# serycjon/MFT

Measured on AMD Instinct MI355X. Metric: tracked frames/sec at 512x512, 12 RAFT iters; flow EPE vs reference, higher is better.
Workload: dtype f32 (update-block products as split fp16 x 3 on the fp16 matrix cores, fp32 accumulation; error per product <= ~2^-23, see DESIGN.md section 4 and parity below); 1 GPU; MFT.track on synthetic 512x512 video, deltas [inf,1,2,4,8,16,32], 7/7.00/7 (min/mean/max) flow pairs per timed frame, 12 RAFT iters, seeded synthetic weights (BASELINE.json configs[1]); parallelism=single GPU, frames_resident_in_hbm=True, preroll_frames=32

## Files before the change

### include/mftx.h

```cpp
#ifndef MFTX_H
#define MFTX_H

#include <stddef.h>
#include <stdint.h>

#ifdef __cplusplus
extern "C" {
#endif

#define MFTX_VERSION 400

#define MFTX_E_ARG (-1)
#define MFTX_E_ALIGN (-2)
#define MFTX_E_WORKSPACE (-3)
#define MFTX_E_STATE (-4)

#define MFTX_MAX_CANDIDATES 16

int mftx_version(void);
const char *mftx_last_error_string(void);

#define MFTX_PROFILE_CATEGORIES 14
int mftx_profile_begin(void);
int mftx_profile_end(double *ms, double *work, long long *count, int n);
// ... 20 lines not shown
                     float *out, int ld_out, float *hx, int ld_hx, void *stream);

int mftx_fmap_pyramid(const float *f2, int P, int C, int h, int w, float *lvl1, float *lvl2, float *lvl3, void *stream);
int mftx_corr_lookup_ondemand(const float *f1, const float *f2l0, const float *f2l1, const float *f2l2, const float *f2l3,
                              const float *coords, int P, int C, int h, int w, int r,
                              float *out, int ld_out, void *stream);

typedef struct mftx_conv_desc {
    const float *a0; int lda0; int c0;
    const float *a1; int lda1; int c1;
    const float *wpk; const float *bias;
    float *out; int ldo;
    int P, h, w;
    int N;
    int kh, kw;
    int act;
    float out_scale;
    const float *addend; int ld_addend;
    int stride, hin, win, pad_y, pad_x, residual_mode;
    int arith;
    int a_split, out_split;
} mftx_conv_desc;
#define MFTX_ARITH_F32 0
#define MFTX_ARITH_SPLIT 1
int mftx_conv2d(const mftx_conv_desc *d, void *stream);
int mftx_conv2d_tile(const mftx_conv_desc *d, int tile, void *stream);

int mftx_pack_tile_conv_weights(const float *wpk, int N, int taps, int cin, int cin_pad, void *wtile, void *stream);
int mftx_tile_conv2d(const mftx_conv_desc *d, const void *wtile, void *stream);
#define MFTX_OU_HEADS_WTILE_BYTES 6635520
int mftx_pack_ou_heads_weights(const float *w1pk, int cin_pad, const float *w2pk, void *wtile, void *wproj, void *stream);
int mftx_ou_heads(const float *a_split, int lda, int P, int h, int w, const void *wtile, const float *b1, const void *wproj, const float *b2,
                  float *T, float *out, int ld_out, void *stream);
int mftx_gru_half(const float *h_in, int ld_hin, const float *motion, int ld_mo, const void *wzr, const void *wq, const float *pre_zr,
                  const float *pre_q, float *z, const float *hf_in, float *hf_out, float *h_out, int ld_hout, int P, int h, int w, int pass,
                  void *stream);
int mftx_tile_conv_fills_chip(int P, int h, int w);
#define MFTX_FLOW_HEAD_WEIGHT_BYTES 32768
int mftx_pack_flow_head_weights(const float *w2pk, void *wproj, void *stream);
int mftx_flow_head(const float *hsplit, int ld_h, int P, int h, int w, const void *wtile, const float *b1, const void *wproj,
                   const float *b2, float *T, float *delta, float *coords, void *stream);
int mftx_split_weights(const float *wpk, void *out, long long n_floats, void *stream);
#define MFTX_SPLIT_LIMIT 65504.0f
int mftx_count_not_below(const float *x, long long n, float limit, unsigned *count, void *stream);

typedef struct mftx_raft mftx_raft;
#define MFTX_RAFT_NUM_WEIGHTS 34
int mftx_raft_create(const float *const *weights, int n_weights, mftx_raft **out);
void mftx_raft_destroy(mftx_raft *r);
size_t mftx_raft_workspace_bytes(int P, int h, int w);
int mftx_raft_set_ondemand(mftx_raft *r, int on);
int mftx_raft_set_split_weights(mftx_raft *r, const void *const *split, int n);
int mftx_raft_arith(const mftx_raft *r);
int mftx_raft_set_lookup_fused(mftx_raft *r, const void *wfused);
int mftx_raft_set_flow_fused(mftx_raft *r, const void *wflow);
int mftx_raft_set_tile_weights(mftx_raft *r, const void *const *tile, int n);
int mftx_raft_set_flow_head(mftx_raft *r, const void *wproj);
int mftx_raft_set_ou_heads(mftx_raft *r, const void *wtile, const void *wproj);
int mftx_raft_set_coords_trace(mftx_raft *r, float *trace);
#define MFTX_RAFT_OPT_FORK 0
#define MFTX_RAFT_OPT_PRESPLIT 1
#define MFTX_RAFT_OPT_GROUP 2
#define MFTX_RAFT_OPT_FUSE_LOOKUP 3
#define MFTX_RAFT_OPT_GRAPH 4
#define MFTX_RAFT_OPT_FUSE_FLOW 5
#define MFTX_RAFT_OPT_TILE_CONV 6
#define MFTX_RAFT_OPT_FUSE_HEAD 7
#define MFTX_RAFT_OPT_TILE_VOLUME 8
#define MFTX_RAFT_OPT_FUSE_GRU 9
#define MFTX_RAFT_OPT_TILE_CELLS 10
#define MFTX_RAFT_OPT_FUSE_OU 11
#define MFTX_RAFT_OPT_TILE_CONV2P 12
int mftx_raft_set_option(mftx_raft *r, int option, int value);
int mftx_raft_set_nonfinite_counter(mftx_raft *r, unsigned *counter);
int mftx_raft_clear_graphs(mftx_raft *r);
int mftx_raft_graph_stats(const mftx_raft *r, unsigned long long *captures, unsigned long long *replays);
size_t mftx_raft_workspace_bytes_for(const mftx_raft *r, int P, int h, int w);
int mftx_raft_workspace_layout(int P, int h, int w, size_t *offsets, int n);
int mftx_raft_workspace_layout_for(const mftx_raft *r, int P, int h, int w, size_t *offsets, int n);
int mftx_raft_refine(mftx_raft *r, int P, int h, int w, int iters,
                     const float *fmap1, const float *fmap2, const float *net, const float *inp,
                     const float *flow_init,
                     int pad_left, int pad_right, int pad_top, int pad_bottom,
                     float *flow, float *occl, float *sigma, float *packed, float *flow_lr,
                     void *workspace, size_t workspace_bytes, void *stream);
int mftx_raft_refine_gather(mftx_raft *r, int P, int h, int w, int iters, const float *const *fmap1,
                            const float *const *fmap2, const float *const *net, const float *const *inp,
                            const float *flow_init, int pad_left, int pad_right, int pad_top, int pad_bottom,
                            float *flow, float *occl, float *sigma, float *packed, float *flow_lr_out,
                            void *workspace, size_t workspace_bytes, void *stream);
size_t mftx_raft_frame_prepare_bytes(int h, int w);
int mftx_raft_frame_prepare(mftx_raft *r, int h, int w, const float *fmap, const float *inp, float *ctx_zr1, float *ctx_q1,
                            float *ctx_zr2, float *ctx_q2, void *fmap_split, void *scratch, size_t scratch_bytes, void *stream);
int mftx_raft_refine_gather_ex(mftx_raft *r, int P, int h, int w, int iters, const float *const *fmap1,
                               const float *const *fmap2, const float *const *net, const float *const *inp,
                               const float *const *ctx_parts, const void *const *fmap1_split, const void *fmap2_split,
                               const float *flow_init, int pad_left, int pad_right, int pad_top, int pad_bottom,
                               float *flow, float *occl, float *sigma, float *packed, float *flow_lr_out,
                               void *workspace, size_t workspace_bytes, void *stream);
int mftx_volume_query_split(const float *in, void *out, long long n_floats, void *stream);

typedef struct mftx_encoder mftx_encoder;
int mftx_encoder_create(const float *const *weights, int n_weights, int instance_norm, mftx_encoder **out);
int mftx_encoder_set_split_weights(mftx_encoder *e, const void *const *split, int n);
int mftx_encoder_set_graph(mftx_encoder *e, int on);
void mftx_encoder_destroy(mftx_encoder *e);
size_t mftx_encoder_workspace_bytes(int H0, int W0);
int mftx_encoder_forward(mftx_encoder *e, const uint8_t *img, int H0, int W0, float *out0, float *out1,
                         void *workspace, size_t workspace_bytes, void *stream);

int mftx_convex_upsample(const float *flow_lr, const float *ou, int ld_ou, const float *mask,
                         int P, int h, int w,
                         int pad_left, int pad_right, int pad_top, int pad_bottom,
                         float *flow, float *occl, float *sigma, float *packed, void *stream);

int mftx_chain(const float *flowL, const float *occlL, const float *sigmaL,
               const float *flowR, const float *occlR, const float *sigmaR,
               int H, int W, float *flowO, float *occlO, float *sigmaO, void *stream);

int mftx_warp_backward(const float *flow, const float *img, int C, int H, int W, float *out, void *stream);

int mftx_select(int K, const float *const *flow, const float *const *occl, const float *const *sigma,
                float thr, int H, int W,
                float *flowO, float *occlO, float *sigmaO, int8_t *chosen, void *stream);

int mftx_chain_select(int K,
                      const float *const *flowL, const float *const *occlL, const float *const *sigmaL,
                      const float *const *flowR, const float *const *occlR, const float *const *sigmaR,
                      float thr, int H, int W,
                      float *flowO, float *occlO, float *sigmaO, int8_t *chosen, void *stream);

int mftx_chain_select_packed(int K,
// ... 43 lines not shown
```

### mft_amd/_lib.py

```python
from __future__ import annotations

import ctypes as C
import os
from pathlib import Path

_HERE = Path(__file__).resolve().parent
LIB_PATH = _HERE / "libmftx.so"

MAX_CANDIDATES = 16
NUM_RAFT_WEIGHTS = 34
LOOKUP_CONVC1_WEIGHT_BYTES = 393216
FLOW_BRANCH_WEIGHT_BYTES = 352256
FLOW_HEAD_WEIGHT_BYTES = 32768
OU_HEADS_WTILE_BYTES = 6635520
SPLIT_LIMIT = 65504.0


class ConvDesc(C.Structure):
    _fields_ = [("a0", C.c_void_p), ("lda0", C.c_int), ("c0", C.c_int),
                ("a1", C.c_void_p), ("lda1", C.c_int), ("c1", C.c_int),
                ("wpk", C.c_void_p), ("bias", C.c_void_p),
                ("out", C.c_void_p), ("ldo", C.c_int),
                ("P", C.c_int), ("h", C.c_int), ("w", C.c_int),
                ("N", C.c_int), ("kh", C.c_int), ("kw", C.c_int),
                ("act", C.c_int), ("out_scale", C.c_float),
                ("addend", C.c_void_p), ("ld_addend", C.c_int),
                ("stride", C.c_int), ("hin", C.c_int), ("win", C.c_int), ("pad_y", C.c_int), ("pad_x", C.c_int),
                ("residual_mode", C.c_int), ("arith", C.c_int), ("a_split", C.c_int), ("out_split", C.c_int)]


_PP = C.POINTER(C.c_void_p)

SIGNATURES = {
    "mftx_version": (C.c_int, []),
    "mftx_last_error_string": (C.c_char_p, []),
    "mftx_profile_begin": (C.c_int, []),
    "mftx_profile_end": (C.c_int, [C.POINTER(C.c_double), C.POINTER(C.c_double), C.POINTER(C.c_longlong), C.c_int]),
    "mftx_corr_pyramid": (C.c_int, [C.c_void_p, C.c_void_p, C.c_int, C.c_int, C.c_int, C.c_int,
                                    C.c_void_p, C.c_void_p, C.c_void_p, C.c_void_p, C.c_void_p]),
    "mftx_corr_pyramid_split": (C.c_int, [C.c_void_p, C.c_void_p, C.c_int, C.c_int, C.c_int, C.c_int,
                                          C.c_void_p, C.c_void_p, C.c_void_p, C.c_void_p, C.c_void_p, C.c_void_p]),
    "mftx_corr_pyramid_layout": (C.c_int, [C.c_int, C.c_int, C.POINTER(C.c_longlong), C.POINTER(C.c_int)]),
    "mftx_corr_lookup": (C.c_int, [C.c_void_p] * 5 + [C.c_int] * 4 + [C.c_void_p, C.c_int, C.c_void_p]),
    "mftx_fmap_pyramid": (C.c_int, [C.c_void_p] + [C.c_int] * 4 + [C.c_void_p] * 4),
    "mftx_corr_lookup_ondemand": (C.c_int, [C.c_void_p] * 6 + [C.c_int] * 5 + [C.c_void_p, C.c_int, C.c_void_p]),
    "mftx_raft_set_ondemand": (C.c_int, [C.c_void_p, C.c_int]),
    "mftx_raft_workspace_bytes_for": (C.c_size_t, [C.c_void_p, C.c_int, C.c_int, C.c_int]),
    "mftx_conv2d": (C.c_int, [C.POINTER(ConvDesc), C.c_void_p]),
    "mftx_conv2d_tile": (C.c_int, [C.POINTER(ConvDesc), C.c_int, C.c_void_p]),
    "mftx_encoder_set_split_weights": (C.c_int, [C.c_void_p, _PP, C.c_int]),
    "mftx_raft_set_split_weights": (C.c_int, [C.c_void_p, _PP, C.c_int]),
    "mftx_raft_arith": (C.c_int, [C.c_void_p]),
    "mftx_raft_set_lookup_fused": (C.c_int, [C.c_void_p, C.c_void_p]),
    "mftx_raft_set_flow_fused": (C.c_int, [C.c_void_p, C.c_void_p]),
    "mftx_raft_set_tile_weights": (C.c_int, [C.c_void_p, _PP, C.c_int]),
    "mftx_raft_set_flow_head": (C.c_int, [C.c_void_p, C.c_void_p]),
    "mftx_raft_set_ou_heads": (C.c_int, [C.c_void_p, C.c_void_p, C.c_void_p]),
    "mftx_pack_ou_heads_weights": (C.c_int, [C.c_void_p, C.c_int, C.c_void_p, C.c_void_p, C.c_void_p, C.c_void_p]),
    "mftx_ou_heads": (C.c_int, [C.c_void_p, C.c_int, C.c_int, C.c_int, C.c_int, C.c_void_p, C.c_void_p, C.c_void_p, C.c_void_p, C.c_void_p,
                                C.c_void_p, C.c_int, C.c_void_p]),
    "mftx_pack_flow_head_weights": (C.c_int, [C.c_void_p, C.c_void_p, C.c_void_p]),
    "mftx_flow_head": (C.c_int, [C.c_void_p, C.c_int, C.c_int, C.c_int, C.c_int] + [C.c_void_p] * 8),
    "mftx_pack_tile_conv_weights": (C.c_int, [C.c_void_p, C.c_int, C.c_int, C.c_int, C.c_int, C.c_void_p, C.c_void_p]),
    "mftx_tile_conv2d": (C.c_int, [C.POINTER(ConvDesc), C.c_void_p, C.c_void_p]),
    "mftx_pack_flow_branch_weights": (C.c_int, [C.c_void_p, C.c_void_p, C.c_void_p, C.c_void_p]),
    "mftx_flow_branch": (C.c_int, [C.c_void_p, C.c_int, C.c_int, C.c_int, C.c_void_p, C.c_void_p, C.c_void_p, C.c_void_p,
                                   C.c_int, C.c_void_p, C.c_int, C.c_void_p]),
    "mftx_raft_set_option": (C.c_int, [C.c_void_p, C.c_int, C.c_int]),
    "mftx_raft_set_coords_trace": (C.c_int, [C.c_void_p, C.c_void_p]),
    "mftx_gru_half": (C.c_int, [C.c_void_p, C.c_int, C.c_void_p, C.c_int, C.c_void_p, C.c_void_p, C.c_void_p, C.c_void_p, C.c_void_p, C.c_void_p,
                                C.c_void_p, C.c_void_p, C.c_int, C.c_int, C.c_int, C.c_int, C.c_int, C.c_void_p]),
    "mftx_tile_conv_fills_chip": (C.c_int, [C.c_int, C.c_int, C.c_int]),
    "mftx_raft_clear_graphs": (C.c_int, [C.c_void_p]),
    "mftx_raft_set_nonfinite_counter": (C.c_int, [C.c_void_p, C.c_void_p]),
    "mftx_raft_graph_stats": (C.c_int, [C.c_void_p, C.POINTER(C.c_ulonglong), C.POINTER(C.c_ulonglong)]),
    "mftx_pack_lookup_convc1_weights": (C.c_int, [C.c_void_p, C.c_int, C.c_void_p, C.c_void_p]),
    "mftx_corr_lookup_convc1": (C.c_int, [C.c_void_p] * 5 + [C.c_int] * 3 + [C.c_void_p, C.c_void_p, C.c_void_p,
                                                                            C.c_int, C.c_int, C.c_void_p]),
    "mftx_split_weights": (C.c_int, [C.c_void_p, C.c_void_p, C.c_longlong, C.c_void_p]),
    "mftx_count_not_below": (C.c_int, [C.c_void_p, C.c_longlong, C.c_float, C.c_void_p, C.c_void_p]),
    "mftx_raft_create": (C.c_int, [_PP, C.c_int, C.POINTER(C.c_void_p)]),
    "mftx_raft_destroy": (None, [C.c_void_p]),
    "mftx_raft_workspace_bytes": (C.c_size_t, [C.c_int, C.c_int, C.c_int]),
    "mftx_raft_workspace_layout": (C.c_int, [C.c_int, C.c_int, C.c_int, C.POINTER(C.c_size_t), C.c_int]),
    "mftx_raft_workspace_layout_for": (C.c_int, [C.c_void_p, C.c_int, C.c_int, C.c_int, C.POINTER(C.c_size_t), C.c_int]),
    "mftx_raft_refine": (C.c_int, [C.c_void_p, C.c_int, C.c_int, C.c_int, C.c_int,
                                   C.c_void_p, C.c_void_p, C.c_void_p, C.c_void_p, C.c_void_p,
                                   C.c_int, C.c_int, C.c_int, C.c_int,
                                   C.c_void_p, C.c_void_p, C.c_void_p, C.c_void_p, C.c_void_p,
                                   C.c_void_p, C.c_size_t, C.c_void_p]),
    "mftx_raft_refine_gather": (C.c_int, [C.c_void_p, C.c_int, C.c_int, C.c_int, C.c_int,
                                          _PP, _PP, _PP, _PP, C.c_void_p,
                                          C.c_int, C.c_int, C.c_int, C.c_int,
                                          C.c_void_p, C.c_void_p, C.c_void_p, C.c_void_p, C.c_void_p,
                                          C.c_void_p, C.c_size_t, C.c_void_p]),
    "mftx_raft_refine_gather_ex": (C.c_int, [C.c_void_p, C.c_int, C.c_int, C.c_int, C.c_int,
                                             _PP, _PP, _PP, _PP, _PP, _PP, C.c_void_p, C.c_void_p,
                                             C.c_int, C.c_int, C.c_int, C.c_int,
                                             C.c_void_p, C.c_void_p, C.c_void_p, C.c_void_p, C.c_void_p,
                                             C.c_void_p, C.c_size_t, C.c_void_p]),
    "mftx_raft_frame_prepare_bytes": (C.c_size_t, [C.c_int, C.c_int]),
    "mftx_raft_frame_prepare": (C.c_int, [C.c_void_p, C.c_int, C.c_int] + [C.c_void_p] * 8 + [C.c_size_t, C.c_void_p]),
    "mftx_volume_query_split": (C.c_int, [C.c_void_p, C.c_void_p, C.c_longlong, C.c_void_p]),
    "mftx_encoder_create": (C.c_int, [_PP, C.c_int, C.c_int, C.POINTER(C.c_void_p)]),
    "mftx_encoder_destroy": (None, [C.c_void_p]),
    "mftx_encoder_set_graph": (C.c_int, [C.c_void_p, C.c_int]),
    "mftx_encoder_workspace_bytes": (C.c_size_t, [C.c_int, C.c_int]),
    "mftx_encoder_forward": (C.c_int, [C.c_void_p, C.c_void_p, C.c_int, C.c_int, C.c_void_p, C.c_void_p,
                                       C.c_void_p, C.c_size_t, C.c_void_p]),
    "mftx_convex_upsample": (C.c_int, [C.c_void_p, C.c_void_p, C.c_int, C.c_void_p] + [C.c_int] * 7
                             + [C.c_void_p] * 5),
    "mftx_chain": (C.c_int, [C.c_void_p] * 6 + [C.c_int, C.c_int] + [C.c_void_p] * 4),
    "mftx_warp_backward": (C.c_int, [C.c_void_p, C.c_void_p, C.c_int, C.c_int, C.c_int, C.c_void_p, C.c_void_p]),
    "mftx_select": (C.c_int, [C.c_int, _PP, _PP, _PP, C.c_float, C.c_int, C.c_int] + [C.c_void_p] * 5),
    "mftx_chain_select": (C.c_int, [C.c_int] + [_PP] * 6 + [C.c_float, C.c_int, C.c_int] + [C.c_void_p] * 5),
    "mftx_chain_select_packed": (C.c_int, [C.c_int] + [_PP] * 4 + [C.c_float, C.c_int, C.c_int] + [C.c_void_p] * 5),
    "mftx_chain_select_multi": (C.c_int, [C.c_int, C.POINTER(C.c_int)] + [_PP] * 4 + [C.c_float, C.c_int, C.c_int] + [_PP] * 4
                                + [C.c_void_p]),
    "mftx_sample_points": (C.c_int, [C.c_int, _PP, _PP, _PP, C.c_int, C.c_int, C.c_int, C.c_void_p, C.c_void_p,
                                     C.c_void_p, C.c_longlong, C.c_int, C.c_void_p]),
    "mftx_splat_forward": (C.c_int, [C.c_void_p, C.c_void_p, C.c_int, C.c_void_p, C.c_int, C.c_int, C.c_int, C.c_int, C.c_int,
                                     C.c_void_p, C.c_void_p]),
    "mftx_splat_resolve": (C.c_int, [C.c_void_p, C.c_int, C.c_int, C.c_int, C.c_int, C.c_float, C.c_int, C.c_void_p, C.c_void_p]),
    "mftx_overlay_edit": (C.c_int, [C.c_void_p, C.c_void_p, C.c_void_p, C.c_void_p, C.c_int, C.c_int, C.c_int, C.c_float,
                                    C.c_void_p, C.c_void_p, C.c_void_p]),
    "mftx_overlay_dots": (C.c_int, [C.c_void_p, C.c_void_p, C.c_int, C.c_int, C.c_void_p, C.c_longlong, C.c_int, C.c_double,
                                    C.c_int, C.c_int, C.c_int, C.c_void_p]),
    "mftx_quantize_workspace_bytes": (C.c_size_t, []),
    "mftx_quantize_u16": (C.c_int, [C.c_void_p, C.c_longlong, C.c_void_p, C.c_void_p, C.c_void_p, C.c_size_t, C.c_void_p]),
    "mftx_dequantize_u16": (C.c_int, [C.c_void_p, C.c_longlong, C.c_float, C.c_float, C.c_void_p, C.c_void_p]),
    "mftx_png_unfilter": (C.c_int, [C.c_void_p, C.c_int, C.c_int, C.c_int]),
    "mftx_copy_bytes": (C.c_int, [C.c_void_p, C.c_void_p, C.c_longlong, C.c_void_p]),
}
# ... 35 lines not shown
```

### mft_amd/csrc/common.h

```cpp
#pragma once
#include <hip/hip_runtime.h>
#include <cstdarg>
#include <cstdio>
#include <cstdint>
#include <cstdlib>
#include "../../include/mftx.h"

namespace mftx {

void set_error(const char *fmt, ...);

inline int fail(int code, const char *fmt, ...) {
    char buf[512];
    va_list ap;
    va_start(ap, fmt);
    vsnprintf(buf, sizeof buf, fmt, ap);
    va_end(ap);
    set_error("%s", buf);
    return code;
}

inline int check_launch(const char *what) {
    hipError_t e = hipGetLastError();
    if (e != hipSuccess) {
// ... 102 lines not shown
                       int ld_out, float *hx, int ld_hx, hipStream_t s, const float *T = nullptr, const float *b2h = nullptr,
                       float *coords_out = nullptr, float *delta_out = nullptr);
struct TileConvLaunch {
    const float *a0; int lda0;
    const float *a1; int lda1;
    int cin;
    const void *wf;
    const float *bias;
    const float *addend; int ld_addend;
    float *out; int ldo; int out_split;
    float *z, *rh, *hf, *hx; int ld_hf, ld_hx;
    const void *wproj; float *tout;
    int P, h, w, N, kh, kw, epi;
    int cells;
};
struct GruHalfLaunch {
    const float *h_in; int ld_hin; const float *mo; int ld_mo;
    const void *wzr, *wq;
    const float *pre_zr, *pre_q;
    const float *const *ctx;
    float *z; const float *hf_in; float *hf_out;
    float *h_out; int ld_hout;
    int P, h, w, pass;
    int cells;
};
int launch_gru_half(const GruHalfLaunch &d, hipStream_t s);
int launch_pack_flow_head(const float *w2pk, void *out, hipStream_t s);
int launch_pack_tile_conv2p(const float *wpk, int N, int cin_pad, void *out, hipStream_t s);
int launch_tile_conv2p(const float *a, int lda, const void *wf, const float *bias, float *out, int ldo, int n_valid, int P, int h, int w, int cells,
                       hipStream_t s);
constexpr size_t OU_HEAD_WTILE_BYTES = 8ull * 5 * 9 * 9 * 128 * 16, OU_HEAD_WPROJ_BYTES = 32768;
int launch_pack_ou_head(const float *w1pk, int cin_pad, const float *w2pk, void *wtile, void *wproj, hipStream_t s);
struct OuGather { const float *hx, *corr; int ld_corr; const float *coords1, *delta; float *flow_lr; };
int launch_ou_heads(const float *a, int lda, int P, int h, int w, const void *wtile, const float *b1, const void *wproj, const float *b2, float *T,
                    float *out, int ld_out, int cells, hipStream_t s, const OuGather *ga = nullptr);
int launch_flow_head_sum(const float *T, const float *b2, float *delta, const float *coords_in, float *coords_out, int P, int h, int w, hipStream_t s);
bool tile_conv_applicable(int kh, int kw, int cin, int N);
bool tile_conv_small_tiles_fill(int P, int h, int w);
bool tile_conv_fills_chip(int P, int h, int w, int kh, int kw);
int launch_pack_tile_conv(const float *wpk, int N, int taps, int cin, int cin_pad, void *out, hipStream_t s);
int launch_tile_conv(const TileConvLaunch &d, hipStream_t s);
int launch_fmap_pyramid(const float *f2, int P, int C, int h, int w, float *const lvl[3], hipStream_t s);
int launch_corr_ondemand(const float *f1, const float *const f2lvl[4], const float *coords, int P, int h, int w,
                         float *out, int ld_out, hipStream_t s);
int launch_convex_upsample(const float *flow_lr, const float *ou, int ld_ou, const float *mask,
                           int P, int h, int w, int pl, int pr, int pt, int pb,
                           float *flow, float *occl, float *sigma, float *packed, hipStream_t s, unsigned *nonfinite = nullptr);

}
```

### mft_amd/csrc/raft_engine.hip

```cpp
#include "common.h"
#include "profile.h"
#include "motion_front.h"
#include "graph_cache.h"
#include <cstdlib>
#include <new>

namespace mftx {


struct InitGather { int on; PairPtrs netp, inpp; };
struct CtxTable { const float **table; const float *own[4]; int supplied; PairPtrs parts[4]; };
__global__ void init_state_kernel(const float *__restrict__ net, const float *__restrict__ inp,
                                  const float *__restrict__ flow_init, float *hx, float *hf, float *coords1, int M, int h,
                                  int w, InitGather ga, CtxTable ct) {
    const long long i = (long long)blockIdx.x * blockDim.x + threadIdx.x;
    if (i >= (long long)M * 64) return;
    if (ct.table != nullptr && i < (long long)(M / (h * w)) * 4) {
        const int b = (int)(i >> 2), k = (int)(i & 3);
        ct.table[i] = ct.supplied ? ct.parts[k].p[b] : ct.own[k] + (long long)b * h * w * ((k & 1) ? 128 : 256);
    }
    const int m = (int)(i >> 6), q = (int)(i & 63);
    if (ga.on) {
        const int b = m / (h * w);
        net = ga.netp.p[b] - (long long)b * h * w * 128;
        inp = ga.inpp.p[b] - (long long)b * h * w * 128;
    }
    const float4 v = (q < 32) ? reinterpret_cast<const float4 *>(net)[(long long)m * 32 + q]
                              : reinterpret_cast<const float4 *>(inp)[(long long)m * 32 + (q - 32)];
    if (hf != nullptr) {
        store_split4v(hx + (long long)m * 384, 4 * q, v);
        if (q < 32) reinterpret_cast<float4 *>(hf + (long long)m * 128)[q] = v;
    } else {
        reinterpret_cast<float4 *>(hx + (long long)m * 384)[q] = v;
    }
    if (q == 0) {
        const int rem = m % (h * w);
        float cx = (float)(rem % w), cy = (float)(rem / w);
        if (flow_init != nullptr) {
            cx += flow_init[2 * (long long)m];
            cy += flow_init[2 * (long long)m + 1];
        }
        coords1[2 * (long long)m] = cx;
        coords1[2 * (long long)m + 1] = cy;
    }
}

__global__ __launch_bounds__(256) void convf1_kernel(ConvF1Args q) {
    __shared__ __attribute__((aligned(16))) float patch[2][7][48];
    const int half = threadIdx.x >> 7;
    convf1_strip(q, blockIdx.x * 2 + half, patch[half], threadIdx.x & 127);
}

__global__ __launch_bounds__(256) void lookup_convf1_kernel(LookupArgs lp, ConvF1Args q, int lookup_blocks, int f1_blocks) {
    __shared__ __attribute__((aligned(16))) float patch[2][7][48];
// ... 28 lines not shown
        } else v = load_split4(hx + (long long)m * 384 + 256, 4 * (q - 146));
        store_split4v(ouin + (long long)m * 712, 4 * q, v);
        return;
    }
    if (q < 64) v = reinterpret_cast<const float4 *>(hx + (long long)m * 384)[q];
    else if (q < 145) v = reinterpret_cast<const float4 *>(corr + (long long)m * ld_corr)[q - 64];
    else if (q == 145) {
        const int rem = m % (h * w);
        const float fx = coords1[2 * (long long)m] - (float)(rem % w);
        const float fy = coords1[2 * (long long)m + 1] - (float)(rem / w);
        v = make_float4(fx, fy, delta[2 * (long long)m], delta[2 * (long long)m + 1]);
        flow_lr[2 * (long long)m] = fx;
        flow_lr[2 * (long long)m + 1] = fy;
    } else v = reinterpret_cast<const float4 *>(hx + (long long)m * 384 + 256)[q - 146];
    reinterpret_cast<float4 *>(ouin + (long long)m * 712)[q] = v;
}

enum WeightSlot {
    W_CONVC1, B_CONVC1, W_CONVC2, B_CONVC2, W_CONVF1, B_CONVF1, W_CONVF2, B_CONVF2, W_CONV, B_CONV,
    W_ZR1_DYN, W_ZR1_INP, B_ZR1, W_Q1_DYN, W_Q1_INP, B_Q1, W_ZR2_DYN, W_ZR2_INP, B_ZR2, W_Q2_DYN, W_Q2_INP, B_Q2,
    W_FH1, B_FH1, W_FH2, B_FH2, W_MASK0, B_MASK0, W_MASK2, B_MASK2,
    W_OU1, B_OU1, W_OU2, B_OU2, W_COUNT
};

struct Workspace {
    float *lvl[4];
    float *f2l[3];
    float *coords1, *corr, *cor1, *corflo, *flo1, *hx, *z, *rh, *fh, *delta, *mask, *ouin, *ouh, *ou, *flow_lr;
    float *pre_zr[2], *pre_q[2];
    float *f2s;
    float *hf;
    float *hb, *hfb;
    const float **ctx;
    int ld_corr;
    size_t bytes;
};

static Workspace carve(void *base, int P, int h, int w, bool ondemand = false, bool split = false) {
    Workspace ws{};
    const size_t N = (size_t)h * w, M = (size_t)P * N;
    size_t off = 0;
    auto take = [&](size_t floats) {
        float *p = base ? reinterpret_cast<float *>(static_cast<char *>(base) + off) : nullptr;
        off += (floats * sizeof(float) + 255) & ~size_t(255);
        return p;
    };
    const PyramidLayout L = pyramid_layout(h, w);
    for (int l = 0; l < 4; ++l) ws.lvl[l] = take(ondemand ? 0 : M * (size_t)L.stride[l]);
    for (int l = 1; l < 4; ++l) ws.f2l[l - 1] = take(ondemand ? (size_t)P * (h >> l) * (w >> l) * 256 : 0);
    ws.coords1 = take(M * 2);
    ws.ld_corr = 324;
    ws.corr = take(M * ws.ld_corr);
    ws.cor1 = take(M * 256);
    ws.corflo = take(M * 256);
    ws.flo1 = take(M * 128);
    ws.hx = take(M * 384);
    ws.z = take(M * 128);
    ws.rh = take(M * 128);
    ws.fh = take(M * 256);
    ws.delta = take(M * 2);
    ws.mask = take(M * 576);
    ws.ouin = take(M * 712);
    ws.ouh = take(M * 256);
    ws.ou = take(M * 4);
    ws.flow_lr = take(M * 2);
    for (int pass = 0; pass < 2; ++pass) { ws.pre_zr[pass] = take(M * 256); ws.pre_q[pass] = take(M * 128); }
    ws.f2s = take(ondemand || !split ? 0 : M * 256);
    ws.hf = take(split ? M * 128 : 0);
    ws.hb = take(split ? M * 128 : 0);
    ws.hfb = take(split ? M * 128 : 0);
    ws.ctx = reinterpret_cast<const float **>(take(split ? (size_t)P * 8 : 0));
    ws.bytes = off;
    return ws;
}

}

using namespace mftx;

struct mftx_raft {
    uint32_t magic;
    int ondemand;
    int arith;
    const float *w[W_COUNT];
    const float *wg[W_COUNT];
    hipStream_t side;
    hipEvent_t ev_fork, ev_join;
    float *coords_trace;
    GraphCache *graphs;
    const void *wfused;
    const void *wflow;
    const void *wproj;
    const void *wt[W_COUNT];
    const void *wou, *wouproj;
    int opt[13];
    unsigned *nonfinite;
};
static constexpr int GEMM_SLOTS[] = {W_CONVC1, W_CONVC2, W_CONVF2, W_CONV, W_ZR1_DYN, W_ZR1_INP, W_Q1_DYN, W_Q1_INP,
                                     W_ZR2_DYN, W_ZR2_INP, W_Q2_DYN, W_Q2_INP, W_FH1, W_MASK0, W_MASK2, W_OU1};
static constexpr uint32_t RAFT_MAGIC = 0x4d465458;

extern "C" int mftx_raft_create(const float *const *weights, int n_weights, mftx_raft **out) {
    if (!weights || !out) return fail(MFTX_E_ARG, "raft_create: null pointer");
    if (n_weights != W_COUNT) return fail(MFTX_E_ARG, "raft_create: expected %d weight tensors, got %d", (int)W_COUNT, n_weights);
    for (int i = 0; i < W_COUNT; ++i) {
        if (!weights[i]) return fail(MFTX_E_ARG, "raft_create: weight %d is null", i);
        if (!aligned16(weights[i])) return fail(MFTX_E_ALIGN, "raft_create: weight %d not 16-byte aligned", i);
    }
    mftx_raft *r = new (std::nothrow) mftx_raft;
    if (!r) return fail(MFTX_E_ARG, "raft_create: out of host memory");
    r->magic = RAFT_MAGIC;
    r->ondemand = 0;
    r->arith = MFTX_ARITH_F32;
    r->side = nullptr; r->ev_fork = nullptr; r->ev_join = nullptr;
    r->wfused = nullptr;
    r->wflow = nullptr;
    r->wproj = nullptr;
    r->wou = nullptr; r->wouproj = nullptr;
    for (int i = 0; i < W_COUNT; ++i) r->wt[i] = nullptr;
    r->coords_trace = nullptr;
    r->nonfinite = nullptr;
    r->graphs = new (std::nothrow) GraphCache;
    r->opt[MFTX_RAFT_OPT_FORK] = -1; r->opt[MFTX_RAFT_OPT_PRESPLIT] = 1; r->opt[MFTX_RAFT_OPT_GROUP] = 1; r->opt[MFTX_RAFT_OPT_FUSE_LOOKUP] = 1; r->opt[MFTX_RAFT_OPT_GRAPH] = 1; r->opt[MFTX_RAFT_OPT_FUSE_FLOW] = 1; r->opt[MFTX_RAFT_OPT_TILE_CONV] = 1; r->opt[MFTX_RAFT_OPT_FUSE_HEAD] = 1; r->opt[MFTX_RAFT_OPT_TILE_VOLUME] = 1; r->opt[MFTX_RAFT_OPT_FUSE_GRU] = 1; r->opt[MFTX_RAFT_OPT_TILE_CELLS] = 0; r->opt[MFTX_RAFT_OPT_FUSE_OU] = 1; r->opt[MFTX_RAFT_OPT_TILE_CONV2P] = 1;
    for (int i = 0; i < W_COUNT; ++i) r->w[i] = r->wg[i] = weights[i];
    *out = r;
    return 0;
}

extern "C" void mftx_raft_destroy(mftx_raft *r) {
    if (r && r->magic == RAFT_MAGIC) {
        r->magic = 0;
        if (r->ev_fork) (void)hipEventDestroy(r->ev_fork);
        if (r->ev_join) (void)hipEventDestroy(r->ev_join);
        if (r->side) (void)hipStreamDestroy(r->side);
        delete r->graphs;
        delete r;
    }
}

static int ensure_side_stream(mftx_raft *r) {
    if (r->side) return 0;
    hipError_t e = hipStreamCreateWithFlags(&r->side, hipStreamNonBlocking);
    if (e == hipSuccess) e = hipEventCreateWithFlags(&r->ev_fork, hipEventDisableTiming);
    if (e == hipSuccess) e = hipEventCreateWithFlags(&r->ev_join, hipEventDisableTiming);
    if (e != hipSuccess) return fail((int)e, "raft_refine: side stream: %s", hipGetErrorString(e));
    return 0;
}

extern "C" size_t mftx_raft_workspace_bytes(int P, int h, int w) {
    if (P <= 0 || h <= 0 || w <= 0) return 0;
    return carve(nullptr, P, h, w).bytes;
// ... 34 lines not shown

extern "C" int mftx_raft_set_flow_fused(mftx_raft *r, const void *wflow) {
    if (!r || r->magic != RAFT_MAGIC) return fail(MFTX_E_STATE, "raft_set_flow_fused: bad handle");
    if (wflow && !aligned16(wflow)) return fail(MFTX_E_ALIGN, "raft_set_flow_fused: weights not 16-byte aligned");
    r->wflow = wflow;
    if (r->graphs) r->graphs->clear();
    return 0;
}

extern "C" int mftx_raft_set_tile_weights(mftx_raft *r, const void *const *tile, int n) {
    if (!r || r->magic != RAFT_MAGIC) return fail(MFTX_E_STATE, "raft_set_tile_weights: bad handle");
    if (r->graphs) r->graphs->clear();
    if (!tile) { for (int i = 0; i < W_COUNT; ++i) r->wt[i] = nullptr; return 0; }
    if (n != W_COUNT) return fail(MFTX_E_ARG, "raft_set_tile_weights: expected %d slots, got %d", (int)W_COUNT, n);
    for (int i = 0; i < W_COUNT; ++i)
        if (tile[i] && !aligned16(tile[i])) return fail(MFTX_E_ALIGN, "raft_set_tile_weights: slot %d not 16-byte aligned", i);
    for (int i = 0; i < W_COUNT; ++i) r->wt[i] = tile[i];
    return 0;
}

extern "C" int mftx_raft_set_flow_head(mftx_raft *r, const void *wproj) {
    if (!r || r->magic != RAFT_MAGIC) return fail(MFTX_E_STATE, "raft_set_flow_head: bad handle");
    if (wproj && !aligned16(wproj)) return fail(MFTX_E_ALIGN, "raft_set_flow_head: weights not 16-byte aligned");
    r->wproj = wproj;
    if (r->graphs) r->graphs->clear();
    return 0;
}

extern "C" int mftx_raft_set_ou_heads(mftx_raft *r, const void *wtile, const void *wproj) {
    if (!r || r->magic != RAFT_MAGIC) return fail(MFTX_E_STATE, "raft_set_ou_heads: bad handle");
    if ((wtile == nullptr) != (wproj == nullptr)) return fail(MFTX_E_ARG, "raft_set_ou_heads: both weight streams, or neither");
    if (wtile && (!aligned16(wtile) || !aligned16(wproj))) return fail(MFTX_E_ALIGN, "raft_set_ou_heads: weights not 16-byte aligned");
    r->wou = wtile; r->wouproj = wproj;
    if (r->graphs) r->graphs->clear();
    return 0;
}

extern "C" int mftx_raft_set_coords_trace(mftx_raft *r, float *trace) {
    if (!r || r->magic != RAFT_MAGIC) return fail(MFTX_E_STATE, "raft_set_coords_trace: bad handle");
    r->coords_trace = trace;
    return 0;
}

extern "C" int mftx_raft_clear_graphs(mftx_raft *r) {
    if (!r || r->magic != RAFT_MAGIC) return fail(MFTX_E_STATE, "raft_clear_graphs: bad handle");
    if (r->graphs) r->graphs->clear();
    return 0;
}

extern "C" int mftx_raft_set_nonfinite_counter(mftx_raft *r, unsigned *counter) {
    if (!r || r->magic != RAFT_MAGIC) return fail(MFTX_E_STATE, "raft_set_nonfinite_counter: bad handle");
    if (counter && (reinterpret_cast<uintptr_t>(counter) & 3)) return fail(MFTX_E_ALIGN, "raft_set_nonfinite_counter: counter not 4-byte aligned");
    r->nonfinite = counter;
    return 0;
}

extern "C" int mftx_raft_set_option(mftx_raft *r, int option, int value) {
    if (!r || r->magic != RAFT_MAGIC) return fail(MFTX_E_STATE, "raft_set_option: bad handle");
    if (option < 0 || option > MFTX_RAFT_OPT_TILE_CONV2P) return fail(MFTX_E_ARG, "raft_set_option: unknown option %d", option);
    r->opt[option] = value;
    if (r->graphs) r->graphs->clear();
    return 0;
}

extern "C" int mftx_raft_arith(const mftx_raft *r) {
    return (r && r->magic == RAFT_MAGIC) ? r->arith : -1;
// ... 5 lines not shown
}

static int workspace_layout(const mftx_raft *r, int P, int h, int w, size_t *offsets, int n) {
    if (P <= 0 || h <= 0 || w <= 0 || !offsets || n != 19) return fail(MFTX_E_ARG, "workspace_layout: need 19 slots");
    char *base = reinterpret_cast<char *>(uintptr_t(1) << 40);
    Workspace ws = carve(base, P, h, w, r && r->ondemand != 0, r && r->arith == MFTX_ARITH_SPLIT);
    float *ptrs[19] = {ws.lvl[0], ws.lvl[1], ws.lvl[2], ws.lvl[3], ws.coords1, ws.corr, ws.cor1, ws.corflo, ws.flo1,
                       ws.hx, ws.z, ws.rh, ws.fh, ws.delta, ws.mask, ws.ouin, ws.ouh, ws.ou, ws.flow_lr};
    for (int i = 0; i < 19; ++i) offsets[i] = (size_t)(reinterpret_cast<char *>(ptrs[i]) - base);
    return 0;
}
extern "C" int mftx_raft_workspace_layout(int P, int h, int w, size_t *offsets, int n) {
    return workspace_layout(nullptr, P, h, w, offsets, n);
}
extern "C" int mftx_raft_workspace_layout_for(const mftx_raft *r, int P, int h, int w, size_t *offsets, int n) {
    if (!r || r->magic != RAFT_MAGIC) return fail(MFTX_E_STATE, "workspace_layout_for: bad handle");
    return workspace_layout(r, P, h, w, offsets, n);
}

#define TRY(expr) do { int _e = (expr); if (_e) return _e; } while (0)

static mftx_conv_desc conv_desc(const float *a0, int lda0, int c0, const float *a1, int lda1, int c1,
                                const float *w, const float *b, float *out, int ldo, int P, int h, int wd, int N,
                                int kh, int kw, int act, float scale = 1.f, const float *addend = nullptr,
                                int ld_addend = 0) {
    mftx_conv_desc d{};
    d.addend = addend; d.ld_addend = ld_addend;
    d.a0 = a0; d.lda0 = lda0; d.c0 = c0; d.a1 = a1; d.lda1 = lda1; d.c1 = c1;
    d.wpk = w; d.bias = b; d.out = out; d.ldo = ldo; d.P = P; d.h = h; d.w = wd; d.N = N;
    d.kh = kh; d.kw = kw; d.act = act; d.out_scale = scale;
    return d;
}

struct RefineGather { PairPtrs f1, f2, net, inp; bool f2_shared; bool has_ctx, has_f1s; PairPtrs ctx[4], f1s; const float *f2s; };

static int launch_context_parts(const mftx_raft *r, bool tiles_on, bool sp, const float *inp, int ld, int P, int h, int w,
                                float *const zr[2], float *const q[2], hipStream_t s) {
    const float *const *W = r->w;
    const float *const *G = r->wg;
    for (int pass = 0; pass < 2; ++pass) {
        const int kh = pass ? 5 : 1, kw = pass ? 1 : 5;
        const int slot[2] = {pass ? W_ZR2_INP : W_ZR1_INP, pass ? W_Q2_INP : W_Q1_INP};
        const float *bias[2] = {W[pass ? B_ZR2 : B_ZR1], W[pass ? B_Q2 : B_Q1]};
        float *out[2] = {zr[pass], q[pass]};
        for (int k = 0; k < 2; ++k) {
            const int N = k ? 128 : 256;
            if (tiles_on && r->wt[slot[k]]) {
                TileConvLaunch t{};
                t.a0 = inp; t.lda0 = ld; t.cin = 128; t.wf = r->wt[slot[k]]; t.bias = bias[k];
                t.P = P; t.h = h; t.w = w; t.N = N; t.kh = kh; t.kw = kw; t.epi = 0;
                t.cells = r->opt[MFTX_RAFT_OPT_TILE_CELLS];
                t.out = out[k]; t.ldo = N;
                TRY(launch_tile_conv(t, s));
            } else {
                mftx_conv_desc d = conv_desc(inp, ld, 128, nullptr, 0, 0, G[slot[k]], bias[k], out[k], N, P, h, w, N, kh, kw, 0);
                d.arith = r->arith; d.a_split = sp; d.out_split = false;
                TRY(launch_conv(d, s));
            }
        }
    }
    return 0;
}
static int refine_impl(mftx_raft *r, int P, int h, int w, int iters, const float *fmap1,
                                const float *fmap2, const float *net, const float *inp, const float *flow_init,
                                int pad_left,
                                int pad_right, int pad_top, int pad_bottom, float *flow, float *occl,
                                float *sigma, float *packed, float *flow_lr_out, void *workspace,
// ... 23 lines not shown
    const bool use_graph = r->graphs && r->opt[MFTX_RAFT_OPT_GRAPH] != 0 && !prof_enabled() && !r->coords_trace && !ondemand;
    hipStream_t caller = s;
    bool proxied = false;
    if (use_graph && s == nullptr) {
        hipStream_t own = r->graphs->proxy.enter(s);
        if (own) { s = own; proxied = true; }
    }
    struct Leave { GraphCache *g; hipStream_t caller; bool on; ~Leave() { if (on) g->proxy.leave(caller); } } leave{r->graphs, caller, proxied};
    const int N = h * w, M = P * N;
    const float *const *W = r->w;
    const float *const *G = r->wg;
    const int AR = r->arith;
    auto gemm = [AR, SP](mftx_conv_desc d, bool a = true, bool o = false) { d.arith = AR; d.a_split = SP && a; d.out_split = SP && o; return d; };

    const float *f2lv[4] = {fmap2, ws.f2l[0], ws.f2l[1], ws.f2l[2]};
    if (ondemand) TRY(launch_fmap_pyramid(fmap2, P, 256, h, w, ws.f2l, s));
    else if (gather) {
        const long long pair_floats = (long long)N * 256;
        const float *f2s = ws.f2s;
        if (gather->f2_shared && gather->f2s) f2s = gather->f2s;
        else if (gather->f2_shared) TRY(launch_split_weights(gather->f2.p[0], ws.f2s, pair_floats, s));
        else for (int b = 0; b < P; ++b) TRY(launch_split_weights(gather->f2.p[b], ws.f2s + b * pair_floats, pair_floats, s));
        TRY(launch_volume_tile(nullptr, f2s, P, h, w, ws.lvl, s, gather->has_f1s ? &gather->f1s : &gather->f1, gather->f2_shared ? 0 : pair_floats,
                               gather->has_f1s));
    }
    else TRY(launch_corr_pyramid(fmap1, fmap2, P, 256, h, w, ws.lvl, s, r->arith == MFTX_ARITH_SPLIT ? ws.f2s : nullptr, r->opt[MFTX_RAFT_OPT_TILE_VOLUME]));
    const bool tiles_on = SP && r->opt[MFTX_RAFT_OPT_TILE_CONV] != 0 &&
                          (r->opt[MFTX_RAFT_OPT_TILE_CONV] == 2 ||
                           (tile_conv_fills_chip(P, h, w, 3, 3) && tile_conv_fills_chip(P, h, w, 1, 5) && tile_conv_fills_chip(P, h, w, 5, 1)));
    auto tile_w = [&](int slot) -> const void * { return tiles_on ? r->wt[slot] : nullptr; };
    const bool gru_fused = tile_w(W_ZR1_DYN) && tile_w(W_Q1_DYN) && tile_w(W_ZR2_DYN) && tile_w(W_Q2_DYN) &&
                           r->opt[MFTX_RAFT_OPT_FUSE_GRU] != 0;
    const bool ctx_supplied = gather && gather->has_ctx && gru_fused;
    {
        const long long slots = (long long)M * 64;
        ProfScope prof(PC_GLUE, s, 0);
        InitGather ga{};
        if (gather) { ga.on = 1; ga.netp = gather->net; ga.inpp = gather->inp; }
        CtxTable ct{};
        if (gru_fused) {
            ct.table = ws.ctx;
            ct.own[0] = ws.pre_zr[0]; ct.own[1] = ws.pre_q[0]; ct.own[2] = ws.pre_zr[1]; ct.own[3] = ws.pre_q[1];
            ct.supplied = ctx_supplied ? 1 : 0;
            if (ctx_supplied) for (int k = 0; k < 4; ++k) ct.parts[k] = gather->ctx[k];
        }
        hipLaunchKernelGGL(init_state_kernel, dim3((unsigned)((slots + 255) / 256)), dim3(256), 0, s, net, inp,
                           flow_init, ws.hx, SP ? ws.hf : nullptr, ws.coords1, M, h, w, ga, ct);
        TRY(check_launch("init_state"));
    }
    float *flow_lr = flow_lr_out ? flow_lr_out : ws.flow_lr;
    auto core = [&]() -> int {
    auto tile_layer = [&](const float *a0, int lda0, const float *a1, int lda1, const void *wf, const float *bias, int N, int kh, int kw, int epi) {
        TileConvLaunch t{};
        t.a0 = a0; t.lda0 = lda0; t.a1 = a1; t.lda1 = lda1; t.cin = a1 ? 256 : 128; t.wf = wf; t.bias = bias;
        t.P = P; t.h = h; t.w = w; t.N = N; t.kh = kh; t.kw = kw; t.epi = epi;
        t.cells = r->opt[MFTX_RAFT_OPT_TILE_CELLS];
        return t;
    };
    if (!ctx_supplied) TRY(launch_context_parts(r, tiles_on, SP, ws.hx + 128, 384, P, h, w, ws.pre_zr, ws.pre_q, s));
    const float *lv[4] = {ws.lvl[0], ws.lvl[1], ws.lvl[2], ws.lvl[3]};
    const int strips = cdiv(w, F1_CELLS);
    float *ccur = ws.coords1, *calt = ws.flo1;
    bool pending = false;
    for (int it = 0; it < iters; ++it) {
        const bool last = (it == iters - 1);
        if (r->coords_trace &&
            hipMemcpyAsync(r->coords_trace + (size_t)it * M * 2, ccur, (size_t)M * 8, hipMemcpyDeviceToDevice, s) != hipSuccess)
            return fail(MFTX_E_STATE, "raft_refine: coords trace copy failed");
        const ConvF1Args f1{ccur, W[W_CONVF1], W[B_CONVF1], ws.flo1, ws.hx, h, w, strips, P * h * strips, SP ? 1 : 0};
        const int f1_blocks = cdiv(f1.n_strips, 2);
        const bool nofuse = r->opt[MFTX_RAFT_OPT_GROUP] == 0, nopair = nofuse;
        const mftx_conv_desc c2 = gemm(conv_desc(ws.cor1, 256, 256, nullptr, 0, 0, G[W_CONVC2], W[B_CONVC2], ws.corflo, 256, P, h, w, 192, 3, 3, 1), true, true);
        const mftx_conv_desc f2 = gemm(conv_desc(ws.flo1, 128, 128, nullptr, 0, 0, G[W_CONVF2], W[B_CONVF2], ws.corflo + 192, 256, P, h, w, 64, 3, 3, 1), true, true);
        const int fork_env = r->opt[MFTX_RAFT_OPT_FORK];
        const bool fuse_flow = SP && r->wflow != nullptr && r->opt[MFTX_RAFT_OPT_FUSE_FLOW] != 0 && !nofuse;
        if (fuse_flow) {
            if (pending) {
                TRY(launch_flow_branch(ccur, P, h, w, r->wflow, W[B_CONVF1], W[B_CONVF2], ws.corflo + 192, 256, ws.hx, 384, s, ws.fh, W[B_FH2], calt, ws.delta));
                float *t = ccur; ccur = calt; calt = t;
                pending = false;
            } else TRY(launch_flow_branch(ccur, P, h, w, r->wflow, W[B_CONVF1], W[B_CONVF2], ws.corflo + 192, 256, ws.hx, 384, s));
        }
        const bool serial = fuse_flow || prof_enabled() || nofuse || (AR == MFTX_ARITH_SPLIT && (fork_env == 0 || fork_env == 2));
        const bool forked = !serial && AR == MFTX_ARITH_SPLIT;
        const bool flow_first = !fuse_flow && serial && fuse_lookup && fork_env == 2 && !prof_enabled() && !nofuse;
        if (flow_first) {
            hipLaunchKernelGGL(convf1_kernel, dim3(f1_blocks), dim3(256), 0, s, f1);
            TRY(check_launch("convf1"));
            TRY(launch_conv(f2, s));
        }
        if (forked) {
            TRY(ensure_side_stream(r));
// ... 73 lines not shown
        }
        const bool head_fused = tile_w(W_FH1) && r->wproj != nullptr && r->opt[MFTX_RAFT_OPT_FUSE_HEAD] != 0;
        if (head_fused) {
            TileConvLaunch t = tile_layer(ws.hx, 384, nullptr, 0, tile_w(W_FH1), W[B_FH1], 256, 3, 3, 4);
            t.wproj = r->wproj; t.tout = ws.fh;
            TRY(launch_tile_conv(t, s));
            const bool defer = !last && fuse_flow && r->opt[MFTX_RAFT_OPT_FUSE_HEAD] != 2 && !r->coords_trace;
            if (defer) pending = true;
            else {
                float *dst = last ? ws.coords1 : ccur;
                TRY(launch_flow_head_sum(ws.fh, W[B_FH2], ws.delta, ccur, dst, P, h, w, s));
                ccur = dst;
            }
        } else if (tile_w(W_FH1)) {
            TileConvLaunch t = tile_layer(ws.hx, 384, nullptr, 0, tile_w(W_FH1), W[B_FH1], 256, 3, 3, 1);
            t.out = ws.fh; t.ldo = 256;
            TRY(launch_tile_conv(t, s));
        } else TRY(launch_conv(gemm(conv_desc(ws.hx, 384, 128, nullptr, 0, 0, G[W_FH1], W[B_FH1], ws.fh, 256, P, h, w, 256, 3, 3, 1), true, false), s));
        if (!head_fused) {
            const mftx_conv_desc fh2 = conv_desc(ws.fh, 256, 256, nullptr, 0, 0, W[W_FH2], W[B_FH2], ws.delta, 2, P, h, w, 2, 3, 3, 0);
            if (!conv_small_applicable(fh2)) return fail(MFTX_E_STATE, "raft_refine: flow-head layer does not fit the small-N kernel");
            TRY(launch_conv_small(fh2, s, ccur, 2));
        }
        if (!last) continue;
        if (r->coords_trace &&
            hipMemcpyAsync(r->coords_trace + (size_t)iters * M * 2, ccur, (size_t)M * 8, hipMemcpyDeviceToDevice, s) != hipSuccess)
            return fail(MFTX_E_STATE, "raft_refine: coords trace copy failed");
        if (tile_w(W_MASK0)) {
            TileConvLaunch t = tile_layer(ws.hx, 384, nullptr, 0, tile_w(W_MASK0), W[B_MASK0], 256, 3, 3, 1);
            t.out = ws.fh; t.ldo = 256; t.out_split = SP ? 1 : 0;
            TRY(launch_tile_conv(t, s));
        } else TRY(launch_conv(gemm(conv_desc(ws.hx, 384, 128, nullptr, 0, 0, G[W_MASK0], W[B_MASK0], ws.fh, 256, P, h, w, 256, 3, 3, 1), true, true), s));
        TRY(launch_conv(gemm(conv_desc(ws.fh, 256, 256, nullptr, 0, 0, G[W_MASK2], W[B_MASK2], ws.mask, 576, P, h, w, 576, 1, 1, 0, 0.25f), true, false), s));
        const bool ou_fused = tiles_on && r->wou != nullptr && r->opt[MFTX_RAFT_OPT_FUSE_OU] != 0;
        if (!ou_fused || r->opt[MFTX_RAFT_OPT_FUSE_OU] == 2) {
            const long long slots = (long long)M * 178;
            ProfScope prof(PC_GLUE, s, 0);
            hipLaunchKernelGGL(ou_gather_kernel, dim3((unsigned)((slots + 255) / 256)), dim3(256), 0, s, ws.hx,
                               ws.corr, ws.ld_corr, ccur, ws.delta, ws.ouin, flow_lr, M, h, w, SP ? 1 : 0);
            TRY(check_launch("ou_gather"));
        }
        if (ou_fused) {
            const OuGather ga{ws.hx, ws.corr, ws.ld_corr, ccur, ws.delta, flow_lr};
            const bool mat = r->opt[MFTX_RAFT_OPT_FUSE_OU] == 2;
            TRY(launch_ou_heads(mat ? ws.ouin : nullptr, 712, P, h, w, r->wou, W[B_OU1], r->wouproj, W[B_OU2], ws.ouh, ws.ou, 4, r->opt[MFTX_RAFT_OPT_TILE_CELLS], s,
                                mat ? nullptr : &ga));
        } else {
            TRY(launch_conv(gemm(conv_desc(ws.ouin, 712, 712, nullptr, 0, 0, G[W_OU1], W[B_OU1], ws.ouh, 256, P, h, w, 256, 3, 3, 1), true, false), s));
            TRY(launch_conv(conv_desc(ws.ouh, 256, 256, nullptr, 0, 0, W[W_OU2], W[B_OU2], ws.ou, 4, P, h, w, 3, 3, 3, 0), s));
        }
    }
    return 0;
    };
    if (use_graph) {
        if (AR == MFTX_ARITH_SPLIT && r->opt[MFTX_RAFT_OPT_FORK] != 0) TRY(ensure_side_stream(r));
        GraphKey key{};
        key.v[0] = (uintptr_t)P; key.v[1] = (uintptr_t)h; key.v[2] = (uintptr_t)w; key.v[3] = (uintptr_t)iters;
        key.v[4] = reinterpret_cast<uintptr_t>(workspace); key.v[5] = reinterpret_cast<uintptr_t>(flow_lr_out);
        key.v[6] = (uintptr_t)AR; key.v[7] = reinterpret_cast<uintptr_t>(r->wfused); key.v[8] = reinterpret_cast<uintptr_t>(s);
        key.v[9] = reinterpret_cast<uintptr_t>(r->wflow); key.v[10] = reinterpret_cast<uintptr_t>(r->wt[W_ZR1_DYN]); key.v[11] = reinterpret_cast<uintptr_t>(r->wproj);
        key.v[12] = reinterpret_cast<uintptr_t>(r->wou); key.v[13] = ctx_supplied ? 1 : 0;
        TRY(r->graphs->run(key, s, core));
    } else {
        TRY(core());
    }
    return launch_convex_upsample(flow_lr, ws.ou, 4, ws.mask, P, h, w, pad_left, pad_right, pad_top, pad_bottom,
                                  flow, occl, sigma, packed, s, r->nonfinite);
}

extern "C" int mftx_raft_refine(mftx_raft *r, int P, int h, int w, int iters, const float *fmap1,
                                const float *fmap2, const float *net, const float *inp, const float *flow_init,
                                int pad_left, int pad_right, int pad_top, int pad_bottom, float *flow, float *occl,
                                float *sigma, float *packed, float *flow_lr_out, void *workspace,
                                size_t workspace_bytes, void *stream) {
    return refine_impl(r, P, h, w, iters, fmap1, fmap2, net, inp, flow_init, pad_left, pad_right, pad_top, pad_bottom, flow, occl, sigma,
                       packed, flow_lr_out, workspace, workspace_bytes, stream, nullptr);
}

extern "C" int mftx_raft_refine_gather(mftx_raft *r, int P, int h, int w, int iters, const float *const *fmap1,
                                       const float *const *fmap2, const float *const *net, const float *const *inp,
                                       const float *flow_init, int pad_left, int pad_right, int pad_top, int pad_bottom,
                                       float *flow, float *occl, float *sigma, float *packed, float *flow_lr_out,
                                       void *workspace, size_t workspace_bytes, void *stream) {
    return mftx_raft_refine_gather_ex(r, P, h, w, iters, fmap1, fmap2, net, inp, nullptr, nullptr, nullptr, flow_init, pad_left, pad_right, pad_top,
                                      pad_bottom, flow, occl, sigma, packed, flow_lr_out, workspace, workspace_bytes, stream);
}

extern "C" int mftx_raft_refine_gather_ex(mftx_raft *r, int P, int h, int w, int iters, const float *const *fmap1,
                                          const float *const *fmap2, const float *const *net, const float *const *inp,
                                          const float *const *ctx_parts, const void *const *fmap1_split, const void *fmap2_split,
                                          const float *flow_init, int pad_left, int pad_right, int pad_top, int pad_bottom,
                                          float *flow, float *occl, float *sigma, float *packed, float *flow_lr_out,
                                          void *workspace, size_t workspace_bytes, void *stream) {
    if (!r || r->magic != RAFT_MAGIC) return fail(MFTX_E_STATE, "raft_refine_gather: bad handle");
    if (!fmap1 || !fmap2 || !net || !inp) return fail(MFTX_E_ARG, "raft_refine_gather: null pointer");
    if (P < 1 || P > MFTX_MAX_GATHER) return fail(MFTX_E_ARG, "raft_refine_gather: 1 .. %d pairs", MFTX_MAX_GATHER);
    if (r->arith != MFTX_ARITH_SPLIT || r->ondemand || r->opt[MFTX_RAFT_OPT_TILE_VOLUME] == 0)
        return fail(MFTX_E_STATE, "raft_refine_gather: needs the split arithmetic with the stored, tile-resident correlation volume (use mftx_raft_refine)");
    RefineGather g{};
    g.f2_shared = true;
    for (int b = 0; b < P; ++b) {
        if (!fmap1[b] || !fmap2[b] || !net[b] || !inp[b]) return fail(MFTX_E_ARG, "raft_refine_gather: pair %d has a null map", b);
        if (!aligned16(fmap1[b]) || !aligned16(fmap2[b]) || !aligned16(net[b]) || !aligned16(inp[b])) return fail(MFTX_E_ALIGN, "raft_refine_gather: maps must be 16-byte aligned");
        g.f1.p[b] = fmap1[b]; g.f2.p[b] = fmap2[b]; g.net.p[b] = net[b]; g.inp.p[b] = inp[b];
        if (fmap2[b] != fmap2[0]) g.f2_shared = false;
    }
    if (ctx_parts) {
        for (int i = 0; i < 4 * P; ++i)
            if (!ctx_parts[i] || !aligned16(ctx_parts[i])) return fail(MFTX_E_ALIGN, "raft_refine_gather: context part %d of pair %d null or not 16-byte aligned", i & 3, i >> 2);
        g.has_ctx = true;
        for (int b = 0; b < P; ++b) for (int k = 0; k < 4; ++k) g.ctx[k].p[b] = ctx_parts[4 * b + k];
    }
    if (fmap1_split) {
        for (int b = 0; b < P; ++b) {
            if (!fmap1_split[b] || !aligned16(fmap1_split[b])) return fail(MFTX_E_ALIGN, "raft_refine_gather: split map of pair %d null or not 16-byte aligned", b);
            g.f1s.p[b] = static_cast<const float *>(fmap1_split[b]);
        }
        g.has_f1s = true;
    }
    if (fmap2_split) {
        if (!aligned16(fmap2_split)) return fail(MFTX_E_ALIGN, "raft_refine_gather: the second map's split form must be 16-byte aligned");
        if (!g.f2_shared) return fail(MFTX_E_ARG, "raft_refine_gather: a split second map goes with ONE second map for all pairs");
        g.f2s = static_cast<const float *>(fmap2_split);
    }
    return refine_impl(r, P, h, w, iters, nullptr, nullptr, nullptr, nullptr, flow_init, pad_left, pad_right, pad_top, pad_bottom, flow, occl,
                       sigma, packed, flow_lr_out, workspace, workspace_bytes, stream, &g);
}

__global__ void split_rows_kernel(const float *__restrict__ in, float *__restrict__ out, long long slots, int c4) {
    const long long i = (long long)blockIdx.x * blockDim.x + threadIdx.x;
    if (i >= slots) return;
    const long long m = i / c4;
    const int q = (int)(i - m * c4);
    store_split4v(out + m * 4 * c4, 4 * q, reinterpret_cast<const float4 *>(in)[i]);
}

extern "C" size_t mftx_raft_frame_prepare_bytes(int h, int w) {
    if (h <= 0 || w <= 0) return 0;
    return ((size_t)h * w * 128 * sizeof(float) + 255) & ~size_t(255);
}

extern "C" int mftx_raft_frame_prepare(mftx_raft *r, int h, int w, const float *fmap, const float *inp, float *ctx_zr1, float *ctx_q1,
                                       float *ctx_zr2, float *ctx_q2, void *fmap_split, void *scratch, size_t scratch_bytes, void *stream) {
    if (!r || r->magic != RAFT_MAGIC) return fail(MFTX_E_STATE, "raft_frame_prepare: bad handle");
    if (h < 16 || w < 16 || (long long)h * w > (1ll << 24)) return fail(MFTX_E_ARG, "raft_frame_prepare: bad size");
    const bool want_ctx = ctx_zr1 || ctx_q1 || ctx_zr2 || ctx_q2;
    if (!want_ctx && !fmap_split) return fail(MFTX_E_ARG, "raft_frame_prepare: nothing to write");
    if (r->arith != MFTX_ARITH_SPLIT || r->opt[MFTX_RAFT_OPT_PRESPLIT] == 0)
        return fail(MFTX_E_STATE, "raft_frame_prepare: needs the split arithmetic with split-form activations");
    hipStream_t s = (hipStream_t)stream;
    const long long N = (long long)h * w;
    if (fmap_split) {
        if (!fmap) return fail(MFTX_E_ARG, "raft_frame_prepare: a split map needs fmap");
        TRY(launch_split_weights(fmap, fmap_split, N * 256, s));
    }
    if (!want_ctx) return 0;
    if (!inp || !ctx_zr1 || !ctx_q1 || !ctx_zr2 || !ctx_q2 || !scratch) return fail(MFTX_E_ARG, "raft_frame_prepare: the context parts need inp, all four outputs and the scratch");
    if (r->opt[MFTX_RAFT_OPT_TILE_CONV] == 1)
        return fail(MFTX_E_STATE, "raft_frame_prepare: MFTX_RAFT_OPT_TILE_CONV must be pinned (0 or 2), the batch decides otherwise");
    if (!aligned16(inp) || !aligned16(ctx_zr1) || !aligned16(ctx_q1) || !aligned16(ctx_zr2) || !aligned16(ctx_q2) ||
        (reinterpret_cast<uintptr_t>(scratch) & 255))
        return fail(MFTX_E_ALIGN, "raft_frame_prepare: maps must be 16-byte and the scratch 256-byte aligned");
    if (scratch_bytes < mftx_raft_frame_prepare_bytes(h, w))
        return fail(MFTX_E_WORKSPACE, "raft_frame_prepare: scratch %zu < %zu bytes", scratch_bytes, mftx_raft_frame_prepare_bytes(h, w));
    float *inps = static_cast<float *>(scratch);
    {
        const long long slots = N * 32;
        hipLaunchKernelGGL(split_rows_kernel, dim3((unsigned)((slots + 255) / 256)), dim3(256), 0, s, inp, inps, slots, 32);
        TRY(check_launch("split_rows"));
    }
    float *const zr[2] = {ctx_zr1, ctx_zr2}, *const q[2] = {ctx_q1, ctx_q2};
    return launch_context_parts(r, r->opt[MFTX_RAFT_OPT_TILE_CONV] == 2, true, inps, 128, 1, h, w, zr, q, s);
}

extern "C" int mftx_volume_query_split(const float *in, void *out, long long n_floats, void *stream) {
    if (!in || !out) return fail(MFTX_E_ARG, "volume_query_split: null pointer");
    return launch_volume_query_split(in, out, n_floats, (hipStream_t)stream);
}

extern "C" int mftx_raft_graph_stats(const mftx_raft *r, unsigned long long *captures, unsigned long long *replays) {
    if (!r || r->magic != RAFT_MAGIC || !captures || !replays) return fail(MFTX_E_STATE, "raft_graph_stats: bad arguments");
    *captures = r->graphs ? r->graphs->captures : 0;
    *replays = r->graphs ? r->graphs->replays : 0;
    return 0;
}

extern "C" int mftx_corr_pyramid(const float *f1, const float *f2, int P, int C, int h, int w, float *lvl0,
                                 float *lvl1, float *lvl2, float *lvl3, void *stream) {
    if (!f1 || !f2 || !lvl0 || !lvl1 || !lvl2 || !lvl3) return fail(MFTX_E_ARG, "corr_pyramid: null pointer");
    if (P <= 0 || C <= 0 || C % 32 || h < 8 || w < 8) return fail(MFTX_E_ARG, "corr_pyramid: need C %% 32 == 0, h, w >= 8");
    if (!aligned16(f1) || !aligned16(f2)) return fail(MFTX_E_ALIGN, "corr_pyramid: features must be 16-byte aligned");
    if (!aligned16(lvl0) || !aligned16(lvl1) || !aligned16(lvl2) || !aligned16(lvl3))
        return fail(MFTX_E_ALIGN, "corr_pyramid: levels must be 16-byte aligned");
    float *const lv[4] = {lvl0, lvl1, lvl2, lvl3};
    return launch_corr_pyramid(f1, f2, P, C, h, w, lv, (hipStream_t)stream);
}

extern "C" int mftx_corr_pyramid_split(const float *f1, const float *f2, int P, int C, int h, int w, float *lvl0,
                                       float *lvl1, float *lvl2, float *lvl3, float *f2_scratch, void *stream) {
    if (!f1 || !f2 || !lvl0 || !lvl1 || !lvl2 || !lvl3 || !f2_scratch) return fail(MFTX_E_ARG, "corr_pyramid_split: null pointer");
    if (P <= 0 || C <= 0 || C % 32 || h < 8 || w < 8) return fail(MFTX_E_ARG, "corr_pyramid_split: need C %% 32 == 0, h, w >= 8");
    if (!aligned16(f1) || !aligned16(f2) || (reinterpret_cast<uintptr_t>(f2_scratch) & 31))
        return fail(MFTX_E_ALIGN, "corr_pyramid_split: features must be 16-byte aligned, the scratch 32-byte aligned");
// ... 58 lines not shown
        return launch_tile_conv2p(d->a0, d->lda0, wtile, d->bias, d->out, d->ldo, d->N, d->P, d->h, d->w, 0, (hipStream_t)stream);
    }
    if (d->c0 != 128 || (d->c1 != 0 && d->c1 != 128)) return fail(MFTX_E_ARG, "tile_conv2d: channel segments of 128");
    TileConvLaunch t{};
    t.a0 = d->a0; t.lda0 = d->lda0; t.a1 = d->c1 ? d->a1 : nullptr; t.lda1 = d->lda1; t.cin = d->c0 + d->c1; t.wf = wtile; t.bias = d->bias;
    t.addend = d->addend; t.ld_addend = d->ld_addend; t.out = d->out; t.ldo = d->ldo; t.out_split = d->out_split;
    t.P = d->P; t.h = d->h; t.w = d->w; t.N = d->N; t.kh = d->kh; t.kw = d->kw; t.epi = d->act;
    return launch_tile_conv(t, (hipStream_t)stream);
}

extern "C" int mftx_gru_half(const float *h_in, int ld_hin, const float *motion, int ld_mo, const void *wzr, const void *wq, const float *pre_zr,
                             const float *pre_q, float *z, const float *hf_in, float *hf_out, float *h_out, int ld_hout, int P, int h, int w, int pass,
                             void *stream) {
    GruHalfLaunch g{};
    g.h_in = h_in; g.ld_hin = ld_hin; g.mo = motion; g.ld_mo = ld_mo; g.wzr = wzr; g.wq = wq; g.pre_zr = pre_zr; g.pre_q = pre_q;
    g.z = z; g.hf_in = hf_in; g.hf_out = hf_out; g.h_out = h_out; g.ld_hout = ld_hout; g.P = P; g.h = h; g.w = w; g.pass = pass;
    return launch_gru_half(g, (hipStream_t)stream);
}

extern "C" int mftx_tile_conv_fills_chip(int P, int h, int w) {
    if (P <= 0 || h <= 0 || w <= 0) return 0;
    return tile_conv_fills_chip(P, h, w, 3, 3) || tile_conv_small_tiles_fill(P, h, w) ? 1 : 0;
}

extern "C" int mftx_pack_ou_heads_weights(const float *w1pk, int cin_pad, const float *w2pk, void *wtile, void *wproj, void *stream) {
    return launch_pack_ou_head(w1pk, cin_pad, w2pk, wtile, wproj, (hipStream_t)stream);
}

extern "C" int mftx_ou_heads(const float *a_split, int lda, int P, int h, int w, const void *wtile, const float *b1, const void *wproj, const float *b2,
                             float *T, float *out, int ld_out, void *stream) {
    return launch_ou_heads(a_split, lda, P, h, w, wtile, b1, wproj, b2, T, out, ld_out, 0, (hipStream_t)stream);
}

extern "C" int mftx_pack_flow_head_weights(const float *w2pk, void *wproj, void *stream) {
    return launch_pack_flow_head(w2pk, wproj, (hipStream_t)stream);
}

extern "C" int mftx_flow_head(const float *hsplit, int ld_h, int P, int h, int w, const void *wtile, const float *b1, const void *wproj,
                              const float *b2, float *T, float *delta, float *coords, void *stream) {
    if (!hsplit || !wtile || !b1 || !wproj || !b2 || !T || !delta) return fail(MFTX_E_ARG, "flow_head: null pointer");
    TileConvLaunch t{};
    t.a0 = hsplit; t.lda0 = ld_h; t.cin = 128; t.wf = wtile; t.bias = b1; t.wproj = wproj; t.tout = T;
    t.P = P; t.h = h; t.w = w; t.N = 256; t.kh = 3; t.kw = 3; t.epi = 4;
    if (int e = launch_tile_conv(t, (hipStream_t)stream)) return e;
    return launch_flow_head_sum(T, b2, delta, coords, coords, P, h, w, (hipStream_t)stream);
}

extern "C" int mftx_pack_flow_branch_weights(const float *w98, const float *w2pk, void *wflow, void *stream) {
    if (!w98 || !w2pk || !wflow) return fail(MFTX_E_ARG, "pack_flow_branch_weights: null pointer");
    if (!aligned16(wflow)) return fail(MFTX_E_ALIGN, "pack_flow_branch_weights: output not 16-byte aligned");
    return launch_pack_flow_branch(w98, w2pk, wflow, (hipStream_t)stream);
}

extern "C" int mftx_flow_branch(const float *coords, int P, int h, int w, const void *wflow, const float *b1, const float *b2,
                                float *out, int ld_out, float *hx, int ld_hx, void *stream) {
    return launch_flow_branch(coords, P, h, w, wflow, b1, b2, out, ld_out, hx, ld_hx, (hipStream_t)stream);
}

extern "C" int mftx_fmap_pyramid(const float *f2, int P, int C, int h, int w, float *lvl1, float *lvl2, float *lvl3,
                                 void *stream) {
    if (!f2 || !lvl1 || !lvl2 || !lvl3) return fail(MFTX_E_ARG, "fmap_pyramid: null pointer");
    if (P <= 0 || C <= 0 || C % 4 || h < 8 || w < 8) return fail(MFTX_E_ARG, "fmap_pyramid: need C %% 4 == 0, h, w >= 8");
    if (!aligned16(f2) || !aligned16(lvl1) || !aligned16(lvl2) || !aligned16(lvl3))
        return fail(MFTX_E_ALIGN, "fmap_pyramid: maps must be 16-byte aligned");
    float *const lv[3] = {lvl1, lvl2, lvl3};
    return launch_fmap_pyramid(f2, P, C, h, w, lv, (hipStream_t)stream);
// ... 41 lines not shown
```

### mft_amd/csrc/tile_conv.hip

```cpp
#include "common.h"
#include "profile.h"
#include "device_prims.h"

namespace mftx {

enum TcEpi { TC_LINEAR = 0, TC_RELU = 1, TC_GRU_ZR = 2, TC_GRU_Q = 3,
             TC_RELU_PROJ = 4 };

#ifdef MFTX_LF_TRACE
__device__ unsigned long long tc_trace_buf[8][16];
#define TC_T(code) do { if (blockIdx.x == 0 && tcount < 16) { unsigned long long t_; asm volatile("s_memtime %0\n\ts_waitcnt lgkmcnt(0)" : "=s"(t_) :: "memory"); \
                        if ((threadIdx.x & 63) == 0) tc_trace_buf[threadIdx.x >> 6][tcount] = ((unsigned long long)(code) << 56) | (t_ & 0x00ffffffffffffffull); ++tcount; } } while (0)
__device__ unsigned long long tc_clock_buf[4096][4];
#define TC_CLK(slot) do { if (wv == ((slot) ? 7 : 0) && blockIdx.x < 4096) { unsigned long long t_, r_; \
                          asm volatile("s_waitcnt vmcnt(0) lgkmcnt(0)\n\ts_memtime %0\n\ts_memrealtime %1\n\ts_waitcnt lgkmcnt(0)" : "=s"(t_), "=s"(r_) :: "memory"); \
                          if (lane == 0) { tc_clock_buf[blockIdx.x][slot] = t_; tc_clock_buf[blockIdx.x][2 + slot] = r_; } } } while (0)
#else
#define TC_T(code) do { } while (0)
#define TC_CLK(slot) do { } while (0)
#endif

struct TileConvArgs {
    const float *a0; int lda0;
    const float *a1; int lda1;
    const void *wf;
    const float *bias;
    const float *addend; int ld_addend;
    float *out; int ldo; int out_split;
    float *z, *rh, *hf, *hx; int ld_hf, ld_hx;
    const void *wproj; float *tout;
    int P, h, w, tiles_x, tiles_y;
};

template <int TH, int TW, int KH, int KW, int CIN, int N>
struct TcGeom {
    static constexpr int CELLS = TH * TW, RT = CELLS / 32;
    static constexpr int HH = TH + KH - 1, HWD = TW + KW - 1, HCELLS = HH * HWD;
    static constexpr int CELLB = CIN * 4 + 16;
    static constexpr int NT = N / 32, KS = 8 / NT;
    static constexpr int CG = CIN / 16, GPW = CG / KS;
    static constexpr int STEPS = KH * KW * GPW;
    static constexpr int RED_ROW = N + 4;
    static constexpr int A_BYTES = HCELLS * CELLB, RED_BYTES = KS * CELLS * RED_ROW * 4;
    static constexpr int LDS = A_BYTES > RED_BYTES ? A_BYTES : RED_BYTES;
    static constexpr int PROJ_ROW = 20, PROJ_BYTES = 2 * CELLS * PROJ_ROW * 4;
    static_assert((CELLS == 128 || CELLS == 64 || CELLS == 32) && (N == 128 || N == 256) && (CIN == 128 || CIN == 256 || CIN == 144), "tile_conv: shapes");
    static_assert(LDS <= 160 * 1024, "tile_conv: the input tile must fit the CU's LDS");
};

template <int TH, int TW, int KH, int KW, int CIN, int N, int EPI>
__global__ __launch_bounds__(512, 2) void tile_conv_kernel(TileConvArgs p) {
    using G = TcGeom<TH, TW, KH, KW, CIN, N>;
    extern __shared__ __attribute__((aligned(16))) unsigned char tc_lds[];
    unsigned char *lds = tc_lds;
    const int tid = (int)threadIdx.x, lane = tid & 63, wv = __builtin_amdgcn_readfirstlane(tid >> 6);
    const int tile = (int)blockIdx.x;
    const int tx_ = tile % p.tiles_x, ty_ = (tile / p.tiles_x) % p.tiles_y, img = tile / (p.tiles_x * p.tiles_y);
    const int x0 = tx_ * TW, y0 = ty_ * TH;
    const long long img_base = (long long)img * p.h * p.w;
    const int nt = wv % G::NT, ks = wv / G::NT;
    const uint4 *__restrict__ w2 = reinterpret_cast<const uint4 *>(p.wf) + (long long)((nt * G::KS + ks) * G::STEPS) * 128 + lane;

#ifdef MFTX_LF_TRACE
    int tcount = 0;
#endif
    TC_T(1);
    TC_CLK(0);
    constexpr int PF = 3;
    uint4 bq[PF][2];
#pragma unroll
    for (int s = 0; s < PF; ++s) { bq[s][0] = w2[s * 128]; bq[s][1] = w2[s * 128 + 64]; }

    {
        constexpr int PPC = CIN / 4;
        constexpr int TOTAL = G::HCELLS * PPC, ROUNDS = (TOTAL + 511) / 512, B = 6;
#pragma unroll 1
        for (int r0 = 0; r0 < ROUNDS; r0 += B) {
            uint4 v[B];
#pragma unroll
// ... 510 lines not shown
        !aligned16(d.pre_zr) || !aligned16(d.pre_q) || !aligned16(d.z) || !aligned16(d.hf_in) || !aligned16(d.hf_out))
        return fail(MFTX_E_ALIGN, "gru_half: split-form rows are 32-byte aligned with strides in multiples of 8; the rest 16-byte aligned");
    GruHalfArgs a{};
    a.h_in = d.h_in; a.ld_hin = d.ld_hin; a.mo = d.mo; a.ld_mo = d.ld_mo; a.wzr = d.wzr; a.wq = d.wq; a.pre_zr = d.pre_zr; a.pre_q = d.pre_q; a.ctx = d.ctx; a.pass = d.pass;
    a.z = d.z; a.hf_in = d.hf_in; a.hf_out = d.hf_out; a.h_out = d.h_out; a.ld_hout = d.ld_hout; a.P = d.P; a.h = d.h; a.w = d.w;
    const bool hz = d.pass == 0;
    auto best = [&](int cells, int &th, int &tw) {
        const int ta = hz ? cells / 64 : 64, tb = hz ? 64 : cells / 64;
        const int sa = hz ? cells / 32 : 32, sb = hz ? 32 : cells / 32;
        const long long nl = cells >= 64 ? gru_half_tiles(d.P, d.h, d.w, ta, tb, hz) : (1ll << 62), ns = gru_half_tiles(d.P, d.h, d.w, sa, sb, hz);
        if (nl <= ns) { th = ta; tw = tb; return nl; }
        th = sa; tw = sb; return ns;
    };
    int th = 0, tw = 0, cells = d.cells;
    if (!cells) {
        cells = 128;
        if (!tc_fills(best(128, th, tw))) cells = 64;
    }
    if (cells != 128 && cells != 64 && cells != 32) return fail(MFTX_E_ARG, "gru_half: 128, 64 or 32 cells per tile");
    if (cells == 32) cells = 64;
    best(cells, th, tw);
#define GH(TH, TW, KH, KW) if (th == TH && tw == TW) return gru_half_launch<TH, TW, KH, KW>(a, s)
    if (hz) { GH(2, 64, 1, 5); GH(4, 32, 1, 5); GH(1, 64, 1, 5); GH(2, 32, 1, 5); }
    else { GH(64, 2, 5, 1); GH(32, 4, 5, 1); GH(64, 1, 5, 1); GH(32, 2, 5, 1); }
#undef GH
    return fail(MFTX_E_STATE, "gru_half: no kernel for tiles of %d x %d cells", th, tw);
}

struct OuHeadArgs {
    const float *a; int lda;
    const float *hx; const float *corr; int ld_corr; const float *coords1; const float *delta; float *flow_lr;
    const void *wf;
    const float *bias;
    const void *wproj; float *tout;
    int P, h, w, tiles_x, tiles_y;
};
constexpr int OU_C = 712, OU_PASSES = 5, OU_CP = 144, OU_PROJ_ROW = 28;

template <int TH, int TW, bool GATHER>
__global__ __launch_bounds__(512, 2) void ou_head_kernel(OuHeadArgs p) {
    using G = TcGeom<TH, TW, 3, 3, OU_CP, 256>;
    constexpr int RT = G::RT, CELLS = G::CELLS, PF = 3;
    extern __shared__ __attribute__((aligned(16))) unsigned char tc_lds[];
    unsigned char *lds = tc_lds;
    const int tid = (int)threadIdx.x, lane = tid & 63, wv = __builtin_amdgcn_readfirstlane(tid >> 6);
    const int tile = (int)blockIdx.x;
    const int tx_ = tile % p.tiles_x, ty_ = (tile / p.tiles_x) % p.tiles_y, img = tile / (p.tiles_x * p.tiles_y);
    const int x0 = tx_ * TW, y0 = ty_ * TH;
    const long long img_base = (long long)img * p.h * p.w;
    const uint4 *__restrict__ w2 = reinterpret_cast<const uint4 *>(p.wf) + (long long)(wv * OU_PASSES * G::STEPS) * 128 + lane;
    f32x16 acc[RT], accx[RT];
#pragma unroll
    for (int i = 0; i < RT; ++i)
#pragma unroll
        for (int r = 0; r < 16; ++r) { acc[i][r] = 0.f; accx[i][r] = 0.f; }
    const unsigned char *abase[RT];
    {
        const int r = lane & 31;
#pragma unroll
        for (int i = 0; i < RT; ++i) {
            const int m = 32 * i + r;
            abase[i] = lds + ((m / TW) * G::HWD + (m % TW)) * G::CELLB + (lane >> 5) * 32;
        }
    }
#pragma unroll 1
    for (int pass = 0; pass < OU_PASSES; ++pass) {
        uint4 bq[PF][2];
        const uint4 *__restrict__ wp = w2 + (long long)pass * G::STEPS * 128;
#pragma unroll
        for (int s = 0; s < PF; ++s) { bq[s][0] = wp[s * 128]; bq[s][1] = wp[s * 128 + 64]; }
        if (pass) lds_barrier();
        if constexpr (!GATHER) {
            constexpr int PPC = OU_CP / 4, TOTAL = G::HCELLS * PPC, ROUNDS = (TOTAL + 511) / 512, B = 7;
            const int pc_valid = pass == OU_PASSES - 1 ? (OU_C - (OU_PASSES - 1) * OU_CP) / 4 : PPC;
#pragma unroll 1
            for (int rr = 0; rr < ROUNDS; rr += B) {
                uint4 v[B];
#pragma unroll
                for (int k = 0; k < B; ++k) {
                    const int q = (rr + k) * 512 + tid;
                    v[k] = make_uint4(0u, 0u, 0u, 0u);
                    if (rr + k < ROUNDS && q < TOTAL) {
                        const int c = q / PPC, pc = q - c * PPC;
                        const int cy = c / G::HWD, cx = c - cy * G::HWD;
                        const int yy = y0 - 1 + cy, xx = x0 - 1 + cx;
                        if (yy >= 0 && yy < p.h && xx >= 0 && xx < p.w && pc < pc_valid)
                            v[k] = *reinterpret_cast<const uint4 *>(p.a + (img_base + (long long)yy * p.w + xx) * p.lda + pass * OU_CP + pc * 4);
                    }
                }
#pragma unroll
                for (int k = 0; k < B; ++k) {
                    const int q = (rr + k) * 512 + tid;
                    if (rr + k < ROUNDS && q < TOTAL) {
                        const int c = q / PPC, pc = q - c * PPC;
                        *reinterpret_cast<uint4 *>(lds + c * G::CELLB + pc * 16) = v[k];
                    }
                }
            }
        } else {
            constexpr int GPC = OU_CP / 8, TOTAL = G::HCELLS * GPC, ROUNDS = (TOTAL + 511) / 512, B = 4;
            const float k2048l = __builtin_bit_cast(float, __builtin_amdgcn_readfirstlane(0x45000000));
#pragma unroll 1
            for (int rr = 0; rr < ROUNDS; rr += B) {
                f32x4 v0[B], v1[B];
                int kind[B];
#pragma unroll
                for (int k = 0; k < B; ++k) {
                    const int q = (rr + k) * 512 + tid;
                    v0[k] = f32x4{0.f, 0.f, 0.f, 0.f}; v1[k] = v0[k]; kind[k] = 0;
                    if (rr + k < ROUNDS && q < TOTAL) {
                        const int c = q / GPC, gl = q - c * GPC, Gi = GPC * pass + gl;
                        const int cy = c / G::HWD, cx = c - cy * G::HWD;
                        const int yy = y0 - 1 + cy, xx = x0 - 1 + cx;
                        if (yy >= 0 && yy < p.h && xx >= 0 && xx < p.w && Gi < 89) {
                            const long long cell = img_base + (long long)yy * p.w + xx;
                            if (Gi < 32 || Gi >= 73) {
                                const float *src = p.hx + cell * 384 + (Gi < 32 ? 8 * Gi : 256 + 8 * (Gi - 73));
                                v0[k] = *reinterpret_cast<const f32x4 *>(src); v1[k] = *reinterpret_cast<const f32x4 *>(src + 4); kind[k] = 1;
                            } else if (Gi < 72) {
                                const float *src = p.corr + cell * p.ld_corr + 8 * (Gi - 32);
                                v0[k] = *reinterpret_cast<const f32x4 *>(src); v1[k] = *reinterpret_cast<const f32x4 *>(src + 4); kind[k] = 2;
                            } else {
                                v0[k] = *reinterpret_cast<const f32x4 *>(p.corr + cell * p.ld_corr + 320);
                                const float2 cc = reinterpret_cast<const float2 *>(p.coords1)[cell], dd = reinterpret_cast<const float2 *>(p.delta)[cell];
                                const float fx = cc.x - (float)xx, fy = cc.y - (float)yy;
                                v1[k] = f32x4{fx, fy, dd.x, dd.y}; kind[k] = 2;
                                if (cy >= 1 && cy <= TH && cx >= 1 && cx <= TW) reinterpret_cast<float2 *>(p.flow_lr)[cell] = make_float2(fx, fy);
                            }
                        }
                    }
                }
#pragma unroll
                for (int k = 0; k < B; ++k) {
                    const int q = (rr + k) * 512 + tid;
                    if (rr + k < ROUNDS && q < TOTAL) {
                        const int c = q / GPC, gl = q - c * GPC;
                        u32x4 hi = __builtin_bit_cast(u32x4, v0[k]), lo = __builtin_bit_cast(u32x4, v1[k]);
                        if (kind[k] == 2) split8_raw(v0[k], v1[k], k2048l, hi, lo);
                        *reinterpret_cast<u32x4 *>(lds + c * G::CELLB + gl * 32) = hi;
                        *reinterpret_cast<u32x4 *>(lds + c * G::CELLB + gl * 32 + 16) = lo;
                    }
                }
            }
        }
        lds_barrier();
        tc_kloop<G, 3>(abase, wp, bq, acc, accx);
    }
    lds_barrier();

    const float inv2048 = 1.f / 2048.f;
    float *red = reinterpret_cast<float *>(lds);
#pragma unroll
    for (int i = 0; i < RT; ++i)
#pragma unroll
        for (int b = 0; b < 4; ++b) {
            f32x4 v;
#pragma unroll
            for (int e = 0; e < 4; ++e) v[e] = acc[i][4 * b + e] + accx[i][4 * b + e] * inv2048;
            *reinterpret_cast<f32x4 *>(red + (32 * i + (lane & 31)) * G::RED_ROW + 32 * wv + 8 * b + 4 * (lane >> 5)) = v;
        }
    lds_barrier();
    const float k2048 = __builtin_bit_cast(float, __builtin_amdgcn_readfirstlane(0x45000000));
    const int mt = wv & 3, kh = wv >> 2;
    const uint4 *__restrict__ wpj = reinterpret_cast<const uint4 *>(p.wproj) + lane;
    float *tp = reinterpret_cast<float *>(lds + G::RED_BYTES);
    if (mt < RT) {
        f32x16 d, dx;
#pragma unroll
        for (int r = 0; r < 16; ++r) { d[r] = 0.f; dx[r] = 0.f; }
        const float *xrow = red + (32 * mt + (lane & 31)) * G::RED_ROW + 8 * (lane >> 5);
#pragma unroll
        for (int gg = 0; gg < 8; ++gg) {
            const int g = 8 * kh + gg;
            f32x4 u = *reinterpret_cast<const f32x4 *>(xrow + 16 * g), v = *reinterpret_cast<const f32x4 *>(xrow + 16 * g + 4);
            u += *reinterpret_cast<const f32x4 *>(p.bias + 16 * g + 8 * (lane >> 5));
            v += *reinterpret_cast<const f32x4 *>(p.bias + 16 * g + 8 * (lane >> 5) + 4);
#pragma unroll
            for (int e = 0; e < 4; ++e) { u[e] = relu_keep_nan(u[e]); v[e] = relu_keep_nan(v[e]); }
            u32x4 hi, lo;
            split8_raw(u, v, k2048, hi, lo);
            const f16x8 wh = __builtin_bit_cast(f16x8, wpj[(g * 2) * 64]), wl = __builtin_bit_cast(f16x8, wpj[(g * 2 + 1) * 64]);
            asm volatile("s_nop 1" : "+v"(hi), "+v"(lo));
            const f16x8 xh = __builtin_bit_cast(f16x8, hi), xl = __builtin_bit_cast(f16x8, lo);
            d = mfma_f16(wh, xh, d);
            dx = mfma_f16(wl, xh, dx);
            dx = mfma_f16(wh, xl, dx);
        }
#pragma unroll
        for (int b = 0; b < 4; ++b) {
            const int j0 = 8 * b + 4 * (lane >> 5);
            if (j0 < OU_PROJ_ROW) {
                f32x4 v;
#pragma unroll
                for (int e = 0; e < 4; ++e) v[e] = d[4 * b + e] + dx[4 * b + e] * inv2048;
                *reinterpret_cast<f32x4 *>(tp + (kh * CELLS + 32 * mt + (lane & 31)) * OU_PROJ_ROW + j0) = v;
            }
        }
    }
    lds_barrier();
    for (int idx = tid; idx < CELLS * 27; idx += 512) {
        const int m = idx / 27, j = idx - m * 27;
        const int yy = y0 + m / TW, xx = x0 + m % TW;
        if (yy < p.h && xx < p.w)
            p.tout[(img_base + (long long)yy * p.w + xx) * 27 + j] = tp[m * OU_PROJ_ROW + j] + tp[(CELLS + m) * OU_PROJ_ROW + j];
    }
}

__global__ void pack_ou_head_kernel(const float *__restrict__ wpk, int cin_pad, uint4 *__restrict__ out, long long pieces) {
    const long long idx = (long long)blockIdx.x * blockDim.x + threadIdx.x;
    if (idx >= pieces) return;
    constexpr int GP = OU_CP / 16, STEPS = 9 * GP;
    const int lane = (int)(idx & 63), part = (int)((idx >> 6) & 1);
    const long long t = idx >> 7;
    const int step = (int)(t % STEPS), pass = (int)((t / STEPS) % OU_PASSES), nt = (int)(t / STEPS / OU_PASSES);
    const int tap = step / GP, g = step % GP;
    const int n = 32 * nt + (lane & 31);
    unsigned w[4];
#pragma unroll
    for (int e = 0; e < 4; ++e) {
        const int c = OU_CP * pass + 16 * g + 8 * (lane >> 5) + 2 * e;
        const long long base = ((long long)n * 9 + tap) * cin_pad + c;
        const unsigned a = split_halves(c < OU_C ? wpk[base] : 0.f), b = split_halves(c + 1 < OU_C ? wpk[base + 1] : 0.f);
        w[e] = part ? ((a >> 16) | (b & 0xffff0000u)) : ((a & 0xffffu) | (b << 16));
    }
    out[idx] = make_uint4(w[0], w[1], w[2], w[3]);
}

__global__ void pack_proj27_kernel(const float *__restrict__ w2pk, uint4 *__restrict__ out) {
    const int idx = (int)(blockIdx.x * blockDim.x + threadIdx.x);
    if (idx >= 16 * 2 * 64) return;
    const int lane = idx & 63, part = (idx >> 6) & 1, g = idx >> 7;
    const int j = lane & 31;
    unsigned w[4];
#pragma unroll
    for (int e = 0; e < 4; ++e) {
        const int k = 16 * g + 8 * (lane >> 5) + 2 * e;
        const float v0 = j < 27 ? w2pk[((long long)(j % 3) * 9 + (j / 3)) * 256 + k] : 0.f;
        const float v1 = j < 27 ? w2pk[((long long)(j % 3) * 9 + (j / 3)) * 256 + k + 1] : 0.f;
        const unsigned a = split_halves(v0), b = split_halves(v1);
        w[e] = part ? ((a >> 16) | (b & 0xffff0000u)) : ((a & 0xffffu) | (b << 16));
    }
    out[idx] = make_uint4(w[0], w[1], w[2], w[3]);
}

__global__ __launch_bounds__(256) void ou_heads_sum_kernel(const float *__restrict__ T, const float *__restrict__ b2, float *__restrict__ out, int ld_out,
                                                           int P, int h, int w) {
    const long long i = (long long)blockIdx.x * blockDim.x + threadIdx.x;
    if (i >= (long long)P * h * w * 4) return;
    const int o = (int)(i & 3);
    if (o == 3) return;
    const long long cell = i >> 2;
    const int rem = (int)(cell % ((long long)h * w)), y = rem / w, x = rem - y * w;
    float sum = 0.f;
#pragma unroll
    for (int dy = 0; dy < 3; ++dy)
#pragma unroll
        for (int dx = 0; dx < 3; ++dx) {
            const int yy = y + dy - 1, xx = x + dx - 1;
            if (yy >= 0 && yy < h && xx >= 0 && xx < w) sum += T[(cell + (long long)(dy - 1) * w + (dx - 1)) * 27 + 3 * (3 * dy + dx) + o];
        }
    out[cell * ld_out + o] = sum + b2[o];
}

int launch_pack_ou_head(const float *w1pk, int cin_pad, const float *w2pk, void *wtile, void *wproj, hipStream_t s) {
    if (!w1pk || !w2pk || !wtile || !wproj) return fail(MFTX_E_ARG, "pack_ou_head_weights: null pointer");
    if (cin_pad < OU_C) return fail(MFTX_E_ARG, "pack_ou_head_weights: the first layers have 712 input channels");
    if (!aligned16(wtile) || !aligned16(wproj)) return fail(MFTX_E_ALIGN, "pack_ou_head_weights: outputs not 16-byte aligned");
    const long long pieces = 8ll * OU_PASSES * 9 * (OU_CP / 16) * 128;
    hipLaunchKernelGGL(pack_ou_head_kernel, dim3((unsigned)((pieces + 255) / 256)), dim3(256), 0, s, w1pk, cin_pad, reinterpret_cast<uint4 *>(wtile), pieces);
    hipLaunchKernelGGL(pack_proj27_kernel, dim3(8), dim3(256), 0, s, w2pk, reinterpret_cast<uint4 *>(wproj));
    return check_launch("pack_ou_head");
}

template <int TH, int TW, bool GATHER>
static int ou_head_launch(OuHeadArgs a, hipStream_t s) {
    using G = TcGeom<TH, TW, 3, 3, OU_CP, 256>;
    constexpr int lds_bytes = (G::A_BYTES > G::RED_BYTES ? G::A_BYTES : G::RED_BYTES) + 2 * G::CELLS * OU_PROJ_ROW * 4;
    static_assert(G::RED_BYTES + 2 * G::CELLS * OU_PROJ_ROW * 4 <= 160 * 1024 && lds_bytes <= 160 * 1024, "ou_head: LDS");
    a.tiles_x = cdiv(a.w, TW); a.tiles_y = cdiv(a.h, TH);
    const long long tiles = (long long)a.P * a.tiles_x * a.tiles_y;
    if (tiles > 0x7fffffffLL) return fail(MFTX_E_ARG, "ou_heads: too many tiles");
    auto kern = ou_head_kernel<TH, TW, GATHER>;
    static bool attr_set = false;
    if (!attr_set) {
        if (hipFuncSetAttribute(reinterpret_cast<const void *>(kern), hipFuncAttributeMaxDynamicSharedMemorySize, lds_bytes) != hipSuccess)
            return fail(MFTX_E_STATE, "ou_heads: cannot reserve %d bytes of LDS", lds_bytes);
        attr_set = true;
    }
    ProfScope prof(PC_CONV_GEMM, s, 2.0 * a.P * a.h * a.w * (256.0 * 9 * OU_C + 256.0 * 27));
    hipLaunchKernelGGL(kern, dim3((unsigned)tiles), dim3(512), lds_bytes, s, a);
    return check_launch("ou_heads");
}

int launch_ou_heads(const float *a, int lda, int P, int h, int w, const void *wtile, const float *b1, const void *wproj, const float *b2, float *T,
                    float *out, int ld_out, int cells, hipStream_t s, const OuGather *ga) {
    if ((!a && !ga) || !wtile || !b1 || !wproj || !b2 || !T || !out) return fail(MFTX_E_ARG, "ou_heads: null pointer");
    if (P <= 0 || h <= 0 || w <= 0 || ld_out < 3) return fail(MFTX_E_ARG, "ou_heads: bad sizes");
    if (!aligned16(wtile) || !aligned16(wproj) || !aligned16(b1) || !aligned16(T))
        return fail(MFTX_E_ALIGN, "ou_heads: weights, bias and scratch 16-byte aligned");
    OuHeadArgs k{};
    k.wf = wtile; k.bias = b1; k.wproj = wproj; k.tout = T; k.P = P; k.h = h; k.w = w;
    if (ga) {
        if (!ga->hx || !ga->corr || !ga->coords1 || !ga->delta || !ga->flow_lr) return fail(MFTX_E_ARG, "ou_heads: null pointer among the input's parts");
        if ((reinterpret_cast<uintptr_t>(ga->hx) & 31) || !aligned16(ga->corr) || ga->ld_corr % 4 || ga->ld_corr < 324 || (reinterpret_cast<uintptr_t>(ga->coords1) & 7) ||
            (reinterpret_cast<uintptr_t>(ga->delta) & 7) || (reinterpret_cast<uintptr_t>(ga->flow_lr) & 7))
            return fail(MFTX_E_ALIGN, "ou_heads: hx 32-byte, corr 16-byte (row stride a multiple of 4), coordinates 8-byte aligned");
        k.hx = ga->hx; k.corr = ga->corr; k.ld_corr = ga->ld_corr; k.coords1 = ga->coords1; k.delta = ga->delta; k.flow_lr = ga->flow_lr;
    } else {
        if ((reinterpret_cast<uintptr_t>(a) & 31) || lda % 8 || lda < OU_C) return fail(MFTX_E_ALIGN, "ou_heads: split-form rows are 32-byte aligned with strides in multiples of 8");
        k.a = a; k.lda = lda;
    }
    if (!cells) cells = tile_conv_cells(P, h, w, 3);
    int e;
    if (cells == 128) e = ga ? ou_head_launch<8, 16, true>(k, s) : ou_head_launch<8, 16, false>(k, s);
    else if (cells == 64) e = ga ? ou_head_launch<4, 16, true>(k, s) : ou_head_launch<4, 16, false>(k, s);
    else if (cells == 32) e = ga ? ou_head_launch<2, 16, true>(k, s) : ou_head_launch<2, 16, false>(k, s);
    else return fail(MFTX_E_ARG, "ou_heads: 128, 64 or 32 cells per tile");
    if (e) return e;
    const long long n = (long long)P * h * w * 4;
    ProfScope prof(PC_CONV_SMALL, s, 2.0 * P * h * w * 3 * 9);
    hipLaunchKernelGGL(ou_heads_sum_kernel, dim3((unsigned)((n + 255) / 256)), dim3(256), 0, s, T, b2, out, ld_out, P, h, w);
    return check_launch("ou_heads_sum");
}

__global__ void pack_tile_conv_kernel(const float *__restrict__ wpk, int taps, int cin, int cin_pad, int N, uint4 *__restrict__ out, long long pieces) {
    const long long idx = (long long)blockIdx.x * blockDim.x + threadIdx.x;
    if (idx >= pieces) return;
    const int NT = N / 32, KS = 8 / NT, GPW = cin / 16 / KS, STEPS = taps * GPW;
    const int lane = (int)(idx & 63), part = (int)((idx >> 6) & 1);
    const long long t = idx >> 7;
    const int step = (int)(t % STEPS), ks = (int)((t / STEPS) % KS), nt = (int)(t / STEPS / KS);
    const int tap = step / GPW, g = (step % GPW) * KS + ks;
    const int n = 32 * nt + (lane & 31);
    unsigned w[4];
#pragma unroll
    for (int e = 0; e < 4; ++e) {
        const long long base = ((long long)n * taps + tap) * cin_pad + 16 * g + 8 * (lane >> 5) + 2 * e;
        const unsigned a = split_halves(wpk[base]), b = split_halves(wpk[base + 1]);
        w[e] = part ? ((a >> 16) | (b & 0xffff0000u)) : ((a & 0xffffu) | (b << 16));
    }
    out[idx] = make_uint4(w[0], w[1], w[2], w[3]);
}

int launch_pack_tile_conv(const float *wpk, int N, int taps, int cin, int cin_pad, void *out, hipStream_t s) {
    if (!wpk || !out) return fail(MFTX_E_ARG, "pack_tile_conv_weights: null pointer");
    if ((N != 128 && N != 256) || (cin != 128 && cin != 256) || (taps != 9 && taps != 5) || cin_pad < cin)
        return fail(MFTX_E_ARG, "pack_tile_conv_weights: N in {128, 256}, cin in {128, 256}, 5 or 9 taps");
    if (!aligned16(out)) return fail(MFTX_E_ALIGN, "pack_tile_conv_weights: output not 16-byte aligned");
    const long long pieces = (long long)N * taps * cin * 4 / 16;
    hipLaunchKernelGGL(pack_tile_conv_kernel, dim3((unsigned)((pieces + 255) / 256)), dim3(256), 0, s, wpk, taps, cin, cin_pad, N,
// ... 383 lines not shown
```

### mft_amd/ops.py

```python
from __future__ import annotations

import ctypes as C
import math
from typing import NamedTuple

import torch

from . import _lib
from ._lib import ConvDesc, MftxError, check

ACT = {None: 0, "none": 0, "relu": 1, "sigmoid": 2, "tanh": 3}


def _stream():
    return C.c_void_p(torch.cuda.current_stream().cuda_stream)


def _device_visible(t):
    return isinstance(t, torch.Tensor) and (t.is_cuda or t.is_pinned())


def copy_bytes(src: torch.Tensor, dst: torch.Tensor):
    if not (_device_visible(src) and _device_visible(dst)):
        raise MftxError("copy_bytes: tensors must be on the device or in pinned host memory")
# ... 319 lines not shown
    check(_lib.load().mftx_gru_half(_chk(h_split, "h"), h_split.shape[1], _chk(motion_split, "motion"), motion_split.shape[1],
                                    _chk(wzr_tile, "wzr", torch.uint8), _chk(wq_tile, "wq", torch.uint8), _chk(pre_zr, "pre_zr"),
                                    _chk(pre_q, "pre_q"), _chk(z, "z"), _chk(hf, "hf"), _chk(hf_out, "hf_out"), _chk(h_out, "h_out"), 128, P, h, w,
                                    1 if vertical else 0, _stream()), "mftx_gru_half")
    return hf_out, h_out, z


def pack_flow_head_weights(w2pk: torch.Tensor, check_range: bool = True) -> torch.Tensor:
    lib = _lib.load()
    if w2pk.dim() != 3 or w2pk.shape[0] < 2 or tuple(w2pk.shape[1:]) != (9, 256):
        raise MftxError("pack_flow_head_weights: expected the packed weight [>= 2, 9, 256]")
    if check_range and count_not_below(w2pk, _lib.SPLIT_LIMIT):
        raise SplitRangeError(f"pack_flow_head_weights: weights not below {_lib.SPLIT_LIMIT} in magnitude")
    out = torch.empty(_lib.FLOW_HEAD_WEIGHT_BYTES, dtype=torch.uint8, device=w2pk.device)
    check(lib.mftx_pack_flow_head_weights(_chk(w2pk, "w2pk"), out.data_ptr(), _stream()), "mftx_pack_flow_head_weights")
    return out


def pack_ou_heads_weights(w1pk: torch.Tensor, w2pk: torch.Tensor, check_range: bool = True):
    lib = _lib.load()
    if w1pk.dim() != 3 or w1pk.shape[0] < 256 or w1pk.shape[1] != 9 or w1pk.shape[2] < 712:
        raise MftxError("pack_ou_heads_weights: expected the packed first layers [>= 256, 9, >= 712]")
    if w2pk.dim() != 3 or w2pk.shape[0] < 3 or tuple(w2pk.shape[1:]) != (9, 256):
        raise MftxError("pack_ou_heads_weights: expected the packed second layers [>= 3, 9, 256]")
    if check_range and (count_not_below(w1pk, _lib.SPLIT_LIMIT) or count_not_below(w2pk, _lib.SPLIT_LIMIT)):
        raise SplitRangeError(f"pack_ou_heads_weights: weights not below {_lib.SPLIT_LIMIT} in magnitude")
    wtile = torch.empty(_lib.OU_HEADS_WTILE_BYTES, dtype=torch.uint8, device=w1pk.device)
    wproj = torch.empty(_lib.FLOW_HEAD_WEIGHT_BYTES, dtype=torch.uint8, device=w1pk.device)
    check(lib.mftx_pack_ou_heads_weights(_chk(w1pk, "w1pk"), w1pk.shape[2], _chk(w2pk, "w2pk"), wtile.data_ptr(), wproj.data_ptr(), _stream()),
          "mftx_pack_ou_heads_weights")
    return wtile, wproj


def ou_heads(a_split: torch.Tensor, h: int, w: int, wtile: torch.Tensor, b1, wproj: torch.Tensor, b2):
    lib = _lib.load()
    M = a_split.shape[0]
    P = M // (h * w)
    T = torch.empty(M, 27, dtype=torch.float32, device=a_split.device)
    out = torch.zeros(M, 4, dtype=torch.float32, device=a_split.device)
    check(lib.mftx_ou_heads(_chk(a_split, "a"), a_split.shape[1], P, h, w, _chk(wtile, "wtile", torch.uint8), _chk(b1, "b1"),
                            _chk(wproj, "wproj", torch.uint8), _chk(b2, "b2"), T.data_ptr(), out.data_ptr(), 4, _stream()), "mftx_ou_heads")
    return out


def flow_head(hsplit: torch.Tensor, h: int, w: int, wtile: torch.Tensor, b1, wproj: torch.Tensor, b2, coords=None):
    lib = _lib.load()
    M = hsplit.shape[0]
    P = M // (h * w)
    T = torch.empty(M, 18, dtype=torch.float32, device=hsplit.device)
    delta = torch.empty(M, 2, dtype=torch.float32, device=hsplit.device)
    check(lib.mftx_flow_head(_chk(hsplit, "hsplit"), hsplit.stride(0), P, h, w, _chk(wtile, "wtile", torch.uint8), _chk(b1, "b1"),
                             _chk(wproj, "wproj", torch.uint8), _chk(b2, "b2"), T.data_ptr(), delta.data_ptr(),
                             _chk(coords, "coords") if coords is not None else None, _stream()), "mftx_flow_head")
    return delta


def pack_flow_branch_weights(w98: torch.Tensor, w2pk: torch.Tensor, check_range: bool = True) -> torch.Tensor:
    lib = _lib.load()
    if tuple(w98.shape) != (98, 128) or w2pk.dim() != 3 or w2pk.shape[0] < 64 or tuple(w2pk.shape[1:]) != (9, 128):
        raise MftxError("pack_flow_branch_weights: expected convf1 as [98, 128] and convf2 as [>= 64, 9, 128]")
    if check_range:
        bad = count_not_below(w98, _lib.SPLIT_LIMIT) + count_not_below(w2pk, _lib.SPLIT_LIMIT)
        if bad:
            raise SplitRangeError(f"pack_flow_branch_weights: {bad} weights are not below {_lib.SPLIT_LIMIT} in magnitude")
    out = torch.empty(_lib.FLOW_BRANCH_WEIGHT_BYTES, dtype=torch.uint8, device=w98.device)
    check(lib.mftx_pack_flow_branch_weights(_chk(w98, "w98"), _chk(w2pk, "w2pk"), out.data_ptr(), _stream()),
# ... 366 lines not shown

    GEMM_SLOTS = (0, 2, 6, 8, 10, 11, 13, 14, 16, 17, 19, 20, 22, 26, 28, 30)

    OPTIONS = {"fork": 0, "presplit": 1, "group": 2, "fuse_lookup": 3, "graph": 4, "fuse_flow": 5, "tile_conv": 6, "fuse_head": 7, "tile_volume": 8, "fuse_gru": 9, "tile_cells": 10, "fuse_ou": 11, "tile_conv2p": 12}
    TILE_SLOTS = {2: (192, 256), 8: (128, 256), 10: (256, 256), 11: (256, 128), 13: (128, 256), 14: (128, 128), 16: (256, 256),
                  17: (256, 128), 19: (128, 256), 20: (128, 128), 22: (256, 128), 26: (256, 128)}

    def __init__(self, state_dict: dict, device, ondemand_corr=False, arith=ARITH_SPLIT, options=None):
        lib = _lib.load()
        self.device = torch.device(device)
        self.weights = pack_raft_weights(state_dict, self.device)
        arr, self._keep = _lib.ptr_array([_chk(t, "weight") for t in self.weights])
        handle = C.c_void_p()
        check(lib.mftx_raft_create(arr, len(self.weights), C.byref(handle)), "mftx_raft_create")
        self._h = handle
        self._ws = None
        self.arith = int(arith)
        if self.arith == ARITH_SPLIT:
            self.split = [split_weights(t) if i in self.GEMM_SLOTS else None for i, t in enumerate(self.weights)]
            sarr, self._keep_split = _lib.ptr_array([t.data_ptr() if t is not None else None for t in self.split])
            check(lib.mftx_raft_set_split_weights(self._h, sarr, len(self.split)), "mftx_raft_set_split_weights")
            self.wfused = pack_lookup_convc1_weights(self.weights[0])
            check(lib.mftx_raft_set_lookup_fused(self._h, self.wfused.data_ptr()), "mftx_raft_set_lookup_fused")
            self.wflow = pack_flow_branch_weights(self.weights[4], self.weights[6])
            check(lib.mftx_raft_set_flow_fused(self._h, self.wflow.data_ptr()), "mftx_raft_set_flow_fused")
            self.wtile = [pack_tile_conv_weights(t, *self.TILE_SLOTS[i]) if i in self.TILE_SLOTS else None
                          for i, t in enumerate(self.weights)]
            tarr, self._keep_tile = _lib.ptr_array([t.data_ptr() if t is not None else None for t in self.wtile])
            check(lib.mftx_raft_set_tile_weights(self._h, tarr, len(self.wtile)), "mftx_raft_set_tile_weights")
            self.wproj = pack_flow_head_weights(self.weights[24])
            check(lib.mftx_raft_set_flow_head(self._h, self.wproj.data_ptr()), "mftx_raft_set_flow_head")
            self.wou, self.wouproj = pack_ou_heads_weights(self.weights[30], self.weights[32])
            check(lib.mftx_raft_set_ou_heads(self._h, self.wou.data_ptr(), self.wouproj.data_ptr()), "mftx_raft_set_ou_heads")
        elif self.arith != ARITH_F32:
            raise MftxError(f"unknown arithmetic {arith!r}")
        self._nonfinite = torch.zeros(4, dtype=torch.int32, device=self.device)
        check(lib.mftx_raft_set_nonfinite_counter(self._h, self._nonfinite.data_ptr()), "mftx_raft_set_nonfinite_counter")
        options = dict(options or {})
        self._gather = bool(options.pop("gather", 1))
        for k, v in options.items():
            self.set_option(k, v)
        self.ondemand_corr = bool(ondemand_corr)
        if self.ondemand_corr:
            check(lib.mftx_raft_set_ondemand(self._h, 1), "mftx_raft_set_ondemand")

    def __del__(self):
        try:
            if getattr(self, "_h", None):
                _lib.load().mftx_raft_destroy(self._h)
                self._h = None
        except Exception:
            pass

    def debug_refine(self, fmap1, fmap2, net, inp, h, w, iters, pads=(0, 0, 0, 0), flow_init=None):
        lib = _lib.load()
        P = fmap1.shape[0]
        M = P * h * w
        trace = torch.empty(iters + 1, M, 2, dtype=torch.float32, device=self.device)
        check(lib.mftx_raft_set_coords_trace(self._h, trace.data_ptr()), "mftx_raft_set_coords_trace")
        try:
            out = self.refine(fmap1, fmap2, net, inp, h, w, iters, pads=pads, flow_init=flow_init)
        finally:
            check(lib.mftx_raft_set_coords_trace(self._h, None), "mftx_raft_set_coords_trace")
        if self.ondemand_corr:
            pyramid = None
        else:
# ... 32 lines not shown
        if name == "tile_volume":
            self._tile_volume = int(value)

    def workspace(self, P, h, w):
        need = _lib.load().mftx_raft_workspace_bytes_for(self._h, P, h, w)
        if self._ws is None or self._ws.numel() < need:
            if self._ws is not None:
                check(_lib.load().mftx_raft_clear_graphs(self._h), "mftx_raft_clear_graphs")
            self._ws = torch.empty(need, dtype=torch.uint8, device=self.device)
        return self._ws

    REGIONS = ("lvl0", "lvl1", "lvl2", "lvl3", "coords1", "corr", "cor1", "corflo", "flo1", "hx", "z", "rh", "fh",
               "delta", "mask", "ouin", "ouh", "ou", "flow_lr")

    SPLIT_REGIONS = {"cor1": 256, "corflo": 256, "flo1": 128, "hx": 384, "rh": 128, "ouin": 712}

    def region(self, name, P, h, w, cols):
        offs = (C.c_size_t * 19)()
        check(_lib.load().mftx_raft_workspace_layout_for(self._h, P, h, w, offs, 19), "mftx_raft_workspace_layout_for")
        off = offs[self.REGIONS.index(name)]
        M = P * h * w
        if self.arith == ARITH_SPLIT and name in self.SPLIT_REGIONS:
            ld = self.SPLIT_REGIONS[name]
            raw = self._ws[off: off + 4 * M * ld].view(torch.float32).reshape(M, ld)
            return unsplit_activations(raw)[:, :cols]
        return self._ws[off: off + 4 * M * cols].view(torch.float32).reshape(M, cols)

    MAX_GATHER = 16

    def can_gather(self, P):
        return (self.arith == ARITH_SPLIT and not self.ondemand_corr and P <= self.MAX_GATHER and
                getattr(self, "_tile_volume", 1) != 0 and getattr(self, "_gather", True))

    def prepare_frame(self, fmap, inp, h, w, context=True, split=True):
        lib = _lib.load()
        N = h * w
        dev = self.device
        ctx = fsplit = scratch = None
        if context:
            ctx = tuple(torch.empty(N, c, dtype=torch.float32, device=dev) for c in (256, 128, 256, 128))
            scratch = torch.empty(lib.mftx_raft_frame_prepare_bytes(h, w), dtype=torch.uint8, device=dev)
        if split:
            fsplit = torch.empty(N, 256, dtype=torch.float32, device=dev)
        cp = [t.data_ptr() for t in ctx] if context else [None] * 4
        check(lib.mftx_raft_frame_prepare(self._h, h, w, _chk(fmap, "fmap") if split else None, _chk(inp, "inp") if context else None,
                                          *cp, fsplit.data_ptr() if split else None,
                                          scratch.data_ptr() if context else None, scratch.numel() if context else 0, _stream()),
              "mftx_raft_frame_prepare")
        return ctx, fsplit

    def refine(self, fmap1, fmap2, net, inp, h, w, iters, pads=(0, 0, 0, 0), want_flow_lr=False, flow_init=None,
               packed=None, planar=True, prepared=None):
        lib = _lib.load()
        gathered = isinstance(fmap1, (list, tuple))
        P = len(fmap1) if gathered else fmap1.shape[0]
        pl, pr, pt, pb = pads
        H0, W0 = 8 * h - pt - pb, 8 * w - pl - pr
        dev = self.device
        if not planar and packed is None:
            raise MftxError("refine: planar=False needs a packed output")
        flow = torch.empty(P, 2, H0, W0, dtype=torch.float32, device=dev) if planar else None
        occl = torch.empty(P, 1, H0, W0, dtype=torch.float32, device=dev) if planar else None
        sigma = torch.empty(P, 1, H0, W0, dtype=torch.float32, device=dev) if planar else None
        flow_lr = torch.empty(P, h * w, 2, dtype=torch.float32, device=dev) if want_flow_lr else None
        if flow_init is not None and tuple(flow_init.shape) != (P, h * w, 2):
            raise MftxError("flow_init must be [P, h*w, 2]")
        if packed is not None and tuple(packed.shape) != (P, H0, W0, 4):
            raise MftxError("packed must be [P, H0, W0, 4]")
        ws = self.workspace(P, h, w)
        if gathered:
            if not self.can_gather(P) or not (len(fmap2) == len(net) == len(inp) == P):
                raise MftxError("refine: per-pair map lists need the split arithmetic with the tile-resident volume and P <= 16")
            arrs = [_lib.ptr_array([_chk(t, "map") for t in lst]) for lst in (fmap1, fmap2, net, inp)]
            if prepared:
                ctx, f1s, f2s = prepared.get("ctx"), prepared.get("f1s"), prepared.get("f2s")
                if (ctx is not None and len(ctx) != P) or (f1s is not None and len(f1s) != P):
                    raise MftxError("refine: prepared parts for every pair, or none")
                carr = _lib.ptr_array([_chk(t, "context part") for parts in ctx for t in parts]) if ctx is not None else (None, None)
                sarr = _lib.ptr_array([_chk(t, "split map") for t in f1s]) if f1s is not None else (None, None)
                check(lib.mftx_raft_refine_gather_ex(self._h, P, h, w, iters, arrs[0][0], arrs[1][0], arrs[2][0], arrs[3][0],
                                                     carr[0], sarr[0], _chk(f2s, "split map") if f2s is not None else None,
                                                     _chk(flow_init, "flow_init") if flow_init is not None else None,
                                                     pl, pr, pt, pb,
                                                     flow.data_ptr() if planar else None, occl.data_ptr() if planar else None,
                                                     sigma.data_ptr() if planar else None,
                                                     _chk(packed, "packed") if packed is not None else None,
                                                     flow_lr.data_ptr() if want_flow_lr else None,
                                                     ws.data_ptr(), ws.numel(), _stream()), "mftx_raft_refine_gather_ex")
                return (flow, occl, sigma, flow_lr) if want_flow_lr else (flow, occl, sigma)
            check(lib.mftx_raft_refine_gather(self._h, P, h, w, iters, arrs[0][0], arrs[1][0], arrs[2][0], arrs[3][0],
                                              _chk(flow_init, "flow_init") if flow_init is not None else None,
                                              pl, pr, pt, pb,
                                              flow.data_ptr() if planar else None, occl.data_ptr() if planar else None,
                                              sigma.data_ptr() if planar else None,
                                              _chk(packed, "packed") if packed is not None else None,
                                              flow_lr.data_ptr() if want_flow_lr else None,
                                              ws.data_ptr(), ws.numel(), _stream()), "mftx_raft_refine_gather")
            return (flow, occl, sigma, flow_lr) if want_flow_lr else (flow, occl, sigma)
        if prepared:
            raise MftxError("refine: prepared parts go with per-pair map lists")
        check(lib.mftx_raft_refine(self._h, P, h, w, iters, _chk(fmap1, "fmap1"), _chk(fmap2, "fmap2"),
                                   _chk(net, "net"), _chk(inp, "inp"),
                                   _chk(flow_init, "flow_init") if flow_init is not None else None,
                                   pl, pr, pt, pb,
                                   flow.data_ptr() if planar else None, occl.data_ptr() if planar else None,
                                   sigma.data_ptr() if planar else None,
                                   _chk(packed, "packed") if packed is not None else None,
                                   flow_lr.data_ptr() if want_flow_lr else None,
                                   ws.data_ptr(), ws.numel(), _stream()), "mftx_raft_refine")
        return (flow, occl, sigma, flow_lr) if want_flow_lr else (flow, occl, sigma)
```

### mft_amd/raft.py

```python
from __future__ import annotations

import logging
import os
from pathlib import Path

import numpy as np
import torch
import torch.nn.functional as F

from . import ops
from .weights import make_weights, strip_module_prefix

logger = logging.getLogger(__name__)


def pad_amounts(H0, W0):
    ph = (((H0 // 8) + 1) * 8 - H0) % 8
    pw = (((W0 // 8) + 1) * 8 - W0) % 8
    return pw // 2, pw - pw // 2, ph // 2, ph - ph // 2


_STREAMS = {}


def _shared_stream(device, kind, index=0):
    device = torch.device(device)
    dev_index = device.index if device.index is not None else torch.cuda.current_device()
    key = (dev_index, kind, index)
    st = _STREAMS.get(key)
    if st is None:
        st = _STREAMS[key] = torch.cuda.Stream(device=torch.device("cuda", dev_index))
    return st


class FrameFeatures:
    __slots__ = ("fmap", "net", "inp", "h", "w", "pads", "shape", "ready", "ctx", "fsplit")

    def __init__(self, fmap, net, inp, h, w, pads, shape, ready=None):
        self.fmap, self.net, self.inp, self.h, self.w, self.pads, self.shape = fmap, net, inp, h, w, pads, shape
        self.ready = ready
        self.ctx = None
        self.fsplit = None

    def tensors(self):
        return [t for t in (self.fmap, self.net, self.inp, self.fsplit) + tuple(self.ctx or ()) if t is not None]


class RAFTWrapper:
    has_packed_output = True
    STAGING_SLOTS = 4

    def __init__(self, config, device="cuda", state_dict=None):
        self.C = config
        self.device = torch.device(device)
        if self.device.type != "cuda":
            raise RuntimeError("mft_amd.RAFTWrapper runs on an MI355X (HIP) device only; there is no CPU path")
        if state_dict is None:
            state_dict = self._load_weights(config)
        sd = {k: (v if isinstance(v, torch.Tensor) else torch.from_numpy(np.asarray(v)))
              for k, v in strip_module_prefix(state_dict).items()}
        self.sd = {k: v.to(self.device) for k, v in sd.items()}
        self._ondemand = bool(getattr(getattr(config, "raft_params", None), "alternate_corr", False))
        arith = getattr(getattr(config, "raft_params", None), "arith", None) or "split"
        if arith not in ("split", "fp32"):
            raise ValueError(f"raft_params.arith must be 'split' or 'fp32', got {arith!r}")
        self._arith = ops.ARITH_SPLIT if arith == "split" else ops.ARITH_F32
        self._engine_options = dict(getattr(getattr(config, "raft_params", None), "engine_options", None) or {})
        try:
            self._build_engines()
        except ops.SplitRangeError as e:
            logger.warning("raft_params.arith = 'split' refused (%s): falling back to arith = 'fp32'", e)
            self._arith = ops.ARITH_F32
            self._build_engines()
        self._check_finite = bool(getattr(getattr(config, "raft_params", None), "check_finite", False))
        self._split_streams = int(os.environ.get("MFTX_SPLIT_STREAMS", "") or getattr(config, "split_streams", 0) or
                                  (1 if self._arith == ops.ARITH_SPLIT else 2))
        self._engines, self._side = [], []
        self._fif = self._frames_in_flight_setting(config)
# ... 11 lines not shown
        ae = getattr(config, "__dict__", {}).get("async_encode", None)
        self._enc_waits_for_device_frames = ae is None
        if ae is None:
            ae = self._frames_in_flight_setting(config) > 1
        self._enc_stream = _shared_stream(self.device, "enc") if ae else None

    def _frames_in_flight_setting(self, config):
        return max(1, int(os.environ.get("MFTX_FRAMES_IN_FLIGHT", "") or getattr(config, "frames_in_flight", 0) or
                          (2 if self._arith == ops.ARITH_SPLIT else 1)))

    def _build_engines(self):
        graph = bool(self._engine_options.get("graph", 1))
        self.fnet_engine = ops.EncoderEngine(self.sd, "fnet", True, self.device, arith=self._arith, graph=graph)
        self.cnet_engine = ops.EncoderEngine(self.sd, "cnet", False, self.device, arith=self._arith, graph=graph)
        self.engine = ops.RaftEngine(self.sd, self.device, ondemand_corr=self._ondemand, arith=self._arith,
                                     options=self._engine_options)

    def set_nominal_pairs(self, n):
        n = max(1, int(n))
        if n != self.nominal_pairs:
            self.nominal_pairs = n
            self._tile_choice = {}

    def _pin_kernels(self, h, w):
        if self._arith != ops.ARITH_SPLIT or "tile_conv" in self._engine_options:
            return
        v = self._tile_choice.get((h, w))
        if v is None:
            v = self._tile_choice[(h, w)] = 2 if ops._lib.load().mftx_tile_conv_fills_chip(self.nominal_pairs, h, w) else 0
        for e in self._all_engines():
            if getattr(e, "_tile_conv", None) != v:
                e.set_option("tile_conv", v)

    PREPARED_FRAMES = 34

    def _prepare(self, f):
        if not self._frame_prepare or f.net is None or not self.engine.can_gather(1) or f.h < 16 or f.w < 16:
            return
        opt = self._engine_options
        if int(opt.get("presplit", 1)) == 0:
            return
        self._pin_kernels(f.h, f.w)
        fits = self._prepare_ok.get((f.h, f.w))
        if fits is None:
            per_frame = f.h * f.w * 4096
            need = self.PREPARED_FRAMES * per_frame
            ws_bytes = int(ops._lib.load().mftx_raft_workspace_bytes_for(self.engine._h, self.nominal_pairs, f.h, f.w))
            for k in range(self._fif):
                e = self._lanes[k][0] if k < len(self._lanes) else (self.engine if k == 0 else None)
                have = e._ws.numel() if e is not None and e._ws is not None else 0
                need += max(0, ws_bytes - have)
            free, total = torch.cuda.mem_get_info(self.device)
            cached = torch.cuda.memory_reserved(self.device) - torch.cuda.memory_allocated(self.device)
            fits = self._prepare_ok[(f.h, f.w)] = need <= free + cached - total // 10
            if not fits:
                logger.warning("frame_prepare: %.1f MB of prepared parts per cached frame of %d x %d cells do not fit beside the "
                               "workspaces (%.1f GB free): computing them per pair", per_frame / 1e6, f.h, f.w, (free + cached) / 1e9)
        if not fits:
            return
        context = getattr(self.engine, "_tile_conv", 1) == 2 and int(opt.get("fuse_gru", 1)) != 0
        f.ctx, f.fsplit = self.engine.prepare_frame(f.fmap, f.inp, f.h, f.w, context=context, split=True)

    def _prepared(self, fls, frs, flow_init):
        if not self._frame_prepare or flow_init is not None:
            return None
        ctx = [f.ctx for f in fls] if all(f.ctx is not None for f in fls) and getattr(self.engine, "_tile_conv", 1) == 2 else None
        f1s = [f.fsplit for f in fls] if all(f.fsplit is not None for f in fls) else None
        f2s = frs[0].fsplit if all(f is frs[0] for f in frs) else None
        if ctx is None and f1s is None and f2s is None:
            return None
        return {"ctx": ctx, "f1s": f1s, "f2s": f2s}

    def _all_engines(self):
        return list(dict.fromkeys([self.engine] + list(self._engines) + [e for e, _ in self._lanes]))

    def _lane(self):
        while len(self._lanes) < self._fif:
            eng = self.engine if not self._lanes else ops.RaftEngine(self.sd, self.device, ondemand_corr=self._ondemand,
                                                                      arith=self._arith, options=self._engine_options)
            self._lanes.append((eng, _shared_stream(self.device, "lane", len(self._lanes))))
            self._lanes_stale = True
        lane = self._lanes[self._lane_next % self._fif]
        self._lane_next += 1
        return lane

    def _lanes_fit(self, P, h, w):
        while self._fif > max(1, len(self._lanes)):
            k = max(1, len(self._lanes))
            need = int(ops._lib.load().mftx_raft_workspace_bytes_for(self.engine._h, P, h, w))
            free, total = torch.cuda.mem_get_info(self.device)
            cached = torch.cuda.memory_reserved(self.device) - torch.cuda.memory_allocated(self.device)
            if need <= free + cached - total // 10:
                return
            logger.warning("frames_in_flight = %d needs %.1f GB more workspace (lane %d, %d pairs of %d x %d cells) but only %.1f GB of "
                           "the device's %.1f GB are free: running with %d frame(s) in flight", self._fif, need / 1e9, k, P, h, w,
                           (free + cached) / 1e9, total / 1e9, k)
            self._fif = k

    def nonfinite_count(self, reset=False):
        return sum(e.nonfinite_count(reset=reset) for e in self._all_engines())

    def nonfinite_snapshot(self, host_words):
        for i, e in enumerate(self._all_engines()):
            e.nonfinite_snapshot(host_words[i])
# ... 399 lines not shown
```

Measured before the change: 193.1 frames/s.

## Hoist OU-head context-input conv contribution into per-frame prepared parts

Splits the occlusion/uncertainty head's first 3x3 conv weights so that the part acting on the loop-invariant context features (inp) is computed once per frame, or once per refine when not supplied, and stored as a 256-channel partial. The fused OU head then uses a smaller weight tile and adds the cached partial. When all context parts are supplied, init_state also skips copying the inp half of the state. This removes repeated per-pair conv work on the same frame's context features, at the cost of extra per-frame HBM storage (prepared bytes per cell rise from 4096 to 5120) and more API surface.

```diff
diff --git a/include/mftx.h b/include/mftx.h
--- a/include/mftx.h
+++ b/include/mftx.h
@@ -76,6 +76,11 @@
 int mftx_pack_ou_heads_weights(const float *w1pk, int cin_pad, const float *w2pk, void *wtile, void *wproj, void *stream);
 int mftx_ou_heads(const float *a_split, int lda, int P, int h, int w, const void *wtile, const float *b1, const void *wproj, const float *b2,
                   float *T, float *out, int ld_out, void *stream);
+#define MFTX_OU_HEADS_WTILE4_BYTES 5455872
+#define MFTX_OU_HEADS_WCTX_BYTES 1179648
+int mftx_pack_ou_heads_context_weights(const float *w1pk, int cin_pad, void *wtile4, void *wctx, void *stream);
+int mftx_ou_heads_context(const float *a_split, int lda, const float *ou_ctx, int P, int h, int w, const void *wtile4, const void *wproj,
+                          const float *b2, float *T, float *out, int ld_out, int cells, void *stream);
 int mftx_gru_half(const float *h_in, int ld_hin, const float *motion, int ld_mo, const void *wzr, const void *wq, const float *pre_zr,
                   const float *pre_q, float *z, const float *hf_in, float *hf_out, float *h_out, int ld_hout, int P, int h, int w, int pass,
                   void *stream);
@@ -101,6 +106,7 @@
 int mftx_raft_set_tile_weights(mftx_raft *r, const void *const *tile, int n);
 int mftx_raft_set_flow_head(mftx_raft *r, const void *wproj);
 int mftx_raft_set_ou_heads(mftx_raft *r, const void *wtile, const void *wproj);
+int mftx_raft_set_ou_context(mftx_raft *r, const void *wtile4, const void *wctx);
 int mftx_raft_set_coords_trace(mftx_raft *r, float *trace);
 #define MFTX_RAFT_OPT_FORK 0
 #define MFTX_RAFT_OPT_PRESPLIT 1
@@ -142,6 +148,15 @@
                                const float *flow_init, int pad_left, int pad_right, int pad_top, int pad_bottom,
                                float *flow, float *occl, float *sigma, float *packed, float *flow_lr_out,
                                void *workspace, size_t workspace_bytes, void *stream);
+int mftx_raft_frame_prepare_ex(mftx_raft *r, int h, int w, const float *fmap, const float *inp, float *ctx_zr1, float *ctx_q1,
+                               float *ctx_zr2, float *ctx_q2, float *ou_ctx, void *fmap_split, void *scratch, size_t scratch_bytes,
+                               void *stream);
+int mftx_raft_refine_gather_ex2(mftx_raft *r, int P, int h, int w, int iters, const float *const *fmap1,
+                                const float *const *fmap2, const float *const *net, const float *const *inp,
+                                const float *const *ctx_parts, const float *const *ou_parts, const void *const *fmap1_split,
+                                const void *fmap2_split, const float *flow_init, int pad_left, int pad_right, int pad_top,
+                                int pad_bottom, float *flow, float *occl, float *sigma, float *packed, float *flow_lr_out,
+                                void *workspace, size_t workspace_bytes, void *stream);
 int mftx_volume_query_split(const float *in, void *out, long long n_floats, void *stream);
 
 typedef struct mftx_encoder mftx_encoder;
diff --git a/mft_amd/_lib.py b/mft_amd/_lib.py
--- a/mft_amd/_lib.py
+++ b/mft_amd/_lib.py
@@ -13,6 +13,8 @@
 FLOW_BRANCH_WEIGHT_BYTES = 352256
 FLOW_HEAD_WEIGHT_BYTES = 32768
 OU_HEADS_WTILE_BYTES = 6635520
+OU_HEADS_WTILE4_BYTES = 5455872
+OU_HEADS_WCTX_BYTES = 1179648
 SPLIT_LIMIT = 65504.0
 
 
@@ -59,6 +61,10 @@
     "mftx_pack_ou_heads_weights": (C.c_int, [C.c_void_p, C.c_int, C.c_void_p, C.c_void_p, C.c_void_p, C.c_void_p]),
     "mftx_ou_heads": (C.c_int, [C.c_void_p, C.c_int, C.c_int, C.c_int, C.c_int, C.c_void_p, C.c_void_p, C.c_void_p, C.c_void_p, C.c_void_p,
                                 C.c_void_p, C.c_int, C.c_void_p]),
+    "mftx_raft_set_ou_context": (C.c_int, [C.c_void_p, C.c_void_p, C.c_void_p]),
+    "mftx_pack_ou_heads_context_weights": (C.c_int, [C.c_void_p, C.c_int, C.c_void_p, C.c_void_p, C.c_void_p]),
+    "mftx_ou_heads_context": (C.c_int, [C.c_void_p, C.c_int, C.c_void_p, C.c_int, C.c_int, C.c_int, C.c_void_p, C.c_void_p, C.c_void_p, C.c_void_p,
+                                        C.c_void_p, C.c_int, C.c_int, C.c_void_p]),
     "mftx_pack_flow_head_weights": (C.c_int, [C.c_void_p, C.c_void_p, C.c_void_p]),
     "mftx_flow_head": (C.c_int, [C.c_void_p, C.c_int, C.c_int, C.c_int, C.c_int] + [C.c_void_p] * 8),
     "mftx_pack_tile_conv_weights": (C.c_int, [C.c_void_p, C.c_int, C.c_int, C.c_int, C.c_int, C.c_void_p, C.c_void_p]),
@@ -99,6 +105,12 @@
                                              C.c_int, C.c_int, C.c_int, C.c_int,
                                              C.c_void_p, C.c_void_p, C.c_void_p, C.c_void_p, C.c_void_p,
                                              C.c_void_p, C.c_size_t, C.c_void_p]),
+    "mftx_raft_refine_gather_ex2": (C.c_int, [C.c_void_p, C.c_int, C.c_int, C.c_int, C.c_int,
+                                              _PP, _PP, _PP, _PP, _PP, _PP, _PP, C.c_void_p, C.c_void_p,
+                                              C.c_int, C.c_int, C.c_int, C.c_int,
+                                              C.c_void_p, C.c_void_p, C.c_void_p, C.c_void_p, C.c_void_p,
+                                              C.c_void_p, C.c_size_t, C.c_void_p]),
+    "mftx_raft_frame_prepare_ex": (C.c_int, [C.c_void_p, C.c_int, C.c_int] + [C.c_void_p] * 9 + [C.c_size_t, C.c_void_p]),
     "mftx_raft_frame_prepare_bytes": (C.c_size_t, [C.c_int, C.c_int]),
     "mftx_raft_frame_prepare": (C.c_int, [C.c_void_p, C.c_int, C.c_int] + [C.c_void_p] * 8 + [C.c_size_t, C.c_void_p]),
     "mftx_volume_query_split": (C.c_int, [C.c_void_p, C.c_void_p, C.c_longlong, C.c_void_p]),
diff --git a/mft_amd/csrc/common.h b/mft_amd/csrc/common.h
--- a/mft_amd/csrc/common.h
+++ b/mft_amd/csrc/common.h
@@ -158,8 +158,11 @@
 constexpr size_t OU_HEAD_WTILE_BYTES = 8ull * 5 * 9 * 9 * 128 * 16, OU_HEAD_WPROJ_BYTES = 32768;
 int launch_pack_ou_head(const float *w1pk, int cin_pad, const float *w2pk, void *wtile, void *wproj, hipStream_t s);
 struct OuGather { const float *hx, *corr; int ld_corr; const float *coords1, *delta; float *flow_lr; };
+constexpr size_t OU_HEAD_WTILE4_BYTES = 8ull * (90 + 3 * 81) * 128 * 16, OU_HEAD_WCTX_BYTES = 256ull * 9 * 128 * 4;
+struct OuContext { const float *part; const float *const *table; };
+int launch_pack_ou_head4(const float *w1pk, int cin_pad, void *wtile4, void *wctx, hipStream_t s);
 int launch_ou_heads(const float *a, int lda, int P, int h, int w, const void *wtile, const float *b1, const void *wproj, const float *b2, float *T,
-                    float *out, int ld_out, int cells, hipStream_t s, const OuGather *ga = nullptr);
+                    float *out, int ld_out, int cells, hipStream_t s, const OuGather *ga = nullptr, const OuContext *oc = nullptr);
 int launch_flow_head_sum(const float *T, const float *b2, float *delta, const float *coords_in, float *coords_out, int P, int h, int w, hipStream_t s);
 bool tile_conv_applicable(int kh, int kw, int cin, int N);
 bool tile_conv_small_tiles_fill(int P, int h, int w);
diff --git a/mft_amd/csrc/raft_engine.hip b/mft_amd/csrc/raft_engine.hip
--- a/mft_amd/csrc/raft_engine.hip
+++ b/mft_amd/csrc/raft_engine.hip
@@ -9,7 +9,8 @@
 
 
 struct InitGather { int on; PairPtrs netp, inpp; };
-struct CtxTable { const float **table; const float *own[4]; int supplied; PairPtrs parts[4]; };
+struct CtxTable { const float **table; const float *own[4]; int supplied; PairPtrs parts[4];
+                  const float **otable; const float *oown; int osupplied; PairPtrs oparts; int skip_inp; };
 __global__ void init_state_kernel(const float *__restrict__ net, const float *__restrict__ inp,
                                   const float *__restrict__ flow_init, float *hx, float *hf, float *coords1, int M, int h,
                                   int w, InitGather ga, CtxTable ct) {
@@ -19,7 +20,9 @@
         const int b = (int)(i >> 2), k = (int)(i & 3);
         ct.table[i] = ct.supplied ? ct.parts[k].p[b] : ct.own[k] + (long long)b * h * w * ((k & 1) ? 128 : 256);
     }
+    if (ct.otable != nullptr && i < (long long)(M / (h * w))) ct.otable[i] = ct.osupplied ? ct.oparts.p[i] : ct.oown + i * h * w * 256;
     const int m = (int)(i >> 6), q = (int)(i & 63);
+    if (ct.skip_inp && q >= 32) return;
     if (ga.on) {
         const int b = m / (h * w);
         net = ga.netp.p[b] - (long long)b * h * w * 128;
@@ -114,6 +117,8 @@
     float *hf;
     float *hb, *hfb;
     const float **ctx;
+    float *ou_ctx;
+    const float **octx;
     int ld_corr;
     size_t bytes;
 };
@@ -152,6 +157,8 @@
     ws.hb = take(split ? M * 128 : 0);
     ws.hfb = take(split ? M * 128 : 0);
     ws.ctx = reinterpret_cast<const float **>(take(split ? (size_t)P * 8 : 0));
+    ws.ou_ctx = take(split ? M * 256 : 0);
+    ws.octx = reinterpret_cast<const float **>(take(split ? (size_t)P * 2 : 0));
     ws.bytes = off;
     return ws;
 }
@@ -175,6 +182,7 @@
     const void *wproj;
     const void *wt[W_COUNT];
     const void *wou, *wouproj;
+    const void *wou4, *wouctx;
     int opt[13];
     unsigned *nonfinite;
 };
@@ -199,6 +207,7 @@
     r->wflow = nullptr;
     r->wproj = nullptr;
     r->wou = nullptr; r->wouproj = nullptr;
+    r->wou4 = nullptr; r->wouctx = nullptr;
     for (int i = 0; i < W_COUNT; ++i) r->wt[i] = nullptr;
     r->coords_trace = nullptr;
     r->nonfinite = nullptr;
@@ -299,6 +308,15 @@
     if ((wtile == nullptr) != (wproj == nullptr)) return fail(MFTX_E_ARG, "raft_set_ou_heads: both weight streams, or neither");
     if (wtile && (!aligned16(wtile) || !aligned16(wproj))) return fail(MFTX_E_ALIGN, "raft_set_ou_heads: weights not 16-byte aligned");
     r->wou = wtile; r->wouproj = wproj;
+    if (r->graphs) r->graphs->clear();
+    return 0;
+}
+
+extern "C" int mftx_raft_set_ou_context(mftx_raft *r, const void *wtile4, const void *wctx) {
+    if (!r || r->magic != RAFT_MAGIC) return fail(MFTX_E_STATE, "raft_set_ou_context: bad handle");
+    if ((wtile4 == nullptr) != (wctx == nullptr)) return fail(MFTX_E_ARG, "raft_set_ou_context: both weight streams, or neither");
+    if (wtile4 && (!aligned16(wtile4) || !aligned16(wctx))) return fail(MFTX_E_ALIGN, "raft_set_ou_context: weights not 16-byte aligned");
+    r->wou4 = wtile4; r->wouctx = wctx;
     if (r->graphs) r->graphs->clear();
     return 0;
 }
@@ -370,7 +388,16 @@
     return d;
 }
 
-struct RefineGather { PairPtrs f1, f2, net, inp; bool f2_shared; bool has_ctx, has_f1s; PairPtrs ctx[4], f1s; const float *f2s; };
+struct RefineGather { PairPtrs f1, f2, net, inp; bool f2_shared; bool has_ctx, has_f1s; PairPtrs ctx[4], f1s; const float *f2s; bool has_octx; PairPtrs octx; };
+
+static int launch_ou_context_part(const mftx_raft *r, const float *inp, int ld, int P, int h, int w, float *out, hipStream_t s) {
+    TileConvLaunch t{};
+    t.a0 = inp; t.lda0 = ld; t.cin = 128; t.wf = r->wouctx; t.bias = r->w[B_OU1];
+    t.P = P; t.h = h; t.w = w; t.N = 256; t.kh = 3; t.kw = 3; t.epi = 0;
+    t.cells = r->opt[MFTX_RAFT_OPT_TILE_CELLS];
+    t.out = out; t.ldo = 256;
+    return launch_tile_conv(t, s);
+}
 
 static int launch_context_parts(const mftx_raft *r, bool tiles_on, bool sp, const float *inp, int ld, int P, int h, int w,
                                 float *const zr[2], float *const q[2], hipStream_t s) {
@@ -460,6 +487,10 @@
     const bool gru_fused = tile_w(W_ZR1_DYN) && tile_w(W_Q1_DYN) && tile_w(W_ZR2_DYN) && tile_w(W_Q2_DYN) &&
                            r->opt[MFTX_RAFT_OPT_FUSE_GRU] != 0;
     const bool ctx_supplied = gather && gather->has_ctx && gru_fused;
+    const bool ou_fused = tiles_on && r->wou != nullptr && r->opt[MFTX_RAFT_OPT_FUSE_OU] != 0;
+    const bool ou_hoist = ou_fused && r->wou4 != nullptr && r->wouctx != nullptr;
+    const bool octx_supplied = ou_hoist && gather && gather->has_octx;
+    const bool skip_inp = ctx_supplied && octx_supplied && r->opt[MFTX_RAFT_OPT_FUSE_OU] != 2;
     {
         const long long slots = (long long)M * 64;
         ProfScope prof(PC_GLUE, s, 0);
@@ -472,6 +503,11 @@
             ct.supplied = ctx_supplied ? 1 : 0;
             if (ctx_supplied) for (int k = 0; k < 4; ++k) ct.parts[k] = gather->ctx[k];
         }
+        if (ou_hoist) {
+            ct.otable = ws.octx; ct.oown = ws.ou_ctx; ct.osupplied = octx_supplied ? 1 : 0;
+            if (octx_supplied) ct.oparts = gather->octx;
+        }
+        ct.skip_inp = skip_inp ? 1 : 0;
         hipLaunchKernelGGL(init_state_kernel, dim3((unsigned)((slots + 255) / 256)), dim3(256), 0, s, net, inp,
                            flow_init, ws.hx, SP ? ws.hf : nullptr, ws.coords1, M, h, w, ga, ct);
         TRY(check_launch("init_state"));
@@ -486,6 +522,7 @@
         return t;
     };
     if (!ctx_supplied) TRY(launch_context_parts(r, tiles_on, SP, ws.hx + 128, 384, P, h, w, ws.pre_zr, ws.pre_q, s));
+    if (ou_hoist && !octx_supplied) TRY(launch_ou_context_part(r, ws.hx + 128, 384, P, h, w, ws.ou_ctx, s));
     const float *lv[4] = {ws.lvl[0], ws.lvl[1], ws.lvl[2], ws.lvl[3]};
     const int strips = cdiv(w, F1_CELLS);
     float *ccur = ws.coords1, *calt = ws.flo1;
@@ -625,7 +662,6 @@
             TRY(launch_tile_conv(t, s));
         } else TRY(launch_conv(gemm(conv_desc(ws.hx, 384, 128, nullptr, 0, 0, G[W_MASK0], W[B_MASK0], ws.fh, 256, P, h, w, 256, 3, 3, 1), true, true), s));
         TRY(launch_conv(gemm(conv_desc(ws.fh, 256, 256, nullptr, 0, 0, G[W_MASK2], W[B_MASK2], ws.mask, 576, P, h, w, 576, 1, 1, 0, 0.25f), true, false), s));
-        const bool ou_fused = tiles_on && r->wou != nullptr && r->opt[MFTX_RAFT_OPT_FUSE_OU] != 0;
         if (!ou_fused || r->opt[MFTX_RAFT_OPT_FUSE_OU] == 2) {
             const long long slots = (long long)M * 178;
             ProfScope prof(PC_GLUE, s, 0);
@@ -635,9 +671,10 @@
         }
         if (ou_fused) {
             const OuGather ga{ws.hx, ws.corr, ws.ld_corr, ccur, ws.delta, flow_lr};
+            const OuContext oc{nullptr, ws.octx};
             const bool mat = r->opt[MFTX_RAFT_OPT_FUSE_OU] == 2;
-            TRY(launch_ou_heads(mat ? ws.ouin : nullptr, 712, P, h, w, r->wou, W[B_OU1], r->wouproj, W[B_OU2], ws.ouh, ws.ou, 4, r->opt[MFTX_RAFT_OPT_TILE_CELLS], s,
-                                mat ? nullptr : &ga));
+            TRY(launch_ou_heads(mat ? ws.ouin : nullptr, 712, P, h, w, ou_hoist ? r->wou4 : r->wou, W[B_OU1], r->wouproj, W[B_OU2], ws.ouh, ws.ou, 4,
+                                r->opt[MFTX_RAFT_OPT_TILE_CELLS], s, mat ? nullptr : &ga, ou_hoist ? &oc : nullptr));
         } else {
             TRY(launch_conv(gemm(conv_desc(ws.ouin, 712, 712, nullptr, 0, 0, G[W_OU1], W[B_OU1], ws.ouh, 256, P, h, w, 256, 3, 3, 1), true, false), s));
             TRY(launch_conv(conv_desc(ws.ouh, 256, 256, nullptr, 0, 0, W[W_OU2], W[B_OU2], ws.ou, 4, P, h, w, 3, 3, 3, 0), s));
@@ -652,7 +689,7 @@
         key.v[4] = reinterpret_cast<uintptr_t>(workspace); key.v[5] = reinterpret_cast<uintptr_t>(flow_lr_out);
         key.v[6] = (uintptr_t)AR; key.v[7] = reinterpret_cast<uintptr_t>(r->wfused); key.v[8] = reinterpret_cast<uintptr_t>(s);
         key.v[9] = reinterpret_cast<uintptr_t>(r->wflow); key.v[10] = reinterpret_cast<uintptr_t>(r->wt[W_ZR1_DYN]); key.v[11] = reinterpret_cast<uintptr_t>(r->wproj);
-        key.v[12] = reinterpret_cast<uintptr_t>(r->wou); key.v[13] = ctx_supplied ? 1 : 0;
+        key.v[12] = reinterpret_cast<uintptr_t>(r->wou); key.v[13] = (ctx_supplied ? 1 : 0) | (octx_supplied ? 2 : 0);
         TRY(r->graphs->run(key, s, core));
     } else {
         TRY(core());
@@ -685,6 +722,16 @@
                                           const float *flow_init, int pad_left, int pad_right, int pad_top, int pad_bottom,
                                           float *flow, float *occl, float *sigma, float *packed, float *flow_lr_out,
                                           void *workspace, size_t workspace_bytes, void *stream) {
+    return mftx_raft_refine_gather_ex2(r, P, h, w, iters, fmap1, fmap2, net, inp, ctx_parts, nullptr, fmap1_split, fmap2_split, flow_init, pad_left, pad_right,
+                                       pad_top, pad_bottom, flow, occl, sigma, packed, flow_lr_out, workspace, workspace_bytes, stream);
+}
+
+extern "C" int mftx_raft_refine_gather_ex2(mftx_raft *r, int P, int h, int w, int iters, const float *const *fmap1,
+                                           const float *const *fmap2, const float *const *net, const float *const *inp,
+                                           const float *const *ctx_parts, const float *const *ou_parts, const void *const *fmap1_split,
+                                           const void *fmap2_split, const float *flow_init, int pad_left, int pad_right, int pad_top,
+                                           int pad_bottom, float *flow, float *occl, float *sigma, float *packed, float *flow_lr_out,
+                                           void *workspace, size_t workspace_bytes, void *stream) {
     if (!r || r->magic != RAFT_MAGIC) return fail(MFTX_E_STATE, "raft_refine_gather: bad handle");
     if (!fmap1 || !fmap2 || !net || !inp) return fail(MFTX_E_ARG, "raft_refine_gather: null pointer");
     if (P < 1 || P > MFTX_MAX_GATHER) return fail(MFTX_E_ARG, "raft_refine_gather: 1 .. %d pairs", MFTX_MAX_GATHER);
@@ -704,6 +751,14 @@
         g.has_ctx = true;
         for (int b = 0; b < P; ++b) for (int k = 0; k < 4; ++k) g.ctx[k].p[b] = ctx_parts[4 * b + k];
     }
+    if (ou_parts) {
+        g.has_octx = true;
+        for (int b = 0; b < P; ++b) {
+            if (ou_parts[b] && !aligned16(ou_parts[b])) return fail(MFTX_E_ALIGN, "raft_refine_gather: the heads' context part of pair %d not 16-byte aligned", b);
+            if (!ou_parts[b]) g.has_octx = false;
+            g.octx.p[b] = ou_parts[b];
+        }
+    }
     if (fmap1_split) {
         for (int b = 0; b < P; ++b) {
             if (!fmap1_split[b] || !aligned16(fmap1_split[b])) return fail(MFTX_E_ALIGN, "raft_refine_gather: split map of pair %d null or not 16-byte aligned", b);
@@ -735,9 +790,16 @@
 
 extern "C" int mftx_raft_frame_prepare(mftx_raft *r, int h, int w, const float *fmap, const float *inp, float *ctx_zr1, float *ctx_q1,
                                        float *ctx_zr2, float *ctx_q2, void *fmap_split, void *scratch, size_t scratch_bytes, void *stream) {
+    return mftx_raft_frame_prepare_ex(r, h, w, fmap, inp, ctx_zr1, ctx_q1, ctx_zr2, ctx_q2, nullptr, fmap_split, scratch, scratch_bytes, stream);
+}
+
+extern "C" int mftx_raft_frame_prepare_ex(mftx_raft *r, int h, int w, const float *fmap, const float *inp, float *ctx_zr1, float *ctx_q1,
+                                          float *ctx_zr2, float *ctx_q2, float *ou_ctx, void *fmap_split, void *scratch, size_t scratch_bytes,
+                                          void *stream) {
     if (!r || r->magic != RAFT_MAGIC) return fail(MFTX_E_STATE, "raft_frame_prepare: bad handle");
     if (h < 16 || w < 16 || (long long)h * w > (1ll << 24)) return fail(MFTX_E_ARG, "raft_frame_prepare: bad size");
-    const bool want_ctx = ctx_zr1 || ctx_q1 || ctx_zr2 || ctx_q2;
+    const bool want_gru = ctx_zr1 || ctx_q1 || ctx_zr2 || ctx_q2;
+    const bool want_ctx = want_gru || ou_ctx;
     if (!want_ctx && !fmap_split) return fail(MFTX_E_ARG, "raft_frame_prepare: nothing to write");
     if (r->arith != MFTX_ARITH_SPLIT || r->opt[MFTX_RAFT_OPT_PRESPLIT] == 0)
         return fail(MFTX_E_STATE, "raft_frame_prepare: needs the split arithmetic with split-form activations");
@@ -748,11 +810,13 @@
         TRY(launch_split_weights(fmap, fmap_split, N * 256, s));
     }
     if (!want_ctx) return 0;
-    if (!inp || !ctx_zr1 || !ctx_q1 || !ctx_zr2 || !ctx_q2 || !scratch) return fail(MFTX_E_ARG, "raft_frame_prepare: the context parts need inp, all four outputs and the scratch");
+    if (!inp || !scratch || (want_gru && (!ctx_zr1 || !ctx_q1 || !ctx_zr2 || !ctx_q2)))
+        return fail(MFTX_E_ARG, "raft_frame_prepare: the context parts need inp, all four outputs and the scratch");
     if (r->opt[MFTX_RAFT_OPT_TILE_CONV] == 1)
         return fail(MFTX_E_STATE, "raft_frame_prepare: MFTX_RAFT_OPT_TILE_CONV must be pinned (0 or 2), the batch decides otherwise");
-    if (!aligned16(inp) || !aligned16(ctx_zr1) || !aligned16(ctx_q1) || !aligned16(ctx_zr2) || !aligned16(ctx_q2) ||
-        (reinterpret_cast<uintptr_t>(scratch) & 255))
+    if (ou_ctx && !r->wouctx) return fail(MFTX_E_STATE, "raft_frame_prepare: the heads' context part needs mftx_raft_set_ou_context");
+    if (!aligned16(inp) || (want_gru && (!aligned16(ctx_zr1) || !aligned16(ctx_q1) || !aligned16(ctx_zr2) || !aligned16(ctx_q2))) ||
+        (ou_ctx && !aligned16(ou_ctx)) || (reinterpret_cast<uintptr_t>(scratch) & 255))
         return fail(MFTX_E_ALIGN, "raft_frame_prepare: maps must be 16-byte and the scratch 256-byte aligned");
     if (scratch_bytes < mftx_raft_frame_prepare_bytes(h, w))
         return fail(MFTX_E_WORKSPACE, "raft_frame_prepare: scratch %zu < %zu bytes", scratch_bytes, mftx_raft_frame_prepare_bytes(h, w));
@@ -762,6 +826,8 @@
         hipLaunchKernelGGL(split_rows_kernel, dim3((unsigned)((slots + 255) / 256)), dim3(256), 0, s, inp, inps, slots, 32);
         TRY(check_launch("split_rows"));
     }
+    if (ou_ctx) TRY(launch_ou_context_part(r, inps, 128, 1, (int)h, (int)w, ou_ctx, s));
+    if (!want_gru) return 0;
     float *const zr[2] = {ctx_zr1, ctx_zr2}, *const q[2] = {ctx_q1, ctx_q2};
     return launch_context_parts(r, r->opt[MFTX_RAFT_OPT_TILE_CONV] == 2, true, inps, 128, 1, h, w, zr, q, s);
 }
@@ -886,6 +952,17 @@
     return launch_ou_heads(a_split, lda, P, h, w, wtile, b1, wproj, b2, T, out, ld_out, 0, (hipStream_t)stream);
 }
 
+extern "C" int mftx_pack_ou_heads_context_weights(const float *w1pk, int cin_pad, void *wtile4, void *wctx, void *stream) {
+    return launch_pack_ou_head4(w1pk, cin_pad, wtile4, wctx, (hipStream_t)stream);
+}
+
+extern "C" int mftx_ou_heads_context(const float *a_split, int lda, const float *ou_ctx, int P, int h, int w, const void *wtile4, const void *wproj,
+                                     const float *b2, float *T, float *out, int ld_out, int cells, void *stream) {
+    if (!ou_ctx) return fail(MFTX_E_ARG, "ou_heads_context: null pointer");
+    const OuContext oc{ou_ctx, nullptr};
+    return launch_ou_heads(a_split, lda, P, h, w, wtile4, nullptr, wproj, b2, T, out, ld_out, cells, (hipStream_t)stream, nullptr, &oc);
+}
+
 extern "C" int mftx_pack_flow_head_weights(const float *w2pk, void *wproj, void *stream) {
     return launch_pack_flow_head(w2pk, wproj, (hipStream_t)stream);
 }
diff --git a/mft_amd/csrc/tile_conv.hip b/mft_amd/csrc/tile_conv.hip
--- a/mft_amd/csrc/tile_conv.hip
+++ b/mft_amd/csrc/tile_conv.hip
@@ -44,7 +44,7 @@
     static constexpr int A_BYTES = HCELLS * CELLB, RED_BYTES = KS * CELLS * RED_ROW * 4;
     static constexpr int LDS = A_BYTES > RED_BYTES ? A_BYTES : RED_BYTES;
     static constexpr int PROJ_ROW = 20, PROJ_BYTES = 2 * CELLS * PROJ_ROW * 4;
-    static_assert((CELLS == 128 || CELLS == 64 || CELLS == 32) && (N == 128 || N == 256) && (CIN == 128 || CIN == 256 || CIN == 144), "tile_conv: shapes");
+    static_assert((CELLS == 128 || CELLS == 64 || CELLS == 32) && (N == 128 || N == 256) && (CIN == 128 || CIN == 256 || CIN == 144 || CIN == 160), "tile_conv: shapes");
     static_assert(LDS <= 160 * 1024, "tile_conv: the input tile must fit the CU's LDS");
 };
 
@@ -621,15 +621,112 @@
     const float *hx; const float *corr; int ld_corr; const float *coords1; const float *delta; float *flow_lr;
     const void *wf;
     const float *bias;
+    const float *octx; const float *const *octx_tab;
     const void *wproj; float *tout;
     int P, h, w, tiles_x, tiles_y;
 };
-constexpr int OU_C = 712, OU_PASSES = 5, OU_CP = 144, OU_PROJ_ROW = 28;
-
-template <int TH, int TW, bool GATHER>
+constexpr int OU_CP = 144, OU_PROJ_ROW = 28;
+template <int SCHED> struct OuSched;
+template <> struct OuSched<0> { static constexpr int PASSES = 5, CP0 = OU_CP, C = 712; };
+template <> struct OuSched<1> { static constexpr int PASSES = 4, CP0 = 160, C = 584; };
+template <class G, int CPW> struct OuPassGeom : G { static constexpr int GPW = CPW / 16, STEPS = 9 * GPW; };
+
+template <int TH, int TW, bool GATHER, int SCHED, class G, int CPW>
+__device__ __forceinline__ void ou_pass(const OuHeadArgs &p, unsigned char *lds, const unsigned char *const (&abase)[G::RT], const uint4 *__restrict__ wp,
+                                        bool first, int c0, int x0, int y0, long long img_base, f32x16 (&acc)[G::RT], f32x16 (&accx)[G::RT]) {
+    using GK = OuPassGeom<G, CPW>;
+    constexpr int PF = 3, C = OuSched<SCHED>::C;
+    const int tid = (int)threadIdx.x;
+    uint4 bq[PF][2];
+#pragma unroll
+    for (int s = 0; s < PF; ++s) { bq[s][0] = wp[s * 128]; bq[s][1] = wp[s * 128 + 64]; }
+    if (!first) lds_barrier();
+    if constexpr (!GATHER) {
+        constexpr int PPC = CPW / 4, TOTAL = G::HCELLS * PPC, ROUNDS = (TOTAL + 511) / 512, B = 7;
+#pragma unroll 1
+        for (int rr = 0; rr < ROUNDS; rr += B) {
+            uint4 v[B];
+#pragma unroll
+            for (int k = 0; k < B; ++k) {
+                const int q = (rr + k) * 512 + tid;
+                v[k] = make_uint4(0u, 0u, 0u, 0u);
+                if (rr + k < ROUNDS && q < TOTAL) {
+                    const int c = q / PPC, pc = q - c * PPC;
+                    const int cy = c / G::HWD, cx = c - cy * G::HWD;
+                    const int yy = y0 - 1 + cy, xx = x0 - 1 + cx;
+                    const int ch = c0 + pc * 4;
+                    const int src = SCHED == 1 && ch >= 128 ? ch + 128 : ch;
+                    if (yy >= 0 && yy < p.h && xx >= 0 && xx < p.w && ch < C)
+                        v[k] = *reinterpret_cast<const uint4 *>(p.a + (img_base + (long long)yy * p.w + xx) * p.lda + src);
+                }
+            }
+#pragma unroll
+            for (int k = 0; k < B; ++k) {
+                const int q = (rr + k) * 512 + tid;
+                if (rr + k < ROUNDS && q < TOTAL) {
+                    const int c = q / PPC, pc = q - c * PPC;
+                    *reinterpret_cast<uint4 *>(lds + c * G::CELLB + pc * 16) = v[k];
+                }
+            }
+        }
+    } else {
+        constexpr int GPC = CPW / 8, TOTAL = G::HCELLS * GPC, ROUNDS = (TOTAL + 511) / 512, B = 4;
+        const float k2048l = __builtin_bit_cast(float, __builtin_amdgcn_readfirstlane(0x45000000));
+#pragma unroll 1
+        for (int rr = 0; rr < ROUNDS; rr += B) {
+            f32x4 v0[B], v1[B];
+            int kind[B];
+#pragma unroll
+            for (int k = 0; k < B; ++k) {
+                const int q = (rr + k) * 512 + tid;
+                v0[k] = f32x4{0.f, 0.f, 0.f, 0.f}; v1[k] = v0[k]; kind[k] = 0;
+                if (rr + k < ROUNDS && q < TOTAL) {
+                    const int c = q / GPC, gl = q - c * GPC, gs = c0 / 8 + gl, Gi = SCHED == 1 && gs >= 16 ? gs + 16 : gs;
+                    const int cy = c / G::HWD, cx = c - cy * G::HWD;
+                    const int yy = y0 - 1 + cy, xx = x0 - 1 + cx;
+                    if (yy >= 0 && yy < p.h && xx >= 0 && xx < p.w && Gi < 89) {
+                        const long long cell = img_base + (long long)yy * p.w + xx;
+                        if (Gi < 32 || Gi >= 73) {
+                            const float *src = p.hx + cell * 384 + (Gi < 32 ? 8 * Gi : 256 + 8 * (Gi - 73));
+                            v0[k] = *reinterpret_cast<const f32x4 *>(src); v1[k] = *reinterpret_cast<const f32x4 *>(src + 4); kind[k] = 1;
+                        } else if (Gi < 72) {
+                            const float *src = p.corr + cell * p.ld_corr + 8 * (Gi - 32);
+                            v0[k] = *reinterpret_cast<const f32x4 *>(src); v1[k] = *reinterpret_cast<const f32x4 *>(src + 4); kind[k] = 2;
+                        } else {
+                            v0[k] = *reinterpret_cast<const f32x4 *>(p.corr + cell * p.ld_corr + 320);
+                            const float2 cc = reinterpret_cast<const float2 *>(p.coords1)[cell], dd = reinterpret_cast<const float2 *>(p.delta)[cell];
+                            const float fx = cc.x - (float)xx, fy = cc.y - (float)yy;
+                            v1[k] = f32x4{fx, fy, dd.x, dd.y}; kind[k] = 2;
+                            if (cy >= 1 && cy <= TH && cx >= 1 && cx <= TW) reinterpret_cast<float2 *>(p.flow_lr)[cell] = make_float2(fx, fy);
+                        }
+                    }
+                }
+            }
+#pragma unroll
+            for (int k = 0; k < B; ++k) {
+                const int q = (rr + k) * 512 + tid;
+                if (rr + k < ROUNDS && q < TOTAL) {
+                    const int c = q / GPC, gl = q - c * GPC;
+                    u32x4 hi = __builtin_bit_cast(u32x4, v0[k]), lo = __builtin_bit_cast(u32x4, v1[k]);
+                    if (kind[k] == 2) split8_raw(v0[k], v1[k], k2048l, hi, lo);
+                    *reinterpret_cast<u32x4 *>(lds + c * G::CELLB + gl * 32) = hi;
+                    *reinterpret_cast<u32x4 *>(lds + c * G::CELLB + gl * 32 + 16) = lo;
+                }
+            }
+        }
+    }
+    lds_barrier();
+    tc_kloop<GK, 3>(abase, wp, bq, acc, accx);
+}
+
+template <int TH, int TW, bool GATHER, int SCHED>
 __global__ __launch_bounds__(512, 2) void ou_head_kernel(OuHeadArgs p) {
-    using G = TcGeom<TH, TW, 3, 3, OU_CP, 256>;
-    constexpr int RT = G::RT, CELLS = G::CELLS, PF = 3;
+    using S = OuSched<SCHED>;
+    using G = TcGeom<TH, TW, 3, 3, S::CP0, 256>;
+    using G0 = OuPassGeom<G, S::CP0>;
+    using G1 = OuPassGeom<G, OU_CP>;
+    constexpr int RT = G::RT, CELLS = G::CELLS;
+    constexpr int PEEL = S::CP0 != OU_CP ? 1 : 0;
     extern __shared__ __attribute__((aligned(16))) unsigned char tc_lds[];
     unsigned char *lds = tc_lds;
     const int tid = (int)threadIdx.x, lane = tid & 63, wv = __builtin_amdgcn_readfirstlane(tid >> 6);
@@ -637,7 +734,7 @@
     const int tx_ = tile % p.tiles_x, ty_ = (tile / p.tiles_x) % p.tiles_y, img = tile / (p.tiles_x * p.tiles_y);
     const int x0 = tx_ * TW, y0 = ty_ * TH;
     const long long img_base = (long long)img * p.h * p.w;
-    const uint4 *__restrict__ w2 = reinterpret_cast<const uint4 *>(p.wf) + (long long)(wv * OU_PASSES * G::STEPS) * 128 + lane;
+    const uint4 *__restrict__ w2 = reinterpret_cast<const uint4 *>(p.wf) + (long long)(wv * (G0::STEPS + (S::PASSES - 1) * G1::STEPS)) * 128 + lane;
     f32x16 acc[RT], accx[RT];
 #pragma unroll
     for (int i = 0; i < RT; ++i)
@@ -652,89 +749,11 @@
             abase[i] = lds + ((m / TW) * G::HWD + (m % TW)) * G::CELLB + (lane >> 5) * 32;
         }
     }
+    if constexpr (PEEL) ou_pass<TH, TW, GATHER, SCHED, G, S::CP0>(p, lds, abase, w2, true, 0, x0, y0, img_base, acc, accx);
 #pragma unroll 1
-    for (int pass = 0; pass < OU_PASSES; ++pass) {
-        uint4 bq[PF][2];
-        const uint4 *__restrict__ wp = w2 + (long long)pass * G::STEPS * 128;
-#pragma unroll
-        for (int s = 0; s < PF; ++s) { bq[s][0] = wp[s * 128]; bq[s][1] = wp[s * 128 + 64]; }
-        if (pass) lds_barrier();
-        if constexpr (!GATHER) {
-            constexpr int PPC = OU_CP / 4, TOTAL = G::HCELLS * PPC, ROUNDS = (TOTAL + 511) / 512, B = 7;
-            const int pc_valid = pass == OU_PASSES - 1 ? (OU_C - (OU_PASSES - 1) * OU_CP) / 4 : PPC;
-#pragma unroll 1
-            for (int rr = 0; rr < ROUNDS; rr += B) {
-                uint4 v[B];
-#pragma unroll
-                for (int k = 0; k < B; ++k) {
-                    const int q = (rr + k) * 512 + tid;
-                    v[k] = make_uint4(0u, 0u, 0u, 0u);
-                    if (rr + k < ROUNDS && q < TOTAL) {
-                        const int c = q / PPC, pc = q - c * PPC;
-                        const int cy = c / G::HWD, cx = c - cy * G::HWD;
-                        const int yy = y0 - 1 + cy, xx = x0 - 1 + cx;
-                        if (yy >= 0 && yy < p.h && xx >= 0 && xx < p.w && pc < pc_valid)
-                            v[k] = *reinterpret_cast<const uint4 *>(p.a + (img_base + (long long)yy * p.w + xx) * p.lda + pass * OU_CP + pc * 4);
-                    }
-                }
-#pragma unroll
-                for (int k = 0; k < B; ++k) {
-                    const int q = (rr + k) * 512 + tid;
-                    if (rr + k < ROUNDS && q < TOTAL) {
-                        const int c = q / PPC, pc = q - c * PPC;
-                        *reinterpret_cast<uint4 *>(lds + c * G::CELLB + pc * 16) = v[k];
-                    }
-                }
-            }
-        } else {
-            constexpr int GPC = OU_CP / 8, TOTAL = G::HCELLS * GPC, ROUNDS = (TOTAL + 511) / 512, B = 4;
-            const float k2048l = __builtin_bit_cast(float, __builtin_amdgcn_readfirstlane(0x45000000));
-#pragma unroll 1
-            for (int rr = 0; rr < ROUNDS; rr += B) {
-                f32x4 v0[B], v1[B];
-                int kind[B];
-#pragma unroll
-                for (int k = 0; k < B; ++k) {
-                    const int q = (rr + k) * 512 + tid;
-                    v0[k] = f32x4{0.f, 0.f, 0.f, 0.f}; v1[k] = v0[k]; kind[k] = 0;
-                    if (rr + k < ROUNDS && q < TOTAL) {
-                        const int c = q / GPC, gl = q - c * GPC, Gi = GPC * pass + gl;
-                        const int cy = c / G::HWD, cx = c - cy * G::HWD;
-                        const int yy = y0 - 1 + cy, xx = x0 - 1 + cx;
-                        if (yy >= 0 && yy < p.h && xx >= 0 && xx < p.w && Gi < 89) {
-                            const long long cell = img_base + (long long)yy * p.w + xx;
-                            if (Gi < 32 || Gi >= 73) {
-                                const float *src = p.hx + cell * 384 + (Gi < 32 ? 8 * Gi : 256 + 8 * (Gi - 73));
-                                v0[k] = *reinterpret_cast<const f32x4 *>(src); v1[k] = *reinterpret_cast<const f32x4 *>(src + 4); kind[k] = 1;
-                            } else if (Gi < 72) {
-                                const float *src = p.corr + cell * p.ld_corr + 8 * (Gi - 32);
-                                v0[k] = *reinterpret_cast<const f32x4 *>(src); v1[k] = *reinterpret_cast<const f32x4 *>(src + 4); kind[k] = 2;
-                            } else {
-                                v0[k] = *reinterpret_cast<const f32x4 *>(p.corr + cell * p.ld_corr + 320);
-                                const float2 cc = reinterpret_cast<const float2 *>(p.coords1)[cell], dd = reinterpret_cast<const float2 *>(p.delta)[cell];
-                                const float fx = cc.x - (float)xx, fy = cc.y - (float)yy;
-                                v1[k] = f32x4{fx, fy, dd.x, dd.y}; kind[k] = 2;
-                                if (cy >= 1 && cy <= TH && cx >= 1 && cx <= TW) reinterpret_cast<float2 *>(p.flow_lr)[cell] = make_float2(fx, fy);
-                            }
-                        }
-                    }
-                }
-#pragma unroll
-                for (int k = 0; k < B; ++k) {
-                    const int q = (rr + k) * 512 + tid;
-                    if (rr + k < ROUNDS && q < TOTAL) {
-                        const int c = q / GPC, gl = q - c * GPC;
-                        u32x4 hi = __builtin_bit_cast(u32x4, v0[k]), lo = __builtin_bit_cast(u32x4, v1[k]);
-                        if (kind[k] == 2) split8_raw(v0[k], v1[k], k2048l, hi, lo);
-                        *reinterpret_cast<u32x4 *>(lds + c * G::CELLB + gl * 32) = hi;
-                        *reinterpret_cast<u32x4 *>(lds + c * G::CELLB + gl * 32 + 16) = lo;
-                    }
-                }
-            }
-        }
-        lds_barrier();
-        tc_kloop<G, 3>(abase, wp, bq, acc, accx);
-    }
+    for (int pass = PEEL; pass < S::PASSES; ++pass)
+        ou_pass<TH, TW, GATHER, SCHED, G, OU_CP>(p, lds, abase, w2 + (long long)(PEEL * G0::STEPS + (pass - PEEL) * G1::STEPS) * 128, pass == 0,
+                                                 PEEL * S::CP0 + (pass - PEEL) * OU_CP, x0, y0, img_base, acc, accx);
     lds_barrier();
 
     const float inv2048 = 1.f / 2048.f;
@@ -748,9 +767,21 @@
             for (int e = 0; e < 4; ++e) v[e] = acc[i][4 * b + e] + accx[i][4 * b + e] * inv2048;
             *reinterpret_cast<f32x4 *>(red + (32 * i + (lane & 31)) * G::RED_ROW + 32 * wv + 8 * b + 4 * (lane >> 5)) = v;
         }
+    const int mt = wv & 3, kh = wv >> 2;
+    f32x4 cu[SCHED == 1 ? 8 : 1], cv[SCHED == 1 ? 8 : 1];
+    if constexpr (SCHED == 1) {
+        const int m = 32 * mt + (lane & 31), yy = y0 + m / TW, xx = x0 + m % TW;
+        const bool inside = mt < RT && yy < p.h && xx < p.w;
+        const float *part = p.octx_tab != nullptr ? p.octx_tab[img] - img_base * 256 : p.octx;
+        const float *crow = part + (img_base + (long long)(inside ? yy * p.w + xx : 0)) * 256 + 128 * kh + 8 * (lane >> 5);
+#pragma unroll
+        for (int gg = 0; gg < 8; ++gg) {
+            cu[gg] = f32x4{0.f, 0.f, 0.f, 0.f}; cv[gg] = cu[gg];
+            if (inside) { cu[gg] = *reinterpret_cast<const f32x4 *>(crow + 16 * gg); cv[gg] = *reinterpret_cast<const f32x4 *>(crow + 16 * gg + 4); }
+        }
+    }
     lds_barrier();
     const float k2048 = __builtin_bit_cast(float, __builtin_amdgcn_readfirstlane(0x45000000));
-    const int mt = wv & 3, kh = wv >> 2;
     const uint4 *__restrict__ wpj = reinterpret_cast<const uint4 *>(p.wproj) + lane;
     float *tp = reinterpret_cast<float *>(lds + G::RED_BYTES);
     if (mt < RT) {
@@ -762,8 +793,11 @@
         for (int gg = 0; gg < 8; ++gg) {
             const int g = 8 * kh + gg;
             f32x4 u = *reinterpret_cast<const f32x4 *>(xrow + 16 * g), v = *reinterpret_cast<const f32x4 *>(xrow + 16 * g + 4);
-            u += *reinterpret_cast<const f32x4 *>(p.bias + 16 * g + 8 * (lane >> 5));
-            v += *reinterpret_cast<const f32x4 *>(p.bias + 16 * g + 8 * (lane >> 5) + 4);
+            if constexpr (SCHED == 1) { u += cu[gg]; v += cv[gg]; }
+            else {
+                u += *reinterpret_cast<const f32x4 *>(p.bias + 16 * g + 8 * (lane >> 5));
+                v += *reinterpret_cast<const f32x4 *>(p.bias + 16 * g + 8 * (lane >> 5) + 4);
+            }
 #pragma unroll
             for (int e = 0; e < 4; ++e) { u[e] = relu_keep_nan(u[e]); v[e] = relu_keep_nan(v[e]); }
             u32x4 hi, lo;
@@ -795,21 +829,25 @@
     }
 }
 
-__global__ void pack_ou_head_kernel(const float *__restrict__ wpk, int cin_pad, uint4 *__restrict__ out, long long pieces) {
+__global__ void pack_ou_head_kernel(const float *__restrict__ wpk, int cin_pad, int sched, uint4 *__restrict__ out, long long pieces) {
     const long long idx = (long long)blockIdx.x * blockDim.x + threadIdx.x;
     if (idx >= pieces) return;
-    constexpr int GP = OU_CP / 16, STEPS = 9 * GP;
+    const int cp0 = sched ? OuSched<1>::CP0 : OuSched<0>::CP0, passes = sched ? OuSched<1>::PASSES : OuSched<0>::PASSES, C = sched ? OuSched<1>::C : OuSched<0>::C;
+    const int steps0 = 9 * (cp0 / 16), steps1 = 9 * (OU_CP / 16), per_nt = steps0 + (passes - 1) * steps1;
     const int lane = (int)(idx & 63), part = (int)((idx >> 6) & 1);
     const long long t = idx >> 7;
-    const int step = (int)(t % STEPS), pass = (int)((t / STEPS) % OU_PASSES), nt = (int)(t / STEPS / OU_PASSES);
+    const int nt = (int)(t / per_nt), r = (int)(t % per_nt);
+    const int pass = r < steps0 ? 0 : 1 + (r - steps0) / steps1, step = r < steps0 ? r : (r - steps0) % steps1;
+    const int GP = (pass ? OU_CP : cp0) / 16, c0 = pass ? cp0 + (pass - 1) * OU_CP : 0;
     const int tap = step / GP, g = step % GP;
     const int n = 32 * nt + (lane & 31);
     unsigned w[4];
 #pragma unroll
     for (int e = 0; e < 4; ++e) {
-        const int c = OU_CP * pass + 16 * g + 8 * (lane >> 5) + 2 * e;
-        const long long base = ((long long)n * 9 + tap) * cin_pad + c;
-        const unsigned a = split_halves(c < OU_C ? wpk[base] : 0.f), b = split_halves(c + 1 < OU_C ? wpk[base + 1] : 0.f);
+        const int c = c0 + 16 * g + 8 * (lane >> 5) + 2 * e;
+        const int src = sched && c >= 128 ? c + 128 : c;
+        const long long base = ((long long)n * 9 + tap) * cin_pad + src;
+        const unsigned a = split_halves(c < C ? wpk[base] : 0.f), b = split_halves(c + 1 < C ? wpk[base + 1] : 0.f);
         w[e] = part ? ((a >> 16) | (b & 0xffff0000u)) : ((a & 0xffffu) | (b << 16));
     }
     out[idx] = make_uint4(w[0], w[1], w[2], w[3]);
@@ -853,42 +891,59 @@
 
 int launch_pack_ou_head(const float *w1pk, int cin_pad, const float *w2pk, void *wtile, void *wproj, hipStream_t s) {
     if (!w1pk || !w2pk || !wtile || !wproj) return fail(MFTX_E_ARG, "pack_ou_head_weights: null pointer");
-    if (cin_pad < OU_C) return fail(MFTX_E_ARG, "pack_ou_head_weights: the first layers have 712 input channels");
+    if (cin_pad < OuSched<0>::C) return fail(MFTX_E_ARG, "pack_ou_head_weights: the first layers have 712 input channels");
     if (!aligned16(wtile) || !aligned16(wproj)) return fail(MFTX_E_ALIGN, "pack_ou_head_weights: outputs not 16-byte aligned");
-    const long long pieces = 8ll * OU_PASSES * 9 * (OU_CP / 16) * 128;
-    hipLaunchKernelGGL(pack_ou_head_kernel, dim3((unsigned)((pieces + 255) / 256)), dim3(256), 0, s, w1pk, cin_pad, reinterpret_cast<uint4 *>(wtile), pieces);
+    const long long pieces = (long long)(OU_HEAD_WTILE_BYTES / 16);
+    hipLaunchKernelGGL(pack_ou_head_kernel, dim3((unsigned)((pieces + 255) / 256)), dim3(256), 0, s, w1pk, cin_pad, 0, reinterpret_cast<uint4 *>(wtile), pieces);
     hipLaunchKernelGGL(pack_proj27_kernel, dim3(8), dim3(256), 0, s, w2pk, reinterpret_cast<uint4 *>(wproj));
     return check_launch("pack_ou_head");
 }
 
-template <int TH, int TW, bool GATHER>
+int launch_pack_ou_head4(const float *w1pk, int cin_pad, void *wtile4, void *wctx, hipStream_t s) {
+    if (!w1pk || !wtile4 || !wctx) return fail(MFTX_E_ARG, "pack_ou_heads_context_weights: null pointer");
+    if (cin_pad < OuSched<0>::C || cin_pad % 4) return fail(MFTX_E_ARG, "pack_ou_heads_context_weights: the first layers have 712 input channels (row stride a multiple of 4)");
+    if (!aligned16(w1pk) || !aligned16(wtile4) || !aligned16(wctx)) return fail(MFTX_E_ALIGN, "pack_ou_heads_context_weights: weights and outputs 16-byte aligned");
+    static_assert(OU_HEAD_WTILE4_BYTES == 8ull * (9 * (OuSched<1>::CP0 / 16) + (OuSched<1>::PASSES - 1) * 9 * (OU_CP / 16)) * 128 * 16, "ou_head: the four-pass stream");
+    const long long pieces = (long long)(OU_HEAD_WTILE4_BYTES / 16);
+    hipLaunchKernelGGL(pack_ou_head_kernel, dim3((unsigned)((pieces + 255) / 256)), dim3(256), 0, s, w1pk, cin_pad, 1, reinterpret_cast<uint4 *>(wtile4), pieces);
+    if (int e = check_launch("pack_ou_head4")) return e;
+    return launch_pack_tile_conv(w1pk + 128, 256, 9, 128, cin_pad, wctx, s);
+}
+
+template <int TH, int TW, bool GATHER, int SCHED>
 static int ou_head_launch(OuHeadArgs a, hipStream_t s) {
-    using G = TcGeom<TH, TW, 3, 3, OU_CP, 256>;
+    using S = OuSched<SCHED>;
+    using G = TcGeom<TH, TW, 3, 3, S::CP0, 256>;
     constexpr int lds_bytes = (G::A_BYTES > G::RED_BYTES ? G::A_BYTES : G::RED_BYTES) + 2 * G::CELLS * OU_PROJ_ROW * 4;
-    static_assert(G::RED_BYTES + 2 * G::CELLS * OU_PROJ_ROW * 4 <= 160 * 1024 && lds_bytes <= 160 * 1024, "ou_head: LDS");
+    static_assert(G::A_BYTES + 2 * G::CELLS * OU_PROJ_ROW * 4 <= 160 * 1024 && G::RED_BYTES + 2 * G::CELLS * OU_PROJ_ROW * 4 <= 160 * 1024 && lds_bytes <= 160 * 1024, "ou_head: LDS");
     a.tiles_x = cdiv(a.w, TW); a.tiles_y = cdiv(a.h, TH);
     const long long tiles = (long long)a.P * a.tiles_x * a.tiles_y;
     if (tiles > 0x7fffffffLL) return fail(MFTX_E_ARG, "ou_heads: too many tiles");
-    auto kern = ou_head_kernel<TH, TW, GATHER>;
+    auto kern = ou_head_kernel<TH, TW, GATHER, SCHED>;
     static bool attr_set = false;
     if (!attr_set) {
         if (hipFuncSetAttribute(reinterpret_cast<const void *>(kern), hipFuncAttributeMaxDynamicSharedMemorySize, lds_bytes) != hipSuccess)
             return fail(MFTX_E_STATE, "ou_heads: cannot reserve %d bytes of LDS", lds_bytes);
         attr_set = true;
     }
-    ProfScope prof(PC_CONV_GEMM, s, 2.0 * a.P * a.h * a.w * (256.0 * 9 * OU_C + 256.0 * 27));
+    ProfScope prof(PC_CONV_GEMM, s, 2.0 * a.P * a.h * a.w * (256.0 * 9 * S::C + 256.0 * 27));
     hipLaunchKernelGGL(kern, dim3((unsigned)tiles), dim3(512), lds_bytes, s, a);
     return check_launch("ou_heads");
 }
 
 int launch_ou_heads(const float *a, int lda, int P, int h, int w, const void *wtile, const float *b1, const void *wproj, const float *b2, float *T,
-                    float *out, int ld_out, int cells, hipStream_t s, const OuGather *ga) {
-    if ((!a && !ga) || !wtile || !b1 || !wproj || !b2 || !T || !out) return fail(MFTX_E_ARG, "ou_heads: null pointer");
+                    float *out, int ld_out, int cells, hipStream_t s, const OuGather *ga, const OuContext *oc) {
+    if ((!a && !ga) || !wtile || (!b1 && !oc) || !wproj || !b2 || !T || !out) return fail(MFTX_E_ARG, "ou_heads: null pointer");
     if (P <= 0 || h <= 0 || w <= 0 || ld_out < 3) return fail(MFTX_E_ARG, "ou_heads: bad sizes");
-    if (!aligned16(wtile) || !aligned16(wproj) || !aligned16(b1) || !aligned16(T))
+    if (!aligned16(wtile) || !aligned16(wproj) || (!oc && !aligned16(b1)) || !aligned16(T))
         return fail(MFTX_E_ALIGN, "ou_heads: weights, bias and scratch 16-byte aligned");
     OuHeadArgs k{};
     k.wf = wtile; k.bias = b1; k.wproj = wproj; k.tout = T; k.P = P; k.h = h; k.w = w;
+    if (oc) {
+        if ((oc->part == nullptr) == (oc->table == nullptr)) return fail(MFTX_E_ARG, "ou_heads: the context part as one tensor or as a table of the pairs' parts");
+        if (oc->part && !aligned16(oc->part)) return fail(MFTX_E_ALIGN, "ou_heads: the context part 16-byte aligned");
+        k.octx = oc->part; k.octx_tab = oc->table;
+    }
     if (ga) {
         if (!ga->hx || !ga->corr || !ga->coords1 || !ga->delta || !ga->flow_lr) return fail(MFTX_E_ARG, "ou_heads: null pointer among the input's parts");
         if ((reinterpret_cast<uintptr_t>(ga->hx) & 31) || !aligned16(ga->corr) || ga->ld_corr % 4 || ga->ld_corr < 324 || (reinterpret_cast<uintptr_t>(ga->coords1) & 7) ||
@@ -896,15 +951,18 @@
             return fail(MFTX_E_ALIGN, "ou_heads: hx 32-byte, corr 16-byte (row stride a multiple of 4), coordinates 8-byte aligned");
         k.hx = ga->hx; k.corr = ga->corr; k.ld_corr = ga->ld_corr; k.coords1 = ga->coords1; k.delta = ga->delta; k.flow_lr = ga->flow_lr;
     } else {
-        if ((reinterpret_cast<uintptr_t>(a) & 31) || lda % 8 || lda < OU_C) return fail(MFTX_E_ALIGN, "ou_heads: split-form rows are 32-byte aligned with strides in multiples of 8");
+        if ((reinterpret_cast<uintptr_t>(a) & 31) || lda % 8 || lda < OuSched<0>::C) return fail(MFTX_E_ALIGN, "ou_heads: split-form rows are 32-byte aligned with strides in multiples of 8");
         k.a = a; k.lda = lda;
     }
     if (!cells) cells = tile_conv_cells(P, h, w, 3);
     int e;
-    if (cells == 128) e = ga ? ou_head_launch<8, 16, true>(k, s) : ou_head_launch<8, 16, false>(k, s);
-    else if (cells == 64) e = ga ? ou_head_launch<4, 16, true>(k, s) : ou_head_launch<4, 16, false>(k, s);
-    else if (cells == 32) e = ga ? ou_head_launch<2, 16, true>(k, s) : ou_head_launch<2, 16, false>(k, s);
+#define OU_BY(TH) (oc ? (ga ? ou_head_launch<TH, 16, true, 1>(k, s) : ou_head_launch<TH, 16, false, 1>(k, s)) \
+                      : (ga ? ou_head_launch<TH, 16, true, 0>(k, s) : ou_head_launch<TH, 16, false, 0>(k, s)))
+    if (cells == 128) e = OU_BY(8);
+    else if (cells == 64) e = OU_BY(4);
+    else if (cells == 32) e = OU_BY(2);
     else return fail(MFTX_E_ARG, "ou_heads: 128, 64 or 32 cells per tile");
+#undef OU_BY
     if (e) return e;
     const long long n = (long long)P * h * w * 4;
     ProfScope prof(PC_CONV_SMALL, s, 2.0 * P * h * w * 3 * 9);
diff --git a/mft_amd/ops.py b/mft_amd/ops.py
--- a/mft_amd/ops.py
+++ b/mft_amd/ops.py
@@ -375,6 +375,31 @@
     return wtile, wproj
 
 
+def pack_ou_heads_context_weights(w1pk: torch.Tensor, check_range: bool = True):
+    lib = _lib.load()
+    if w1pk.dim() != 3 or w1pk.shape[0] < 256 or w1pk.shape[1] != 9 or w1pk.shape[2] < 712 or w1pk.shape[2] % 4:
+        raise MftxError("pack_ou_heads_context_weights: expected the packed first layers [>= 256, 9, >= 712]")
+    if check_range and count_not_below(w1pk, _lib.SPLIT_LIMIT):
+        raise SplitRangeError(f"pack_ou_heads_context_weights: weights not below {_lib.SPLIT_LIMIT} in magnitude")
+    wtile4 = torch.empty(_lib.OU_HEADS_WTILE4_BYTES, dtype=torch.uint8, device=w1pk.device)
+    wctx = torch.empty(_lib.OU_HEADS_WCTX_BYTES, dtype=torch.uint8, device=w1pk.device)
+    check(lib.mftx_pack_ou_heads_context_weights(_chk(w1pk, "w1pk"), w1pk.shape[2], wtile4.data_ptr(), wctx.data_ptr(), _stream()),
+          "mftx_pack_ou_heads_context_weights")
+    return wtile4, wctx
+
+
+def ou_heads_context(a_split: torch.Tensor, ou_ctx: torch.Tensor, h: int, w: int, wtile4: torch.Tensor, wproj: torch.Tensor, b2, cells: int = 0):
+    lib = _lib.load()
+    M = a_split.shape[0]
+    P = M // (h * w)
+    T = torch.empty(M, 27, dtype=torch.float32, device=a_split.device)
+    out = torch.zeros(M, 4, dtype=torch.float32, device=a_split.device)
+    check(lib.mftx_ou_heads_context(_chk(a_split, "a"), a_split.shape[1], _chk(ou_ctx, "ou_ctx"), P, h, w, _chk(wtile4, "wtile4", torch.uint8),
+                                    _chk(wproj, "wproj", torch.uint8), _chk(b2, "b2"), T.data_ptr(), out.data_ptr(), 4, int(cells), _stream()),
+          "mftx_ou_heads_context")
+    return out
+
+
 def ou_heads(a_split: torch.Tensor, h: int, w: int, wtile: torch.Tensor, b1, wproj: torch.Tensor, b2):
     lib = _lib.load()
     M = a_split.shape[0]
@@ -807,6 +832,8 @@
             check(lib.mftx_raft_set_flow_head(self._h, self.wproj.data_ptr()), "mftx_raft_set_flow_head")
             self.wou, self.wouproj = pack_ou_heads_weights(self.weights[30], self.weights[32])
             check(lib.mftx_raft_set_ou_heads(self._h, self.wou.data_ptr(), self.wouproj.data_ptr()), "mftx_raft_set_ou_heads")
+            self.wou4, self.wouctx = pack_ou_heads_context_weights(self.weights[30])
+            check(lib.mftx_raft_set_ou_context(self._h, self.wou4.data_ptr(), self.wouctx.data_ptr()), "mftx_raft_set_ou_context")
         elif self.arith != ARITH_F32:
             raise MftxError(f"unknown arithmetic {arith!r}")
         self._nonfinite = torch.zeros(4, dtype=torch.int32, device=self.device)
@@ -905,22 +932,27 @@
         return (self.arith == ARITH_SPLIT and not self.ondemand_corr and P <= self.MAX_GATHER and
                 getattr(self, "_tile_volume", 1) != 0 and getattr(self, "_gather", True))
 
-    def prepare_frame(self, fmap, inp, h, w, context=True, split=True):
+    def prepare_frame(self, fmap, inp, h, w, context=True, split=True, ou_context=False):
         lib = _lib.load()
         N = h * w
         dev = self.device
-        ctx = fsplit = scratch = None
+        ctx = fsplit = scratch = ou_ctx = None
         if context:
             ctx = tuple(torch.empty(N, c, dtype=torch.float32, device=dev) for c in (256, 128, 256, 128))
+        if ou_context:
+            ou_ctx = torch.empty(N, 256, dtype=torch.float32, device=dev)
+        if context or ou_context:
             scratch = torch.empty(lib.mftx_raft_frame_prepare_bytes(h, w), dtype=torch.uint8, device=dev)
         if split:
             fsplit = torch.empty(N, 256, dtype=torch.float32, device=dev)
         cp = [t.data_ptr() for t in ctx] if context else [None] * 4
-        check(lib.mftx_raft_frame_prepare(self._h, h, w, _chk(fmap, "fmap") if split else None, _chk(inp, "inp") if context else None,
-                                          *cp, fsplit.data_ptr() if split else None,
-                                          scratch.data_ptr() if context else None, scratch.numel() if context else 0, _stream()),
+        check(lib.mftx_raft_frame_prepare_ex(self._h, h, w, _chk(fmap, "fmap") if split else None,
+                                             _chk(inp, "inp") if scratch is not None else None,
+                                             *cp, ou_ctx.data_ptr() if ou_context else None, fsplit.data_ptr() if split else None,
+                                             scratch.data_ptr() if scratch is not None else None,
+                                             scratch.numel() if scratch is not None else 0, _stream()),
               "mftx_raft_frame_prepare")
-        return ctx, fsplit
+        return (ctx, fsplit, ou_ctx) if ou_context else (ctx, fsplit)
 
     def refine(self, fmap1, fmap2, net, inp, h, w, iters, pads=(0, 0, 0, 0), want_flow_lr=False, flow_init=None,
                packed=None, planar=True, prepared=None):
@@ -949,17 +981,21 @@
                 ctx, f1s, f2s = prepared.get("ctx"), prepared.get("f1s"), prepared.get("f2s")
                 if (ctx is not None and len(ctx) != P) or (f1s is not None and len(f1s) != P):
                     raise MftxError("refine: prepared parts for every pair, or none")
+                ou = prepared.get("ou")
+                if ou is not None and len(ou) != P:
+                    raise MftxError("refine: prepared parts for every pair, or none")
                 carr = _lib.ptr_array([_chk(t, "context part") for parts in ctx for t in parts]) if ctx is not None else (None, None)
+                oarr = _lib.ptr_array([_chk(t, "context part") if t is not None else None for t in ou]) if ou is not None else (None, None)
                 sarr = _lib.ptr_array([_chk(t, "split map") for t in f1s]) if f1s is not None else (None, None)
-                check(lib.mftx_raft_refine_gather_ex(self._h, P, h, w, iters, arrs[0][0], arrs[1][0], arrs[2][0], arrs[3][0],
-                                                     carr[0], sarr[0], _chk(f2s, "split map") if f2s is not None else None,
-                                                     _chk(flow_init, "flow_init") if flow_init is not None else None,
-                                                     pl, pr, pt, pb,
-                                                     flow.data_ptr() if planar else None, occl.data_ptr() if planar else None,
-                                                     sigma.data_ptr() if planar else None,
-                                                     _chk(packed, "packed") if packed is not None else None,
-                                                     flow_lr.data_ptr() if want_flow_lr else None,
-                                                     ws.data_ptr(), ws.numel(), _stream()), "mftx_raft_refine_gather_ex")
+                check(lib.mftx_raft_refine_gather_ex2(self._h, P, h, w, iters, arrs[0][0], arrs[1][0], arrs[2][0], arrs[3][0],
+                                                      carr[0], oarr[0], sarr[0], _chk(f2s, "split map") if f2s is not None else None,
+                                                      _chk(flow_init, "flow_init") if flow_init is not None else None,
+                                                      pl, pr, pt, pb,
+                                                      flow.data_ptr() if planar else None, occl.data_ptr() if planar else None,
+                                                      sigma.data_ptr() if planar else None,
+                                                      _chk(packed, "packed") if packed is not None else None,
+                                                      flow_lr.data_ptr() if want_flow_lr else None,
+                                                      ws.data_ptr(), ws.numel(), _stream()), "mftx_raft_refine_gather_ex")
                 return (flow, occl, sigma, flow_lr) if want_flow_lr else (flow, occl, sigma)
             check(lib.mftx_raft_refine_gather(self._h, P, h, w, iters, arrs[0][0], arrs[1][0], arrs[2][0], arrs[3][0],
                                               _chk(flow_init, "flow_init") if flow_init is not None else None,
diff --git a/mft_amd/raft.py b/mft_amd/raft.py
--- a/mft_amd/raft.py
+++ b/mft_amd/raft.py
@@ -34,16 +34,17 @@
 
 
 class FrameFeatures:
-    __slots__ = ("fmap", "net", "inp", "h", "w", "pads", "shape", "ready", "ctx", "fsplit")
+    __slots__ = ("fmap", "net", "inp", "h", "w", "pads", "shape", "ready", "ctx", "fsplit", "ou_ctx")
 
     def __init__(self, fmap, net, inp, h, w, pads, shape, ready=None):
         self.fmap, self.net, self.inp, self.h, self.w, self.pads, self.shape = fmap, net, inp, h, w, pads, shape
         self.ready = ready
         self.ctx = None
         self.fsplit = None
+        self.ou_ctx = None
 
     def tensors(self):
-        return [t for t in (self.fmap, self.net, self.inp, self.fsplit) + tuple(self.ctx or ()) if t is not None]
+        return [t for t in (self.fmap, self.net, self.inp, self.fsplit, self.ou_ctx) + tuple(self.ctx or ()) if t is not None]
 
 
 class RAFTWrapper:
@@ -121,6 +122,7 @@
             if getattr(e, "_tile_conv", None) != v:
                 e.set_option("tile_conv", v)
 
+    PREPARED_BYTES_PER_CELL = 5120
     PREPARED_FRAMES = 34
 
     def _prepare(self, f):
@@ -132,7 +134,7 @@
         self._pin_kernels(f.h, f.w)
         fits = self._prepare_ok.get((f.h, f.w))
         if fits is None:
-            per_frame = f.h * f.w * 4096
+            per_frame = f.h * f.w * self.PREPARED_BYTES_PER_CELL
             need = self.PREPARED_FRAMES * per_frame
             ws_bytes = int(ops._lib.load().mftx_raft_workspace_bytes_for(self.engine._h, self.nominal_pairs, f.h, f.w))
             for k in range(self._fif):
@@ -148,7 +150,8 @@
         if not fits:
             return
         context = getattr(self.engine, "_tile_conv", 1) == 2 and int(opt.get("fuse_gru", 1)) != 0
-        f.ctx, f.fsplit = self.engine.prepare_frame(f.fmap, f.inp, f.h, f.w, context=context, split=True)
+        ou = getattr(self.engine, "_tile_conv", 1) == 2 and int(opt.get("fuse_ou", 1)) != 0
+        f.ctx, f.fsplit, f.ou_ctx = (self.engine.prepare_frame(f.fmap, f.inp, f.h, f.w, context=context, split=True, ou_context=ou) + (None,))[:3]
 
     def _prepared(self, fls, frs, flow_init):
         if not self._frame_prepare or flow_init is not None:
@@ -156,9 +159,10 @@
         ctx = [f.ctx for f in fls] if all(f.ctx is not None for f in fls) and getattr(self.engine, "_tile_conv", 1) == 2 else None
         f1s = [f.fsplit for f in fls] if all(f.fsplit is not None for f in fls) else None
         f2s = frs[0].fsplit if all(f is frs[0] for f in frs) else None
-        if ctx is None and f1s is None and f2s is None:
+        ou = [f.ou_ctx for f in fls] if all(f.ou_ctx is not None for f in fls) and getattr(self.engine, "_tile_conv", 1) == 2 else None
+        if ctx is None and f1s is None and f2s is None and ou is None:
             return None
-        return {"ctx": ctx, "f1s": f1s, "f2s": f2s}
+        return {"ctx": ctx, "f1s": f1s, "f2s": f2s, "ou": ou}
 
     def _all_engines(self):
         return list(dict.fromkeys([self.engine] + list(self._engines) + [e for e, _ in self._lanes]))
```

Measured after the change: 194.1 frames/s (median of 6 runs). About the same (+0.5%).
